# 2noise/ChatTTS

Measured on AMD Instinct MI355X. Metric: audio seconds/sec (RTF), batch=64 per GPU, higher is better.
Workload: dtype f32x3

## Files before the change

chattts_amd/_lib.py:

```python
from __future__ import annotations

import ctypes as C
import os

import numpy as np

import torch

HERE = os.path.dirname(os.path.abspath(__file__))
LIB_PATH = os.environ.get("CTTS_LIB") or os.path.join(HERE, "csrc", "libchattts_amd.so")

F32, BF16 = 0, 1
P = C.c_void_p
PP = C.POINTER(C.c_void_p)


class GptWeights(C.Structure):
    _fields_ = [
        ("n_layers", C.c_int32), ("weight_dtype", C.c_int32), ("kv_dtype", C.c_int32), ("max_pos", C.c_int32),
        ("wqkv", PP), ("wo", PP), ("wgu", PP), ("wd", PP), ("ln1", PP), ("ln2", PP),
        ("norm", P), ("emb_code", P), ("heads", P), ("rope_cos", P), ("rope_sin", P),
        ("rms_eps", C.c_float),
        ("emb_text", P), ("head_text", P), ("n_text", C.c_int32),
        ("wqkv_pk", PP), ("wo_pk", PP), ("wgu_pk", PP), ("wd_pk", PP),
        ("heads_pk", P), ("head_text_pk", P),
        ("wo_hd", PP),
        ("wqkv_x3", PP), ("wo_x3", PP), ("wgu_x3", PP), ("wd_x3", PP),
    ]


class GenState(C.Structure):
    _fields_ = [
        ("B", C.c_int32), ("T", C.c_int32), ("max_new", C.c_int32),
        ("ids_buf", P), ("len", P), ("kv_start", P), ("finish", P), ("end_idx", P), ("hiddens", P),
        ("kcache", P), ("vcache", P), ("q", P), ("nq", C.c_int32),
        ("temperature", P), ("pow_table", P),
        ("top_p_thr", C.c_float), ("use_top_p", C.c_int32), ("top_k", C.c_int32), ("use_top_k", C.c_int32),
        ("min_new", C.c_int32), ("eos", C.c_int32), ("row_offset", C.c_int32),
        ("stop_at", P), ("workspace", P), ("workspace_bytes", C.c_size_t), ("row_map", P), ("n_active", P),
        ("cap", C.c_int32), ("hid_cap", C.c_int32), ("kv_batch", C.c_int32), ("q_batch", C.c_int32), ("prompt_len", P),
        ("infer_text", C.c_int32), ("teacher_ids", P), ("sampled_ids", P), ("order", P),
        ("rng_device", C.c_int32), ("rng_per_step", C.c_int32), ("rng_seed", P), ("rng_nonce", P),
        ("margin", P), ("row_base", P), ("proj_exact", C.c_int32), ("prefill_valid_rows", C.c_int32),
        ("row_sampling", P),
    ]


RS_WINDOW = np.dtype([("in_off", "<i8"), ("n_in", "<i8"), ("origin", "<i8"), ("total", "<i8"), ("o_lo", "<i8"), ("o_hi", "<i8"),
                      ("out_off", "<i8"), ("rate", "<i4"), ("pad", "<i4")])


G711_RANGE = np.dtype([("start", "<i8"), ("n", "<i8"), ("law", "<i4"), ("pad0", "<i4"), ("pad1", "<i8")])


class Rate(C.Structure):
    _fields_ = [("taps", P), ("L", C.c_int32), ("M", C.c_int32), ("K", C.c_int32), ("reserved", C.c_int32)]


class SamplingRow(C.Structure):
    _fields_ = [
        ("temperature", C.c_float * 4), ("pow_table", C.c_float * 17), ("use_penalty", C.c_int32),
        ("top_p_thr", C.c_float), ("use_top_p", C.c_int32), ("top_k", C.c_int32), ("use_top_k", C.c_int32),
        ("min_new", C.c_int32), ("reserved0", C.c_int32), ("rng_seed", C.c_uint64), ("rng_per_step", C.c_int32),
        ("reserved1", C.c_int32),
    ]


class CodecWeights(C.Structure):
    _fields_ = [
        ("conv_in0_w", P), ("conv_in0_b", P), ("conv_in2_w", P), ("conv_in2_b", P),
        ("n_dvae_blocks", C.c_int32),
        ("d_dw_w", PP), ("d_dw_b", PP), ("d_ln_w", PP), ("d_ln_b", PP), ("d_pw1_w", PP), ("d_pw1_b", PP),
        ("d_pw2_w", PP), ("d_pw2_b", PP), ("d_gamma", PP),
        ("conv_out_w", P), ("out_conv_w", P), ("coef", P),
        ("v_embed_w", P), ("v_embed_b", P), ("v_norm_w", P), ("v_norm_b", P),
        ("n_vocos_blocks", C.c_int32),
        ("v_dw_w", PP), ("v_dw_b", PP), ("v_ln_w", PP), ("v_ln_b", PP), ("v_pw1_w", PP), ("v_pw1_b", PP),
        ("v_pw2_w", PP), ("v_pw2_b", PP), ("v_gamma", PP),
        ("v_final_w", P), ("v_final_b", P), ("head_w", P), ("head_b", P), ("window", P), ("twiddle", P),
        ("gemm_mode", C.c_int32),
        ("d_pw1_x3p", PP), ("d_pw2_x3p", PP), ("v_pw1_x3p", PP), ("v_pw2_x3p", PP),
    ]


class TrunkWeights(C.Structure):
    _fields_ = [
        ("idim", C.c_int32), ("odim", C.c_int32), ("hidden", C.c_int32), ("bn_dim", C.c_int32), ("n_blocks", C.c_int32),
        ("conv_in0_w", P), ("conv_in0_b", P), ("conv_in2_w", P), ("conv_in2_b", P),
        ("dw_w", PP), ("dw_b", PP), ("ln_w", PP), ("ln_b", PP), ("pw1_w", PP), ("pw1_b", PP), ("pw2_w", PP), ("pw2_b", PP),
        ("gamma", PP), ("conv_out_w", P),
    ]


class DvaeWeights(C.Structure):
    _fields_ = [
        ("encoder", TrunkWeights), ("decoder", TrunkWeights),
        ("ds0_w", P), ("ds0_b", P), ("ds1_w", P), ("ds1_b", P), ("out_conv_w", P), ("coef", P),
        ("q_in_w", P), ("q_in_b", P), ("q_out_w", P), ("q_out_b", P),
        ("levels", C.c_int32 * 4), ("G", C.c_int32), ("R", C.c_int32), ("D", C.c_int32), ("bound_first", C.c_int32),
        ("mel_window", P), ("mel_fb", P), ("twiddle", P),
    ]


I32, F, SZ = C.c_int32, C.c_float, C.c_size_t

SIGNATURES = {
    "ctts_last_error": (C.c_char_p, []),
    "ctts_version": (C.c_int, []),
    "ctts_gpt_create": (C.c_int, [PP, C.POINTER(GptWeights)]),
    "ctts_gpt_destroy": (None, [P]),
    "ctts_gpt_workspace_bytes": (SZ, [I32, I32]),
    "ctts_gpt_prefill": (C.c_int, [P, C.POINTER(GenState), P, P]),
    "ctts_gpt_prefill_chunk": (C.c_int, [P, C.POINTER(GenState), P, I32, I32, I32, P]),
    "ctts_gpt_decode_step": (C.c_int, [P, C.POINTER(GenState), P]),
    "ctts_gpt_graph_build": (C.c_int, [P, C.POINTER(GenState), P]),
    "ctts_gpt_graph_launch": (C.c_int, [P, I32, P]),
    "ctts_gpt_graph_build_rows": (C.c_int, [P, C.POINTER(GenState), I32, P]),
    "ctts_gpt_graph_launch_rows": (C.c_int, [P, I32, I32, P]),
    "ctts_gpt_graph_destroy": (None, [P]),
    "ctts_gpt_profile_begin": (C.c_int, [P, I32, I32, I32]),
    "ctts_gpt_profile_samples": (C.c_int, [P, C.POINTER(C.c_float), I32, C.POINTER(I32)]),
    "ctts_gpt_profile_end": (C.c_int, [P, C.POINTER(I32), C.POINTER(C.c_double)]),
    "ctts_codec_create": (C.c_int, [PP, C.POINTER(CodecWeights)]),
    "ctts_codec_destroy": (None, [P]),
    "ctts_codec_workspace_bytes": (SZ, [I32, I32]),
    "ctts_copy_bytes": (C.c_int, [P, P, SZ, P]),
    "ctts_float_to_int16": (C.c_int, [P, P, P, I32, C.c_int64, C.c_int64, I32, I32, F, P, P]),
    "ctts_dvae_decode": (C.c_int, [P, P, P, I32, I32, P, SZ, P]),
    "ctts_vocos_decode": (C.c_int, [P, P, P, I32, I32, P, SZ, P]),
    "ctts_codec_ragged_workspace_bytes": (SZ, [I32, I32]),
    "ctts_dvae_decode_ragged": (C.c_int, [P, P, P, P, I32, P, P, SZ, P]),
    "ctts_vocos_decode_ragged": (C.c_int, [P, P, P, P, I32, P, P, SZ, P]),
    "ctts_float_to_int16_ragged": (C.c_int, [P, P, P, P, P, I32, I32, F, P, P]),
    "ctts_float_to_int16_groups_scratch_bytes": (SZ, [P, I32, P, I32]),
    "ctts_float_to_int16_groups": (C.c_int, [P, P, P, P, P, I32, P, P, I32, I32, F, P, P, SZ, P]),
    "ctts_resample_supported": (I32, [I32, I32, I32]),
    "ctts_resample_ragged": (C.c_int, [P, P, P, P, P, P, I32, P, P, I32, P, I32, I32, I32, P]),
    "ctts_time_scale_ragged": (C.c_int, [P, P, P, P, P, P, P, P, P, I32, P, I32, I32, P]),
    "ctts_codec_windows_workspace_bytes": (SZ, [I32, I32]),
    "ctts_codec_decode_windows": (C.c_int, [P, P, C.c_int64, C.c_int64, I32, I32, P, P, I32, I32, P, P, I32, F, P, SZ, P]),
    "ctts_resample_windows": (C.c_int, [P, C.c_int64, P, P, I32, P, C.c_int64, P, P, I32, P, I32, I32, I32, P]),
    "ctts_codec_windows_rate_workspace_bytes": (SZ, [I32, I32, C.c_int64]),
    "ctts_codec_decode_windows_rate": (C.c_int, [P, P, C.c_int64, C.c_int64, I32, I32, P, P, P, P, P, P, I32, P, I32, I32, P, P, I32, F, P,
                                                 SZ, P]),
    "ctts_g711_encode_ranges": (C.c_int, [P, P, P, P, I32, P]),
    "ctts_dvae_create": (C.c_int, [PP, C.POINTER(DvaeWeights)]),
    "ctts_dvae_destroy": (None, [P]),
    "ctts_dvae_code_frames": (I32, [I32]),
    "ctts_dvae_encode_workspace_bytes": (SZ, [I32]),
    "ctts_dvae_decode_workspace_bytes": (SZ, [I32, I32]),
    "ctts_dvae_encode": (C.c_int, [P, P, I32, P, P, SZ, P]),
    "ctts_dvae_decode_codes": (C.c_int, [P, P, P, I32, I32, P, SZ, P]),
    "ctts_k_gemm": (C.c_int, [I32, P, P, P, I32, I32, I32, I32, I32, I32, I32, P, F, P, I32, P, P, I32, I32, I32, I32, I32, P]),
    "ctts_k_gemm_x3p": (C.c_int, [P, P, I32, I32, I32, I32, P, P, P, P, P, P]),
    "ctts_k_gemm_h1p": (C.c_int, [P, P, I32, I32, I32, I32, P, P, P, P, P, P]),
    "ctts_stream_create_cu_mask": (C.c_int, [I32, I32, I32, I32, P]),
    "ctts_stream_destroy": (C.c_int, [P]),
    "ctts_k_mlp_fused": (C.c_int, [P, P, P, I32, I32, P, P, P, P, I32, P]),
    "ctts_k_gemm_fast": (C.c_int, [P, I32, P, I32, I32, I32, P, F, I32, P, I32, P, I32, P, P]),
    "ctts_k_qkv_rope": (C.c_int, [P, P, I32, P, F, P, P, P, I32, P, P, I32, P, P, I32, P]),
    "ctts_k_gemm_dec": (C.c_int, [P, P, I32, I32, I32, P, P, F, I32, P, I32, P, I32, P, I32, P]),
    "ctts_k_gemm_dec32x": (C.c_int, [P, C.c_int64, P, C.c_int64, I32, I32, I32, P, P, I32, F, I32, P, I32, P, I32, P, C.c_int64, I32, P, I32, P, P, P]),
    "ctts_k_gemm_pre_x3": (C.c_int, [P, I32, P, P, I32, I32, I32, I32, I32, P, P, P, I32, P]),
    "ctts_k_dec32_last_variant": (C.c_char_p, []),
    "ctts_k_gemm_dec32": (C.c_int, [P, P, I32, I32, I32, P, P, I32, P, F, I32, P, I32, P, I32, P, I32, I32, I32, P]),
    "ctts_k_rows_prep": (C.c_int, [P, P, P, I32, P]),
    "ctts_k_rope_append": (C.c_int, [P, P, P, I32, I32, P, P, I32, P, P, I32, P]),
    "ctts_k_attention": (C.c_int, [P, P, P, I32, I32, P, I32, P, P, I32, P]),
    "ctts_k_attention_prefill": (C.c_int, [P, P, P, I32, P, I32, I32, P, I32, P]),
    "ctts_k_attention_dec": (C.c_int, [P, P, P, I32, P, P, P, I32, P, P, I32, P]),
    "ctts_k_attention_dec2": (C.c_int, [P, P, P, I32, I32, P, P, P, I32, I32, P]),
    "ctts_k_attention_cfg": (C.c_int, [I32, I32, I32]),
    "ctts_k_attention_heads_per_wg": (C.c_int, [I32]),
    "ctts_rccl_unique_id": (C.c_int, [P]),
    "ctts_rccl_comm_create": (C.c_int, [P, I32, P, I32]),
    "ctts_rccl_comm_destroy": (None, [P]),
    "ctts_broadcast_weights": (C.c_int, [P, P, I32, P, I32, P]),
    "ctts_k_attention_oproj": (C.c_int, [P, P, P, I32, P, P, P, I32, P, P, P, P, P, P]),
    "ctts_k_device_guard_probe": (C.c_int, [P, P, P, P, P]),
    "ctts_k_embed_codes": (C.c_int, [P, P, I32, P, P, I32, P]),
    "ctts_k_final_norm": (C.c_int, [P, I32, P, F, P, P, I32, P, I32, I32, P]),
    "ctts_k_sample": (C.c_int, [C.POINTER(GenState), P, P]),
    "ctts_k_sample_text": (C.c_int, [C.POINTER(GenState), P, I32, P]),
    "ctts_k_exp_draws": (C.c_int, [C.c_uint64, I32, I32, I32, I32, P, P]),
    "ctts_k_dwconv_ln": (C.c_int, [P, P, P, P, P, F, I32, P, I32, I32, P]),
    "ctts_k_layernorm": (C.c_int, [P, P, P, F, P, I32, P]),
    "ctts_k_istft": (C.c_int, [P, P, P, P, P, I32, I32, P]),
}

_lib = None


class EngineError(RuntimeError):
    pass


def lib() -> C.CDLL:
    global _lib
    if _lib is None:
        if not os.path.exists(LIB_PATH):
            raise EngineError(
                f"{LIB_PATH} not found: build it with `python -m chattts_amd.build` "
                "(hipcc --offload-arch=gfx950).  chattts_amd has no CPU/eager fallback.")
        l = C.CDLL(LIB_PATH)
        for name, (res, args) in SIGNATURES.items():
            fn = getattr(l, name)
            fn.restype = res
            fn.argtypes = args
        _lib = l
    return _lib


def check(rc: int, what: str = "") -> None:
    if rc != 0:
        msg = lib().ctts_last_error()
        raise EngineError(f"{what}: {msg.decode() if msg else 'unknown error'}")


def ptr(t) -> int:
    return None if t is None else t.data_ptr()


def ptr_array(tensors):
    arr = (C.c_void_p * len(tensors))(*[t.data_ptr() for t in tensors])
    return arr
```

chattts_amd/csrc/capi.hip:

```cpp
#include <hip/hip_runtime.h>
#include <dlfcn.h>
#include <stdarg.h>
#include <stdio.h>
#include <stdlib.h>
#include <string.h>
#include <algorithm>
#include <map>
#include <vector>

#include "../../include/chattts_amd.h"
#include "kernels.hpp"

static thread_local char g_err[512] = "";
int ctts_fail(const char* fmt, ...) {
  va_list ap;
  va_start(ap, fmt);
  vsnprintf(g_err, sizeof(g_err), fmt, ap);
  va_end(ap);
  return -1;
}
#define fail ctts_fail
#define CK(expr)                                                                                   \
  do {                                                                                             \
    hipError_t _e = (expr);                                                                        \
    if (_e != hipSuccess) return fail("%s failed: %s (%s:%d)", #expr, hipGetErrorString(_e), __FILE__, __LINE__); \
  } while (0)

extern "C" const char* ctts_last_error(void) { return g_err; }
extern "C" int ctts_version(void) { return 1; }

static const int HID = 768, INTER = 3072, NHEAD = 12, HDIM = 64, NVQ = 4, NAUDIO = 626, NTEXT_MAX = 21248;

struct ctts_gpt {
  ctts_gpt_weights w;
  std::vector<const void*> wqkv, wo, wgu, wd;
  std::vector<const void*> wqkv_pk, wo_pk, wgu_pk, wd_pk;
  std::vector<const void*> wo_hd;
  std::vector<const void*> wqkv_x3, wo_x3, wgu_x3, wd_x3;
  bool dec_x3 = false;
  bool qkv_att = false;
  bool att_oproj = false;
  bool dec_packed = false;
  bool dec_packed32 = false;
  bool heads_packed = false;
  int pf_mask = 0;
  int temporal_layers = 0;
  bool pre32_packed = true;
  bool embed_fold = false;
  bool pre_compact = true;
  bool pre_x3 = true;
  bool fnorm_fuse = true;
  std::vector<const float*> ln1, ln2;
  hipGraph_t graph = nullptr;
  hipGraphExec_t exec = nullptr;
  hipGraph_t graph_multi = nullptr;
  hipGraphExec_t exec_multi = nullptr;
  struct RowsGraph { hipGraph_t graph = nullptr, gm = nullptr; hipGraphExec_t exec = nullptr, exec_multi = nullptr; };
  std::map<int, RowsGraph> rows_graphs;
  int multi_steps = 1;
  int prof_tag = -1;
  int prof_max = 0;
  bool skip_finished = true;
  int n_cu = 0;
  int prof_stride = 1;
  int prof_seen = 0;
  std::vector<hipEvent_t> ev0, ev1;
  int prof_n = 0;
};

static size_t align_up(size_t v) { return (v + 255) & ~(size_t)255; }
#define ATT_CUS_MAX 512
#define QA_LAYERS_MAX 32
#define QA_STRIDE HO_STRIDE
struct GptWs {
  float *x, *qkv, *ao, *act, *hfin, *logits, *ssq;
  uint16_t* xb;
  uint16_t *xp, *aop, *actp;
  float *xp32, *aop32, *actp32;
  float* hfinp;
  float* rstd;
  RowDesc* desc;
  float* att_part;
  int32_t* att_cnt;
  int32_t* row_map;
  float* rope_cs;
  int32_t* qa_flag;
  float* op_part;
  int32_t* op_cnt;
  size_t op_part_bytes;
  size_t bytes;
};
static size_t cnt_bytes(int B) { return ((size_t)ATT_CUS_MAX + ((size_t)B + 15) / 16 * 16) * sizeof(int32_t); }
static GptWs carve(void* base, int B, int T) {
  const size_t M = (size_t)B * (T > 1 ? T : 1);
  GptWs w;
  size_t off = 0;
  char* p = (char*)base;
  w.x = (float*)(p + off); off += align_up(M * HID * 4);
  w.qkv = (float*)(p + off); off += align_up(M * 3 * HID * 4);
  w.ao = (float*)(p + off); off += align_up(M * HID * 4);
  w.act = (float*)(p + off); off += align_up(M * INTER * 4);
  w.hfin = (float*)(p + off); off += align_up((size_t)B * HID * 4);
  w.logits = (float*)(p + off); off += align_up((size_t)B * NTEXT_MAX * 4);
  w.ssq = (float*)(p + off); off += align_up(M * SSQ_PARTS * 4);
  w.xb = (uint16_t*)(p + off); off += align_up(M * HID * 2);
  const size_t Bp = ((size_t)B + 15) / 16 * 16;
  w.xp = (uint16_t*)(p + off); off += align_up(Bp * HID * 2);
  w.aop = (uint16_t*)(p + off); off += align_up(Bp * HID * 2);
  w.actp = (uint16_t*)(p + off); off += align_up(Bp * INTER * 2);
  const size_t Mp = (M + 15) / 16 * 16;
  w.xp32 = (float*)(p + off); off += align_up(Mp * HID * 4);
  w.aop32 = (float*)(p + off); off += align_up(Mp * HID * 4);
  w.actp32 = (float*)(p + off); off += align_up(Mp * INTER * 4);
  w.hfinp = (float*)(p + off); off += align_up(Bp * HID * 4);
  w.desc = (RowDesc*)(p + off); off += align_up(Mp * sizeof(RowDesc));
  w.rstd = (float*)(p + off); off += align_up(Mp * sizeof(float));
  w.row_map = (int32_t*)(p + off); off += align_up(Bp * sizeof(int32_t));
  w.att_part = (float*)(p + off); off += align_up((size_t)ATT_CUS_MAX * ATT_SPLIT_MAX * 66 * sizeof(float));
  w.att_cnt = (int32_t*)(p + off); off += align_up(cnt_bytes(B));
  w.op_cnt = w.att_cnt + ATT_CUS_MAX;
  w.op_part_bytes = Bp * NHEAD * HID * sizeof(float);
  w.op_part = (float*)(p + off); off += align_up(w.op_part_bytes);
  w.rope_cs = (float*)(p + off); off += align_up(Bp * 64 * sizeof(float));
  w.qa_flag = (int32_t*)(p + off); off += align_up((size_t)QA_LAYERS_MAX * NHEAD * QA_STRIDE * sizeof(int32_t));
  w.bytes = off;
  return w;
}

extern "C" size_t ctts_gpt_workspace_bytes(int32_t B, int32_t T) { return carve(nullptr, B, T).bytes; }

extern "C" int ctts_gpt_create(ctts_gpt** out, const ctts_gpt_weights* w) {
  if (!out || !w || w->n_layers <= 0) return fail("ctts_gpt_create: bad arguments");
  ctts_gpt* g = new ctts_gpt();
  g->w = *w;
  const int L = w->n_layers;
  g->wqkv.assign(w->wqkv, w->wqkv + L);
  g->wo.assign(w->wo, w->wo + L);
  g->wgu.assign(w->wgu, w->wgu + L);
  g->wd.assign(w->wd, w->wd + L);
  g->ln1.assign(w->ln1, w->ln1 + L);
  g->ln2.assign(w->ln2, w->ln2 + L);
  if (w->wqkv_pk && w->wo_pk && w->wgu_pk && w->wd_pk) {
    g->wqkv_pk.assign(w->wqkv_pk, w->wqkv_pk + L);
    g->wo_pk.assign(w->wo_pk, w->wo_pk + L);
    g->wgu_pk.assign(w->wgu_pk, w->wgu_pk + L);
    g->wd_pk.assign(w->wd_pk, w->wd_pk + L);
    const char* e = getenv("CTTS_DEC_PACKED");
    const bool on = !(e && atoi(e) == 0);
    g->dec_packed = on && w->weight_dtype == CTTS_BF16;
    g->dec_packed32 = on && w->weight_dtype != CTTS_BF16 && w->kv_dtype != CTTS_BF16;
  }
  { const char* e = getenv("CTTS_DEC_PACKED"); g->heads_packed = w->heads_pk != nullptr && !(e && atoi(e) == 0); }
  if (w->wqkv_x3 && w->wo_x3 && w->wgu_x3 && w->wd_x3 && w->weight_dtype != CTTS_BF16 && w->kv_dtype != CTTS_BF16) {
    g->wqkv_x3.assign(w->wqkv_x3, w->wqkv_x3 + L);
    g->wo_x3.assign(w->wo_x3, w->wo_x3 + L);
    g->wgu_x3.assign(w->wgu_x3, w->wgu_x3 + L);
    g->wd_x3.assign(w->wd_x3, w->wd_x3 + L);
    g->dec_x3 = true;
  }
  if (w->wo_hd && g->dec_packed) {
    g->wo_hd.assign(w->wo_hd, w->wo_hd + L);
    const char* e = getenv("CTTS_ATT_OPROJ");
    g->att_oproj = e && atoi(e) == 1;
  }
  { const char* e = getenv("CTTS_SKIP_FINISHED"); if (e && atoi(e) == 0) g->skip_finished = false; }
  { const char* e = getenv("CTTS_FNORM_FUSE"); if (e && atoi(e) == 0) g->fnorm_fuse = false; }
  { const char* e = getenv("CTTS_W_TEMPORAL_LAYERS"); if (e) g->temporal_layers = atoi(e); }
  { const char* e = getenv("CTTS_PF"); if (e) g->pf_mask = atoi(e); }
  { const char* e = getenv("CTTS_QKV_ATT"); g->qkv_att = e && atoi(e) == 1; }
  { const char* e = getenv("CTTS_PRE32_PACKED"); if (e && atoi(e) == 0) g->pre32_packed = false; }
  { const char* e = getenv("CTTS_PRE_X3"); if (e && atoi(e) == 0) g->pre_x3 = false; }
  { const char* e = getenv("CTTS_PRE_COMPACT"); if (e && atoi(e) == 0) g->pre_compact = false; }
  { const char* e = getenv("CTTS_EMBED_FOLD"); if (e) g->embed_fold = atoi(e) != 0; }
  {
    int dev = 0, cus = 0;
    const char* e = getenv("CTTS_ATT_SPLIT");
    if (e && atoi(e) == 1 && hipGetDevice(&dev) == hipSuccess &&
        hipDeviceGetAttribute(&cus, hipDeviceAttributeMultiprocessorCount, dev) == hipSuccess && cus > 0 && cus <= ATT_CUS_MAX)
      g->n_cu = cus;
  }
  *out = g;
  return 0;
}

extern "C" void ctts_gpt_graph_destroy(ctts_gpt* g) {
  if (!g) return;
  if (g->exec) { (void)hipGraphExecDestroy(g->exec); g->exec = nullptr; }
  if (g->graph) { (void)hipGraphDestroy(g->graph); g->graph = nullptr; }
  if (g->exec_multi) { (void)hipGraphExecDestroy(g->exec_multi); g->exec_multi = nullptr; }
  if (g->graph_multi) { (void)hipGraphDestroy(g->graph_multi); g->graph_multi = nullptr; }
  for (auto& kv : g->rows_graphs) {
    if (kv.second.exec) (void)hipGraphExecDestroy(kv.second.exec);
    if (kv.second.graph) (void)hipGraphDestroy(kv.second.graph);
    if (kv.second.exec_multi) (void)hipGraphExecDestroy(kv.second.exec_multi);
    if (kv.second.gm) (void)hipGraphDestroy(kv.second.gm);
  }
  g->rows_graphs.clear();
}

extern "C" void ctts_gpt_destroy(ctts_gpt* g) {
  if (!g) return;
  ctts_gpt_graph_destroy(g);
  for (auto e : g->ev0) (void)hipEventDestroy(e);
  for (auto e : g->ev1) (void)hipEventDestroy(e);
  delete g;
}

thread_local hipEvent_t ctts_prof_start = nullptr, ctts_prof_stop = nullptr;

struct Prof {
  ctts_gpt* g; bool on;
  Prof(ctts_gpt* g_, int tag, hipStream_t, bool allow) : g(g_), on(false) {
    if (allow && g->prof_tag == tag && g->prof_n < g->prof_max && (g->prof_seen++ % g->prof_stride) == 0) {
      on = true;
      ctts_prof_start = g->ev0[g->prof_n];
      ctts_prof_stop = g->ev1[g->prof_n];
    }
  }
  ~Prof() {
    if (on) { g->prof_n++; ctts_prof_start = nullptr; ctts_prof_stop = nullptr; }
  }
};

static_assert(sizeof(SamplingRow) == sizeof(ctts_sampling_row) && sizeof(ctts_sampling_row) == 128, "ctts_sampling_row layout");
static_assert(offsetof(SamplingRow, pow_table) == offsetof(ctts_sampling_row, pow_table) &&
              offsetof(SamplingRow, min_new) == offsetof(ctts_sampling_row, min_new) &&
              offsetof(SamplingRow, rng_seed) == offsetof(ctts_sampling_row, rng_seed) &&
              offsetof(SamplingRow, rng_per_step) == offsetof(ctts_sampling_row, rng_per_step), "ctts_sampling_row layout");

static SampleArgs make_sample_args(const ctts_gen_state* s, const float* logits) {
  SampleArgs a;
  a.logits = logits; a.ids_buf = s->ids_buf; a.tcap = s->cap ? s->cap : s->T + s->max_new; a.T = s->T; a.len = s->len; a.finish = s->finish;
  a.end_idx = s->end_idx; a.q = s->q; a.nq = s->nq; a.temperature = s->temperature; a.pow_table = s->pow_table;
  a.top_p_thr = s->top_p_thr; a.use_top_p = s->use_top_p; a.top_k = s->top_k; a.use_top_k = s->use_top_k;
  a.min_new = s->min_new; a.eos = s->eos; a.row_offset = s->row_offset; a.max_input_ids = NAUDIO - 1; a.stop_at = s->stop_at;
  a.B = s->B; a.row_map = nullptr; a.n_active = nullptr; a.prompt_len = s->prompt_len; a.q_rows = s->q_batch ? s->q_batch : s->B;
  a.teacher = s->teacher_ids; a.teacher_stride = s->hid_cap ? s->hid_cap : s->max_new; a.sampled = s->sampled_ids;
  a.dbg = nullptr;
  { const char* e = getenv("CTTS_SAMPLE_DBG_PTR"); if (e) a.dbg = (long long*)strtoull(e, nullptr, 0); }
  a.desc = nullptr; a.rng_device = s->rng_device; a.rng_per_step = s->rng_per_step; a.rng_seed = reinterpret_cast<const unsigned long long*>(s->rng_seed);
  a.rng_nonce = s->rng_nonce;
  a.margin = s->margin; a.row_base = s->row_base;
  a.rows = reinterpret_cast<const SamplingRow*>(s->row_sampling);
  memset(&a.next, 0, sizeof(a.next));
  return a;
}

static int check_state(const ctts_gpt* g, const ctts_gen_state* s, int ws_T = 0) {
  if (!g || !s) return fail("null engine/state");
  if (s->B <= 0 || s->T <= 0 || s->max_new <= 0) return fail("bad B/T/max_new");
  const int cap_ = s->cap ? s->cap : s->T + s->max_new;
  if (cap_ > g->w.max_pos) return fail("slot capacity T + max_new (%d) exceeds the RoPE table (%d)", cap_, g->w.max_pos);
  if (s->cap && s->T + 1 > s->cap) return fail("prompt does not fit the slot capacity");
  if (s->workspace_bytes < ctts_gpt_workspace_bytes(s->B, ws_T > 0 ? ws_T : s->T)) return fail("workspace too small");
  if (!s->rng_device && (s->nq <= 0 || !s->q)) return fail("q draws missing");
  if (s->rng_device && !s->rng_seed && !s->row_sampling) return fail("rng_device needs the rng_seed device scalar (or row_sampling)");
  if (g->w.weight_dtype == CTTS_BF16 && g->w.kv_dtype != CTTS_BF16) return fail("perf mode needs a bf16 KV cache");
  if (s->infer_text) {
    if (!g->w.emb_text || !g->w.head_text || g->w.n_text <= 0 || g->w.n_text > NTEXT_MAX) return fail("text head/embedding not loaded");
    if (s->pow_table) return fail("refine-text mode does not support a repetition penalty (the reference's own processor mis-broadcasts there)");
    if (s->eos < 0 || s->eos >= g->w.n_text) return fail("bad eos for text mode");
  }
  return 0;
}

static bool dev_compact(const ctts_gpt* g, const ctts_gen_state* s) {
  return s->row_map == nullptr && s->n_active != nullptr && g->skip_finished;
}

static bool prefill_compacts(const ctts_gpt* g, const ctts_gen_state* s) {
  return g->w.weight_dtype != CTTS_BF16 && g->dec_x3 && !s->proj_exact && g->pre_x3 && g->pre_compact && s->row_map == nullptr &&
         s->prefill_valid_rows > 0 && s->prefill_valid_rows < s->B * s->T;
}

static int run_step(ctts_gpt* g, const ctts_gen_state* s, int q_per_b, hipStream_t st, bool prof_ok, int slot0 = 0, bool heads = true,
                    int ws_T = 0, int rows = 0, int pre_rows = 0, const EmbedNext* next = nullptr) {
  const GptWs ws = carve(s->workspace, s->B, ws_T ? ws_T : s->T);
  const int B = s->B, Bh = (q_per_b == 1 && rows > 0 && rows < s->B) ? rows : s->B, M = q_per_b == 1 ? Bh : (pre_rows > 0 ? pre_rows : B * q_per_b);
  const int cmax = s->cap ? s->cap : s->T + s->max_new;
  const int wt = g->w.weight_dtype, kt = g->w.kv_dtype;
  const size_t kv_layer = (size_t)(s->kv_batch ? s->kv_batch : B) * NHEAD * cmax * HDIM * (kt == CTTS_BF16 ? 2 : 4);
  const bool dec = q_per_b == 1;
  const int32_t* rmap = (dec && dev_compact(g, s)) ? ws.row_map : s->row_map;
  const bool no_compact = dec && !g->skip_finished && s->row_map == nullptr;
  const int32_t* nact = (dec && !no_compact) ? s->n_active : nullptr;
  GptRowMap rm{q_per_b, s->len, s->kv_start, rmap, nact, (dec && g->skip_finished) ? s->finish : nullptr, nullptr, nullptr, nullptr, 0, slot0, 0};
  const bool fast = wt == CTTS_BF16;
  const bool packed = fast && dec && g->dec_packed;
  if (dec || pre_rows > 0) rm.desc = ws.desc;
  if (dec && dev_compact(g, s)) rm.desc_covers_all = 1;
  if (packed && g->n_cu > 0) { rm.sp_part = ws.att_part; rm.sp_cnt = ws.att_cnt; rm.sp_cus = g->n_cu; }
  if (packed) { const char* e = getenv("CTTS_ATT_DBG_PTR"); if (e) rm.dbg = (long long*)strtoull(e, nullptr, 0); }
  const bool packed32_ = !fast && dec && ((g->dec_x3 && !s->proj_exact) || g->dec_packed32);
  const bool fuse_fnorm = dec && heads && g->fnorm_fuse && g->heads_packed && (packed || packed32_) &&
                          (s->infer_text ? g->w.head_text_pk : g->w.heads_pk) != nullptr;
  for (int l = 0; packed && l < g->w.n_layers; ++l) {
    void* kc = (char*)s->kcache + kv_layer * l;
    void* vc = (char*)s->vcache + kv_layer * l;
    DecGemmArgs d;
    memset(&d, 0, sizeof(d));
    d.M = M; d.eps = g->w.rms_eps; d.n_active = nact;
    d.force_nt = l < g->temporal_layers ? 1 : 0;
#ifdef CTTS_PF_BUILD
    const PfDesc pf_none{nullptr, 0, 0};
    const PfDesc pf_o{(const char*)g->wo_pk[l], 16u * HID * 2u, HID / 16u};
    const PfDesc pf_gu{(const char*)g->wgu_pk[l], 16u * HID * 2u, 2u * INTER / 16u};
    const PfDesc pf_d{(const char*)g->wd_pk[l], 16u * INTER * 2u, HID / 16u};
    const PfDesc pf_next = l + 1 < g->w.n_layers ? PfDesc{(const char*)g->wqkv_pk[l + 1], 16u * HID * 2u, 3u * HID / 16u}
                           : (fuse_fnorm && !s->infer_text) ? PfDesc{(const char*)g->w.heads_pk, 16u * HID * 4u, (NVQ * NAUDIO + 15u) / 16u} : pf_none;
    d.pf[0] = (g->pf_mask & 1) ? pf_o : pf_none; d.pf[1] = (g->pf_mask & 16) ? pf_gu : pf_none;
    rm.pf = (g->pf_mask & 2) ? pf_gu : pf_none;
#endif
    d.Ap = ws.xp; d.Wp = (const uint16_t*)g->wqkv_pk[l]; d.N = 3 * HID; d.K = HID; d.ssq_in = ws.ssq; d.epi = FEPI_QKV_ROPE;
    d.C32 = ws.qkv; d.ldc = 3 * HID; d.desc = ws.desc; d.cos_t = g->w.rope_cos; d.sin_t = g->w.rope_sin;
    d.kc = (uint16_t*)kc; d.vc = (uint16_t*)vc; d.cmax = cmax;
    const bool fuse_qa = g->qkv_att && M <= 64 && kv_layer < ((size_t)1 << 31) && g->w.n_layers <= QA_LAYERS_MAX && g->n_cu == 0 && g->pf_mask == 0 && !(g->att_oproj) && rm.dbg == nullptr;
    bool need_o = true;
    if (fuse_qa) {
      d.ho_flag = ws.qa_flag + (size_t)l * NHEAD * QA_STRIDE; rm.qf_flag = d.ho_flag; d.rope_cs = ws.rope_cs; rm.qf_kv_bytes = (int)kv_layer;
      Prof p(g, 3, st, prof_ok);
      CK(launch_qkv_attention(d, kc, vc, cmax, ws.aop, rm, M, st));
    } else {
      { Prof p(g, 1, st, prof_ok); CK(launch_gemm_dec(d, st)); }
      if (g->att_oproj && g->n_cu == 0) {
        rm.wo_h = (const uint16_t*)g->wo_hd[l]; rm.op_part = ws.op_part; rm.op_part_bytes = (int)ws.op_part_bytes; rm.op_cnt = ws.op_cnt;
        rm.x32 = ws.x; rm.xp = ws.xp; rm.ssq = ws.ssq;
        Prof p(g, 3, st, prof_ok);
        CK(launch_attention_oproj(ws.qkv, kc, vc, cmax, rm, M, st));
        need_o = false;
      } else {
        Prof p(g, 3, st, prof_ok);
        CK(launch_attention(ws.qkv, kc, vc, kt, cmax, ws.aop, 2, rm, M, st));
      }
    }
    if (need_o) {
      d.Ap = ws.aop; d.Wp = (const uint16_t*)g->wo_pk[l]; d.N = HID; d.ssq_in = nullptr; d.epi = FEPI_RES; d.C32 = ws.x; d.ldc = HID;
      d.Cp = ws.xp; d.kch_out = HID / 32; d.ssq_out = ws.ssq; d.ho_flag = nullptr;
      Prof p(g, 4, st, prof_ok);
      CK(launch_gemm_dec(d, st));
    }
    d.Ap = ws.xp; d.Wp = (const uint16_t*)g->wgu_pk[l]; d.N = INTER; d.ssq_in = ws.ssq; d.epi = FEPI_SILU; d.C32 = nullptr;
    d.Cp = ws.actp; d.kch_out = INTER / 32; d.ssq_out = nullptr;
#ifdef CTTS_PF_BUILD
    d.pf[0] = pf_none; d.pf[1] = pf_none; (void)pf_d; (void)pf_next;
#endif
    { Prof p(g, 5, st, prof_ok); CK(launch_gemm_dec(d, st)); }
    d.Ap = ws.actp; d.Wp = (const uint16_t*)g->wd_pk[l]; d.N = HID; d.K = INTER; d.ssq_in = nullptr; d.epi = FEPI_RES; d.C32 = ws.x;
    d.ldc = HID; d.Cp = ws.xp; d.kch_out = HID / 32; d.ssq_out = ws.ssq;
    d.Cp32 = (fuse_fnorm && l == g->w.n_layers - 1) ? ws.xp32 : nullptr;
    { Prof p(g, 6, st, prof_ok); CK(launch_gemm_dec(d, st)); }
  }
  for (int l = 0; fast && !packed && l < g->w.n_layers; ++l) {
    void* kc = (char*)s->kcache + kv_layer * l;
    void* vc = (char*)s->vcache + kv_layer * l;
    uint16_t* aob = (uint16_t*)ws.ao;
    uint16_t* actb = (uint16_t*)ws.act;
    FastGemmArgs f;
    memset(&f, 0, sizeof(f));
    f.M = M; f.eps = g->w.rms_eps; f.n_active = nact; f.row_map = rmap; f.slot0 = slot0;
    f.A = ws.xb; f.lda = HID; f.W = (const uint16_t*)g->wqkv[l]; f.N = 3 * HID; f.K = HID; f.ssq_in = ws.ssq; f.epi = FEPI_QKV_ROPE;
    f.C32 = ws.qkv; f.ldc = 3 * HID;
    f.q_per_b = q_per_b; f.len = s->len; f.kv_start = s->kv_start; f.cos_t = g->w.rope_cos; f.sin_t = g->w.rope_sin;
    f.kc = (uint16_t*)kc; f.vc = (uint16_t*)vc; f.cmax = cmax;
    { Prof p(g, 1, st, prof_ok); CK(launch_gemm_fast(f, st)); }
    { Prof p(g, 3, st, prof_ok); CK(launch_attention(ws.qkv, kc, vc, kt, cmax, aob, 1, rm, M, st)); }
    f.A = aob; f.W = (const uint16_t*)g->wo[l]; f.N = HID; f.K = HID; f.ssq_in = nullptr; f.epi = FEPI_RES; f.C32 = ws.x; f.ldc = HID;
    f.Cb = ws.xb; f.ldcb = HID; f.ssq_out = ws.ssq;
    { Prof p(g, 4, st, prof_ok); CK(launch_gemm_fast(f, st)); }
    f.A = ws.xb; f.W = (const uint16_t*)g->wgu[l]; f.N = INTER; f.K = HID; f.ssq_in = ws.ssq; f.epi = FEPI_SILU; f.C32 = nullptr;
    f.Cb = actb; f.ldcb = INTER; f.ssq_out = nullptr;
    { Prof p(g, 5, st, prof_ok); CK(launch_gemm_fast(f, st)); }
    f.A = actb; f.lda = INTER; f.W = (const uint16_t*)g->wd[l]; f.N = HID; f.K = INTER; f.ssq_in = nullptr; f.epi = FEPI_RES;
    f.C32 = ws.x; f.ldc = HID; f.Cb = ws.xb; f.ldcb = HID; f.ssq_out = ws.ssq;
    { Prof p(g, 6, st, prof_ok); CK(launch_gemm_fast(f, st)); }
  }
  const bool x3 = !fast && dec && g->dec_x3 && !s->proj_exact;
  const size_t Bp16 = ((size_t)M + 15) / 16 * 16;
  for (int l = 0; x3 && l < g->w.n_layers; ++l) {
    void* kc = (char*)s->kcache + kv_layer * l;
    void* vc = (char*)s->vcache + kv_layer * l;
    uint16_t* xpx = reinterpret_cast<uint16_t*>(ws.xp32);
    uint16_t* aopx = reinterpret_cast<uint16_t*>(ws.aop32);
    uint16_t* actx = reinterpret_cast<uint16_t*>(ws.actp32);
    Dec32xArgs d;
    memset(&d, 0, sizeof(d));
    d.M = M; d.eps = g->w.rms_eps; d.n_active = nact;
    d.Ap = xpx; d.a_plane = Bp16 * HID; d.Wp = (const uint16_t*)g->wqkv_x3[l]; d.w_plane = (size_t)3 * HID * HID; d.N = 3 * HID; d.K = HID;
    d.rms = 1; d.X = ws.x; d.ldx = HID; d.ssq_in = ws.ssq; d.rope_cs = ws.rope_cs; d.epi = D32_EPI_QKV_ROPE; d.C = ws.qkv; d.ldc = 3 * HID; d.desc = ws.desc;
    d.cos_t = g->w.rope_cos; d.sin_t = g->w.rope_sin; d.kc = (float*)kc; d.vc = (float*)vc; d.cmax = cmax;
    { Prof p(g, 1, st, prof_ok); CK(launch_gemm_dec32x(d, st)); }
    rm.x3_plane = Bp16 * HID;
    { Prof p(g, 3, st, prof_ok); CK(launch_attention(ws.qkv, kc, vc, kt, cmax, aopx, 4, rm, M, st)); }
    d.Ap = aopx; d.a_plane = Bp16 * HID; d.Wp = (const uint16_t*)g->wo_x3[l]; d.w_plane = (size_t)HID * HID; d.N = HID; d.rms = 0; d.X = nullptr;
    d.ssq_in = nullptr; d.ssq_out = ws.ssq;
    d.epi = EPI_RES; d.C = ws.x; d.ldc = HID; d.res = ws.x; d.ldr = HID; d.Cp = xpx; d.c_plane = Bp16 * HID; d.kch_out = HID / 32;
    { Prof p(g, 4, st, prof_ok); CK(launch_gemm_dec32x(d, st)); }
    d.Ap = xpx; d.a_plane = Bp16 * HID; d.Wp = (const uint16_t*)g->wgu_x3[l]; d.w_plane = (size_t)2 * INTER * HID; d.N = INTER; d.rms = 1; d.X = ws.x;
    d.ssq_in = ws.ssq; d.ssq_out = nullptr;
    d.epi = EPI_SILU_MUL; d.C = nullptr; d.res = nullptr; d.Cp = actx; d.c_plane = Bp16 * INTER; d.kch_out = INTER / 32;
    { Prof p(g, 5, st, prof_ok); CK(launch_gemm_dec32x(d, st)); }
    d.Ap = actx; d.a_plane = Bp16 * INTER; d.Wp = (const uint16_t*)g->wd_x3[l]; d.w_plane = (size_t)HID * INTER; d.N = HID; d.K = INTER; d.rms = 0;
    d.ssq_in = nullptr; d.ssq_out = ws.ssq;
    d.X = nullptr; d.epi = EPI_RES; d.C = ws.x; d.ldc = HID; d.res = ws.x; d.ldr = HID; d.Cp = xpx; d.c_plane = Bp16 * HID; d.kch_out = HID / 32;
    d.Cp32 = (fuse_fnorm && l == g->w.n_layers - 1) ? ws.hfinp : nullptr; d.kch32_out = HID / 16;
    { Prof p(g, 6, st, prof_ok); CK(launch_gemm_dec32x(d, st)); }
  }
  const bool packed32 = !fast && dec && g->dec_packed32 && !x3;
  for (int l = 0; packed32 && l < g->w.n_layers; ++l) {
    void* kc = (char*)s->kcache + kv_layer * l;
    void* vc = (char*)s->vcache + kv_layer * l;
    Dec32Args d;
    memset(&d, 0, sizeof(d));
    d.M = M; d.eps = g->w.rms_eps; d.n_active = nact;
    d.Ap = ws.xp32; d.Wp = (const float*)g->wqkv_pk[l]; d.N = 3 * HID; d.K = HID; d.X = ws.x; d.ldx = HID; d.norm_w = g->ln1[l];
    d.epi = D32_EPI_QKV_ROPE; d.C = ws.qkv; d.ldc = 3 * HID; d.desc = ws.desc; d.cos_t = g->w.rope_cos; d.sin_t = g->w.rope_sin;
    d.kc = (float*)kc; d.vc = (float*)vc; d.cmax = cmax;
    { Prof p(g, 1, st, prof_ok); CK(launch_gemm_dec32(d, st)); }
    { Prof p(g, 3, st, prof_ok); CK(launch_attention(ws.qkv, kc, vc, kt, cmax, ws.aop32, 3, rm, M, st)); }
    d.Ap = ws.aop32; d.Wp = (const float*)g->wo_pk[l]; d.N = HID; d.X = nullptr; d.norm_w = nullptr; d.epi = EPI_RES; d.C = ws.x; d.ldc = HID;
    d.res = ws.x; d.ldr = HID; d.Cp = ws.xp32; d.kch_out = HID / 16;
    { Prof p(g, 4, st, prof_ok); CK(launch_gemm_dec32(d, st)); }
    d.Ap = ws.xp32; d.Wp = (const float*)g->wgu_pk[l]; d.N = INTER; d.X = ws.x; d.norm_w = g->ln2[l]; d.epi = EPI_SILU_MUL; d.C = nullptr;
    d.res = nullptr; d.Cp = ws.actp32; d.kch_out = INTER / 16;
    { Prof p(g, 5, st, prof_ok); CK(launch_gemm_dec32(d, st)); }
    d.Ap = ws.actp32; d.Wp = (const float*)g->wd_pk[l]; d.N = HID; d.K = INTER; d.X = nullptr; d.norm_w = nullptr; d.epi = EPI_RES;
    d.C = ws.x; d.ldc = HID; d.res = ws.x; d.ldr = HID; d.Cp = ws.xp32; d.kch_out = HID / 16;
    { Prof p(g, 6, st, prof_ok); CK(launch_gemm_dec32(d, st)); }
  }
  const bool pre_x3 = !fast && !dec && g->dec_x3 && !s->proj_exact && g->pre_x3;
  const bool pre32 = !fast && !dec && g->dec_packed32 && g->pre32_packed && !pre_x3;
  if (pre32) {
    CK(launch_prefill_prep32(ws.x, ws.xp32, ws.desc, q_per_b, slot0, s->kv_start, s->row_map, M, st));
  }
  for (int l = 0; pre32 && l < g->w.n_layers; ++l) {
    void* kc = (char*)s->kcache + kv_layer * l;
    void* vc = (char*)s->vcache + kv_layer * l;
    Dec32Args d;
    memset(&d, 0, sizeof(d));
    d.M = M; d.eps = g->w.rms_eps; d.n_active = nullptr;
    CK(launch_rows_rstd32(ws.x, HID, M, g->w.rms_eps, ws.rstd, st));
    d.Ap = ws.xp32; d.Wp = (const float*)g->wqkv_pk[l]; d.N = 3 * HID; d.K = HID; d.norm_w = g->ln1[l];
    d.epi = D32_EPI_QKV_ROPE; d.C = ws.qkv; d.ldc = 3 * HID; d.desc = ws.desc; d.cos_t = g->w.rope_cos; d.sin_t = g->w.rope_sin;
    d.kc = (float*)kc; d.vc = (float*)vc; d.cmax = cmax;
    CK(launch_gemm_pre32(d, ws.rstd, st));
    CK(launch_attention(ws.qkv, kc, vc, kt, cmax, ws.aop32, 3, rm, M, st));
    d.Ap = ws.aop32; d.Wp = (const float*)g->wo_pk[l]; d.N = HID; d.norm_w = nullptr; d.epi = EPI_RES; d.C = ws.x; d.ldc = HID;
    d.res = ws.x; d.ldr = HID; d.Cp = ws.xp32; d.kch_out = HID / 16;
    CK(launch_gemm_pre32(d, nullptr, st));
    CK(launch_rows_rstd32(ws.x, HID, M, g->w.rms_eps, ws.rstd, st));
    d.Ap = ws.xp32; d.Wp = (const float*)g->wgu_pk[l]; d.N = INTER; d.norm_w = g->ln2[l]; d.epi = EPI_SILU_MUL; d.C = nullptr;
    d.res = nullptr; d.Cp = ws.actp32; d.kch_out = INTER / 16;
    CK(launch_gemm_pre32(d, ws.rstd, st));
    d.Ap = ws.actp32; d.Wp = (const float*)g->wd_pk[l]; d.N = HID; d.K = INTER; d.norm_w = nullptr; d.epi = EPI_RES;
    d.C = ws.x; d.ldc = HID; d.res = ws.x; d.ldr = HID; d.Cp = ws.xp32; d.kch_out = HID / 16;
    CK(launch_gemm_pre32(d, nullptr, st));
  }
  for (int l = 0; !fast && !packed32 && !pre32 && !x3 && l < g->w.n_layers; ++l) {
    void* kc = (char*)s->kcache + kv_layer * l;
    void* vc = (char*)s->vcache + kv_layer * l;
    GemmArgs a;
    memset(&a, 0, sizeof(a));
    a.taps = 1;
    a.n_active = nact;
    a.A = ws.x; a.lda = HID; a.W = g->wqkv[l]; a.C = ws.qkv; a.ldc = 3 * HID; a.M = M; a.N = 3 * HID; a.K = HID; a.wt = wt;
    a.epi = EPI_STORE; a.norm_w = g->ln1[l]; a.eps = g->w.rms_eps;
    if (pre_x3) { CK(launch_rows_rstd32(ws.x, HID, M, g->w.rms_eps, ws.rstd, st)); CK(launch_gemm_pre_x3(a, ws.rstd, st)); }
    else { Prof p(g, 1, st, prof_ok); CK(launch_gemm_skinny(a, st)); }
    { Prof p(g, 2, st, prof_ok); CK(launch_rope_append(ws.qkv, kc, vc, kt, cmax, g->w.rope_cos, g->w.rope_sin, rm, M, st)); }
    { Prof p(g, 3, st, prof_ok); CK(launch_attention(ws.qkv, kc, vc, kt, cmax, ws.ao, 0, rm, M, st)); }
    a.A = ws.ao; a.lda = HID; a.W = g->wo[l]; a.C = ws.x; a.ldc = HID; a.N = HID; a.K = HID; a.epi = EPI_RES; a.norm_w = nullptr;
    a.res = ws.x; a.ldr = HID;
    if (pre_x3) CK(launch_gemm_pre_x3(a, nullptr, st));
    else { Prof p(g, 4, st, prof_ok); CK(launch_gemm_skinny(a, st)); }
    a.A = ws.x; a.W = g->wgu[l]; a.C = ws.act; a.ldc = INTER; a.N = INTER; a.K = HID; a.epi = EPI_SILU_MUL; a.norm_w = g->ln2[l];
    a.res = nullptr;
    if (pre_x3) { CK(launch_rows_rstd32(ws.x, HID, M, g->w.rms_eps, ws.rstd, st)); CK(launch_gemm_pre_x3(a, ws.rstd, st)); }
    else { Prof p(g, 5, st, prof_ok); CK(launch_gemm_skinny(a, st)); }
    a.A = ws.act; a.lda = INTER; a.W = g->wd[l]; a.C = ws.x; a.ldc = HID; a.N = HID; a.K = INTER; a.epi = EPI_RES; a.norm_w = nullptr;
    a.res = ws.x; a.ldr = HID;
    if (pre_x3) CK(launch_gemm_pre_x3(a, nullptr, st));
    else { Prof p(g, 6, st, prof_ok); CK(launch_gemm_skinny(a, st)); }
  }
  if (!heads) return 0;
  if (fuse_fnorm) {
    const int nlog = s->infer_text ? g->w.n_text : NVQ * NAUDIO;
    Dec32Args d;
    memset(&d, 0, sizeof(d));
    d.Ap = x3 ? ws.hfinp : ws.xp32; d.Wp = s->infer_text ? g->w.head_text_pk : g->w.heads_pk; d.M = Bh; d.N = (nlog + 15) / 16 * 16; d.K = HID; d.n_active = nact;
    d.epi = EPI_STORE; d.C = ws.logits; d.ldc = nlog; d.n_cols = nlog;
    d.fnorm = 1; d.norm_w = g->w.norm; d.eps = g->w.rms_eps; d.desc = ws.desc; d.hid = s->hiddens; d.hid_cap = s->hid_cap ? s->hid_cap : s->max_new;
    d.T = s->T; d.prompt_len = s->prompt_len;
    Prof p(g, 8, st, prof_ok);
    CK(launch_gemm_dec32(d, st));
  } else {
  { Prof p(g, 7, st, prof_ok);
    CK(launch_final_norm(ws.x, q_per_b, g->w.norm, g->w.rms_eps, ws.hfin, s->hiddens, s->hid_cap ? s->hid_cap : s->max_new, s->len, s->T, Bh, rmap,
                         nact, s->prompt_len, st, ws.hfinp, pre_rows > 0 ? ws.row_map : nullptr)); }
  {
    const int nlog = s->infer_text ? g->w.n_text : NVQ * NAUDIO;
    const float* hpk = s->infer_text ? g->w.head_text_pk : g->w.heads_pk;
    if (g->heads_packed && hpk != nullptr) {
      Dec32Args d;
      memset(&d, 0, sizeof(d));
      d.Ap = ws.hfinp; d.Wp = hpk; d.M = Bh; d.N = (nlog + 15) / 16 * 16; d.K = HID; d.n_active = nact; d.epi = EPI_STORE;
      d.C = ws.logits; d.ldc = nlog; d.n_cols = nlog;
      Prof p(g, 8, st, prof_ok);
      CK(launch_gemm_dec32(d, st));
    } else {
    GemmArgs a;
    memset(&a, 0, sizeof(a));
    a.taps = 1;
    a.A = ws.hfin; a.lda = HID; a.W = s->infer_text ? g->w.head_text : g->w.heads; a.C = ws.logits; a.ldc = nlog; a.M = Bh; a.N = nlog;
    a.K = HID; a.wt = WT_F32; a.epi = EPI_STORE; a.n_active = nact;
    Prof p(g, 8, st, prof_ok);
    CK(launch_gemm_skinny(a, st));
    }
  }
  }
  {
    Prof p(g, 9, st, prof_ok);
    SampleArgs sa = make_sample_args(s, ws.logits);
    sa.B = Bh;
    sa.row_map = rmap; sa.n_active = nact;
    if (dec && dev_compact(g, s)) sa.desc = ws.desc;
    if (next != nullptr && sa.desc != nullptr && !s->infer_text) sa.next = *next;
    if (s->infer_text) CK(launch_sample_text(sa, g->w.n_text, st));
    else CK(launch_sample(sa, st));
  }
  return 0;
}

extern "C" int ctts_gpt_prefill(ctts_gpt* g, const ctts_gen_state* s, const float* emb, void* stream) {
  if (check_state(g, s)) return -1;
  CttsDeviceGuard dg(stream);
  hipStream_t st = (hipStream_t)stream;
  const GptWs ws = carve(s->workspace, s->B, s->T);
  CK(hipMemsetAsync(ws.att_cnt, 0, cnt_bytes(s->B), st));
  if (prefill_compacts(g, s)) {
    CK(launch_prefill_compact(emb, ws.x, ws.desc, ws.row_map, s->B, s->T, s->kv_start, st));
    if (run_step(g, s, s->T, st, false, 0, true, 0, 0, s->prefill_valid_rows)) return -1;
    CK(hipMemsetAsync(carve(s->workspace, s->B, 1).att_cnt, 0, cnt_bytes(s->B), st));
    return 0;
  }
  CK(hipMemcpyAsync(ws.x, emb, (size_t)s->B * s->T * HID * 4, hipMemcpyDeviceToDevice, st));
  if (g->w.weight_dtype == CTTS_BF16) CK(launch_rows_prep(ws.x, ws.xb, ws.ssq, s->B * s->T, st));
  if (run_step(g, s, s->T, st, false)) return -1;
  CK(hipMemsetAsync(carve(s->workspace, s->B, 1).att_cnt, 0, cnt_bytes(s->B), st));
  return 0;
}

extern "C" int ctts_gpt_prefill_chunk(ctts_gpt* g, const ctts_gen_state* s, const float* emb_chunk, int32_t t0, int32_t tc, int32_t last,
                                      void* stream) {
  if (check_state(g, s, tc > 0 ? tc : 1)) return -1;
  if (t0 < 0 || tc <= 0 || t0 + tc > s->T || (last && t0 + tc != s->T)) return fail("ctts_gpt_prefill_chunk: bad chunk [%d, %d) of a %d-slot prompt", t0, t0 + tc, s->T);
  if (s->workspace_bytes < ctts_gpt_workspace_bytes(s->B, tc)) return fail("workspace too small for the chunk");
  CttsDeviceGuard dg(stream);
  hipStream_t st = (hipStream_t)stream;
  const GptWs ws = carve(s->workspace, s->B, tc);
  CK(hipMemcpyAsync(ws.x, emb_chunk, (size_t)s->B * tc * HID * 4, hipMemcpyDeviceToDevice, st));
  if (g->w.weight_dtype == CTTS_BF16) CK(launch_rows_prep(ws.x, ws.xb, ws.ssq, s->B * tc, st));
  if (run_step(g, s, tc, st, false, t0, last != 0, tc)) return -1;
  if (last) CK(hipMemsetAsync(carve(s->workspace, s->B, 1).att_cnt, 0, cnt_bytes(s->B), st));
  return 0;
}

static int decode_body(ctts_gpt* g, const ctts_gen_state* s, hipStream_t st, bool prof_ok, int rows = 0, bool skip_embed = false,
                       bool fold_next = false) {
  const GptWs ws = carve(s->workspace, s->B, 1);
  EmbedNext nx;
  memset(&nx, 0, sizeof(nx));
  { Prof p(g, 0, st, prof_ok); const bool fast = g->w.weight_dtype == CTTS_BF16;
    const bool packed = fast && g->dec_packed;
    const bool dc = dev_compact(g, s);
    const bool x3 = !fast && g->dec_x3 && !s->proj_exact;
    StepPrep sp{ws.desc, s->kv_start, g->skip_finished ? s->finish : nullptr, (packed || x3) ? 1 : 0, (!fast && g->dec_packed32 && !x3) ? ws.xp32 : nullptr,
                dc ? ws.row_map : nullptr,
                dc ? const_cast<int32_t*>(s->n_active) : nullptr, dc ? s->order : nullptr,
                ((packed && g->qkv_att && g->w.n_layers <= QA_LAYERS_MAX) || x3) ? ws.rope_cs : nullptr, g->w.rope_cos, g->w.rope_sin,
                (packed && g->qkv_att && g->w.n_layers <= QA_LAYERS_MAX) ? ws.qa_flag : nullptr, g->w.n_layers * NHEAD, QA_STRIDE};
    const int32_t* nact0 = (!g->skip_finished && s->row_map == nullptr) ? nullptr : s->n_active;
    uint16_t* xb = fast ? (packed ? ws.xp : ws.xb) : x3 ? reinterpret_cast<uint16_t*>(ws.xp32) : nullptr;
    if (x3) sp.xb_lo_plane = ((size_t)((rows > 0 && rows < s->B) ? rows : s->B) + 15) / 16 * 16 * HID;
    const bool foldable = dc && !s->infer_text && sp.zero_p == nullptr;
    if (fold_next && foldable) { nx.emb_code = g->w.emb_code; nx.x = ws.x; nx.xb = xb; nx.ssq = (fast || x3) ? ws.ssq : nullptr; nx.sp = sp; }
    if (skip_embed && foldable) {  }
    else if (s->infer_text)
      CK(launch_embed_text(g->w.emb_text, g->w.n_text, s->ids_buf, s->cap ? s->cap : s->T + s->max_new, s->len, ws.x, xb,
                           (fast || x3) ? ws.ssq : nullptr, s->B, s->row_map, nact0, st, &sp));
    else
      CK(launch_embed_codes(g->w.emb_code, s->ids_buf, s->cap ? s->cap : s->T + s->max_new, s->len, ws.x, xb, (fast || x3) ? ws.ssq : nullptr, s->B,
                            s->row_map, nact0, st, &sp)); }
  return run_step(g, s, 1, st, prof_ok, 0, true, 1, rows, 0, nx.x != nullptr ? &nx : nullptr);
}

extern "C" int ctts_gpt_decode_step(ctts_gpt* g, const ctts_gen_state* s, void* stream) {
  if (check_state(g, s, 1)) return -1;
  CttsDeviceGuard dg(stream);
  return decode_body(g, s, (hipStream_t)stream, true);
}

static int capture_graphs(ctts_gpt* g, const ctts_gen_state* s, hipStream_t st, int rows, hipGraph_t* graph, hipGraphExec_t* exec, hipGraph_t* gm,
                          hipGraphExec_t* exec_multi) {
  CK(hipStreamBeginCapture(st, hipStreamCaptureModeThreadLocal));
  const int rc = decode_body(g, s, st, false, rows);
  hipGraph_t gr = nullptr;
  hipError_t e = hipStreamEndCapture(st, &gr);
  if (rc != 0) { if (gr) (void)hipGraphDestroy(gr); return -1; }
  if (e != hipSuccess) return fail("hipStreamEndCapture: %s", hipGetErrorString(e));
  *graph = gr;
  CK(hipGraphInstantiate(exec, gr, nullptr, nullptr, 0));
  if (g->multi_steps > 1) {
    CK(hipStreamBeginCapture(st, hipStreamCaptureModeThreadLocal));
    int rc2 = 0;
    for (int i = 0; i < g->multi_steps && rc2 == 0; ++i)
      rc2 = decode_body(g, s, st, false, rows, g->embed_fold && i > 0, g->embed_fold && i + 1 < g->multi_steps);
    hipGraph_t g2 = nullptr;
    hipError_t e3 = hipStreamEndCapture(st, &g2);
    if (rc2 != 0) { if (g2) (void)hipGraphDestroy(g2); return -1; }
    if (e3 != hipSuccess) return fail("hipStreamEndCapture (multi-step graph): %s", hipGetErrorString(e3));
    *gm = g2;
    CK(hipGraphInstantiate(exec_multi, g2, nullptr, nullptr, 0));
  }
  return 0;
}

extern "C" int ctts_gpt_graph_build(ctts_gpt* g, const ctts_gen_state* s, void* stream) {
  if (check_state(g, s, 1)) return -1;
  CttsDeviceGuard dg(stream);
  ctts_gpt_graph_destroy(g);
  hipStream_t st = (hipStream_t)stream;
  if (st == nullptr) return fail("graph capture needs a non-default stream");
  {
    const GptWs ws = carve(s->workspace, s->B, 1);
    CK(hipMemsetAsync(ws.att_cnt, 0, cnt_bytes(s->B), st));
  }
  { const char* e2 = getenv("CTTS_GRAPH_STEPS"); g->multi_steps = e2 ? atoi(e2) : 8; }
  if (g->multi_steps < 1 || g->multi_steps > 64) g->multi_steps = 1;
  return capture_graphs(g, s, st, 0, &g->graph, &g->exec, &g->graph_multi, &g->exec_multi);
}

extern "C" int ctts_gpt_graph_build_rows(ctts_gpt* g, const ctts_gen_state* s, int32_t rows, void* stream) {
  if (check_state(g, s, 1)) return -1;
  if (!g->exec) return fail("ctts_gpt_graph_build_rows: build the plain graph first");
  if (rows <= 0) return fail("ctts_gpt_graph_build_rows: bad bound");
  if (rows >= s->B || g->rows_graphs.count(rows)) return 0;
  CttsDeviceGuard dg(stream);
  hipStream_t st = (hipStream_t)stream;
  if (st == nullptr) return fail("graph capture needs a non-default stream");
  ctts_gpt::RowsGraph rg;
  if (capture_graphs(g, s, st, rows, &rg.graph, &rg.exec, &rg.gm, &rg.exec_multi)) return -1;
  g->rows_graphs[rows] = rg;
  return 0;
}

extern "C" int ctts_gpt_graph_launch(ctts_gpt* g, int32_t n_steps, void* stream) {
  if (!g || !g->exec) return fail("no captured graph");
  CttsDeviceGuard dg(stream);
  int left = n_steps;
  while (g->exec_multi && left >= g->multi_steps) { CK(hipGraphLaunch(g->exec_multi, (hipStream_t)stream)); left -= g->multi_steps; }
  for (int i = 0; i < left; ++i) CK(hipGraphLaunch(g->exec, (hipStream_t)stream));
  return 0;
}

extern "C" int ctts_gpt_graph_launch_rows(ctts_gpt* g, int32_t n_steps, int32_t rows, void* stream) {
  if (!g || !g->exec) return fail("no captured graph");
  auto it = g->rows_graphs.find(rows);
  if (rows <= 0 || it == g->rows_graphs.end()) return ctts_gpt_graph_launch(g, n_steps, stream);
  CttsDeviceGuard dg(stream);
  int left = n_steps;
  while (it->second.exec_multi && left >= g->multi_steps) { CK(hipGraphLaunch(it->second.exec_multi, (hipStream_t)stream)); left -= g->multi_steps; }
  for (int i = 0; i < left; ++i) CK(hipGraphLaunch(it->second.exec, (hipStream_t)stream));
  return 0;
}

extern "C" int ctts_gpt_profile_begin(ctts_gpt* g, int32_t tag, int32_t max_samples, int32_t stride) {
  if (!g || max_samples <= 0 || stride <= 0) return fail("bad profile args");
  while ((int)g->ev0.size() < max_samples) {
    hipEvent_t a, b;
    static int sysfence = -1;
    if (sysfence < 0) { const char* e = getenv("CTTS_PROF_SYSFENCE"); sysfence = (e && atoi(e) == 1) ? 1 : 0; }
    const unsigned fl = sysfence ? hipEventDefault : hipEventDisableSystemFence;
    CK(hipEventCreateWithFlags(&a, fl));
    CK(hipEventCreateWithFlags(&b, fl));
    g->ev0.push_back(a);
    g->ev1.push_back(b);
  }
  g->prof_tag = tag; g->prof_max = max_samples; g->prof_n = 0; g->prof_stride = stride; g->prof_seen = 0;
  return 0;
}

extern "C" int ctts_gpt_profile_samples(ctts_gpt* g, float* ms_out, int32_t cap, int32_t* n_samples) {
  if (!g || !ms_out || cap < 0) return fail("bad profile_samples args");
  const int n = g->prof_n < cap ? g->prof_n : cap;
  for (int i = 0; i < n; ++i) {
    CK(hipEventSynchronize(g->ev1[i]));
    CK(hipEventElapsedTime(&ms_out[i], g->ev0[i], g->ev1[i]));
  }
  if (n_samples) *n_samples = n;
  return 0;
}

extern "C" int ctts_gpt_profile_end(ctts_gpt* g, int32_t* n_samples, double* total_ms) {
  if (!g) return fail("null engine");
  double tot = 0.0;
  for (int i = 0; i < g->prof_n; ++i) {
    CK(hipEventSynchronize(g->ev1[i]));
    float ms = 0.f;
    CK(hipEventElapsedTime(&ms, g->ev0[i], g->ev1[i]));
// ... 463 lines not shown
}
extern "C" int ctts_stream_destroy(void* stream) {
  if (stream) CK(hipStreamDestroy((hipStream_t)stream));
  return 0;
}

extern "C" int ctts_k_mlp_fused(const uint16_t* Ap, const uint16_t* W1p, const uint16_t* W2p, int32_t M, int32_t inter, const float* b1,
                                const float* b2, const float* gamma, float* C, int32_t planes, void* stream) {
  if (planes != 1) return fail("ctts_k_mlp_fused: planes must be 1 (fp16 plane)");
  MlpArgs m;
  memset(&m, 0, sizeof(m));
  m.Ap = Ap; m.W1p = W1p; m.W2p = W2p; m.M = M; m.inter = inter; m.b1 = b1; m.b2 = b2; m.gamma = gamma; m.C = C;
  { const char* e = getenv("CTTS_X3_DBG_PTR"); if (e) m.dbg = (long long*)strtoull(e, nullptr, 0); }
  CK(launch_mlp_fused_h1p(m, (hipStream_t)stream));
  return 0;
}
extern "C" int ctts_k_gemm_fast(const uint16_t* A, int32_t lda, const uint16_t* W, int32_t M, int32_t N, int32_t K, const float* ssq_in,
                                float eps, int32_t epi, float* C32, int32_t ldc, uint16_t* Cb, int32_t ldcb, float* ssq_out, void* stream) {
  FastGemmArgs f;
  memset(&f, 0, sizeof(f));
  f.A = A; f.lda = lda; f.W = W; f.M = M; f.N = N; f.K = K; f.ssq_in = ssq_in; f.eps = eps; f.epi = epi; f.C32 = C32; f.ldc = ldc;
  f.Cb = Cb; f.ldcb = ldcb; f.ssq_out = ssq_out;
  { const char* e = getenv("CTTS_GEMM_DBG_PTR"); if (e) f.dbg = (long long*)strtoull(e, nullptr, 0); }
  CK(launch_gemm_fast(f, (hipStream_t)stream));
  return 0;
}
extern "C" int ctts_k_qkv_rope(const uint16_t* A, const uint16_t* W, int32_t M, const float* ssq_in, float eps, float* qkv, uint16_t* kcache,
                               uint16_t* vcache, int32_t cmax, const float* cos_tab, const float* sin_tab, int32_t q_per_b,
                               const int32_t* len, const int32_t* kv_start, int32_t force_mb, void* stream) {
  FastGemmArgs f;
  memset(&f, 0, sizeof(f));
  f.A = A; f.lda = HID; f.W = W; f.M = M; f.N = 3 * HID; f.K = HID; f.ssq_in = ssq_in; f.eps = eps; f.epi = FEPI_QKV_ROPE; f.C32 = qkv;
  f.ldc = 3 * HID; f.q_per_b = q_per_b; f.len = len; f.kv_start = kv_start; f.cos_t = cos_tab; f.sin_t = sin_tab; f.kc = kcache;
  f.vc = vcache; f.cmax = cmax; f.force_mb = force_mb;
  CK(launch_gemm_fast(f, (hipStream_t)stream));
  return 0;
}
extern "C" int ctts_k_gemm_dec(const uint16_t* Ap, const uint16_t* Wp, int32_t M, int32_t N, int32_t K, const int32_t* n_active,
                               const float* ssq_in, float eps, int32_t epi, float* C32, int32_t ldc, uint16_t* Cp, int32_t kch_out,
                               float* ssq_out, int32_t force_mb, void* stream) {
  if (epi == FEPI_QKV_ROPE) return fail("ctts_k_gemm_dec: the fused QKV epilogue is reached through the decode step only");
  DecGemmArgs d;
  memset(&d, 0, sizeof(d));
  d.Ap = Ap; d.Wp = Wp; d.M = M; d.N = N; d.K = K; d.n_active = n_active; d.ssq_in = ssq_in; d.eps = eps; d.epi = epi; d.C32 = C32;
  d.ldc = ldc; d.Cp = Cp; d.kch_out = kch_out; d.ssq_out = ssq_out; d.force_mb = force_mb;
  { const char* e = getenv("CTTS_GEMM_DBG_PTR"); if (e) d.dbg = (long long*)strtoull(e, nullptr, 0); }
  CK(launch_gemm_dec(d, (hipStream_t)stream));
  return 0;
}
extern "C" int ctts_k_gemm_dec32(const float* Ap, const float* Wp, int32_t M, int32_t N, int32_t K, const int32_t* n_active, const float* X,
                                 int32_t ldx, const float* norm_w, float eps, int32_t epi, float* C, int32_t ldc, const float* res, int32_t ldr,
                                 float* Cp, int32_t kch_out, int32_t force_mb, int32_t n_cols, void* stream) {
  Dec32Args d;
  memset(&d, 0, sizeof(d));
  d.n_cols = n_cols;
  d.Ap = Ap; d.Wp = Wp; d.M = M; d.N = N; d.K = K; d.n_active = n_active; d.X = X; d.ldx = ldx; d.norm_w = norm_w; d.eps = eps; d.epi = epi;
  d.C = C; d.ldc = ldc; d.res = res; d.ldr = ldr; d.Cp = Cp; d.kch_out = kch_out; d.force_mb = force_mb;
  CK(launch_gemm_dec32(d, (hipStream_t)stream));
  return 0;
}
extern "C" int ctts_k_gemm_dec32x(const uint16_t* Ap, int64_t a_plane, const uint16_t* Wp, int64_t w_plane, int32_t M, int32_t N, int32_t K,
                                  const int32_t* n_active, const float* X, int32_t ldx, float eps, int32_t epi, float* C, int32_t ldc,
                                  const float* res, int32_t ldr, uint16_t* Cp, int64_t c_plane, int32_t kch_out, float* Cp32, int32_t force_mb,
                                  const float* ssq_in, float* ssq_out, void* stream) {
  Dec32xArgs d;
  memset(&d, 0, sizeof(d));
  d.ssq_in = ssq_in; d.ssq_out = ssq_out;
  d.Ap = Ap; d.a_plane = (size_t)a_plane; d.Wp = Wp; d.w_plane = (size_t)w_plane; d.M = M; d.N = N; d.K = K; d.n_active = n_active;
  d.rms = X != nullptr || ssq_in != nullptr; d.X = X; d.ldx = ldx; d.eps = eps; d.epi = epi; d.C = C; d.ldc = ldc; d.res = res; d.ldr = ldr;
  d.Cp = Cp; d.c_plane = (size_t)c_plane; d.kch_out = kch_out; d.Cp32 = Cp32; d.kch32_out = N / 16; d.force_mb = force_mb;
  CK(launch_gemm_dec32x(d, (hipStream_t)stream));
  return 0;
}
extern "C" const char* ctts_k_dec32_last_variant(void) { return dec32_last_variant(); }
extern "C" int ctts_k_rows_prep(const float* x32, uint16_t* xb, float* ssq, int32_t M, void* stream) {
  CK(launch_rows_prep(x32, xb, ssq, M, (hipStream_t)stream));
  return 0;
}
extern "C" int ctts_k_rope_append(float* qkv, void* kcache, void* vcache, int32_t kv_dtype, int32_t cmax, const float* cos_tab,
                                  const float* sin_tab, int32_t q_per_b, const int32_t* len, const int32_t* kv_start, int32_t M,
                                  void* stream) {
  GptRowMap rm{q_per_b, len, kv_start, nullptr, nullptr, nullptr, nullptr, nullptr, nullptr, 0, 0, 0};
  CK(launch_rope_append(qkv, kcache, vcache, kv_dtype, cmax, cos_tab, sin_tab, rm, M, (hipStream_t)stream));
  return 0;
}
extern "C" int ctts_k_attention(const float* qkv, const void* kcache, const void* vcache, int32_t kv_dtype, int32_t cmax, float* out,
                                int32_t q_per_b, const int32_t* len, const int32_t* kv_start, int32_t M, void* stream) {
  GptRowMap rm{q_per_b, len, kv_start, nullptr, nullptr, nullptr, nullptr, nullptr, nullptr, 0, 0, 0};
  CK(launch_attention(qkv, kcache, vcache, kv_dtype, cmax, out, 0, rm, M, (hipStream_t)stream));
  return 0;
}
extern "C" int ctts_k_attention_prefill(const float* qkv, const uint16_t* kcache, const uint16_t* vcache, int32_t cmax, float* out, int32_t q_per_b,
                                        int32_t slot0, const int32_t* kv_start, int32_t M, void* stream) {
  GptRowMap rm{q_per_b, nullptr, kv_start, nullptr, nullptr, nullptr, nullptr, nullptr, nullptr, 0, slot0, 0};
  CK(launch_attention(qkv, kcache, vcache, WT_BF16, cmax, out, 0, rm, M, (hipStream_t)stream));
  return 0;
}
extern "C" int ctts_k_attention_dec(const float* qkv, const uint16_t* kcache, const uint16_t* vcache, int32_t cmax, uint16_t* out_packed,
                                    const int32_t* desc, const int32_t* n_active, int32_t M, float* part, int32_t* cnt, int32_t n_cu,
                                    void* stream) {
  if (n_cu < 0 || n_cu > ATT_CUS_MAX) return fail("ctts_k_attention_dec: bad n_cu");
  GptRowMap rm{1, nullptr, nullptr, nullptr, n_active, nullptr, reinterpret_cast<const RowDesc*>(desc), part, cnt, n_cu, 0, 0};
  CK(launch_attention(qkv, kcache, vcache, WT_BF16, cmax, out_packed, 2, rm, M, (hipStream_t)stream));
  return 0;
}
extern "C" int ctts_k_attention_dec2(const float* qkv, const void* kcache, const void* vcache, int32_t kv_dtype, int32_t cmax, void* out_packed,
                                     const int32_t* desc, const int32_t* n_active, int32_t covers_all, int32_t M, void* stream) {
  if (!desc || M <= 0 || kv_dtype < 0 || kv_dtype > 2) return fail("ctts_k_attention_dec2: bad arguments");
  GptRowMap rm{1, nullptr, nullptr, nullptr, n_active, nullptr, reinterpret_cast<const RowDesc*>(desc), nullptr, nullptr, 0, 0, covers_all};
  if (kv_dtype == 2) rm.x3_plane = ((size_t)M + 15) / 16 * 16 * HID;
  CK(launch_attention(qkv, kcache, vcache, kv_dtype == CTTS_BF16 ? WT_BF16 : WT_F32, cmax, out_packed, kv_dtype == CTTS_BF16 ? 2 : kv_dtype == 2 ? 4 : 3, rm, M,
                      (hipStream_t)stream));
  return 0;
}
extern "C" int ctts_k_attention_cfg(int32_t persist, int32_t workgroups, int32_t ring) {
  if (ring > 0 && ring != 2 && ring != 3 && ring != 4) return fail("ctts_k_attention_cfg: ring depth must be 2, 3 or 4");
  attention_persist_override(persist, workgroups, ring);
  return 0;
}
extern "C" int ctts_k_attention_heads_per_wg(int32_t hpw) {
  if (hpw != 1 && hpw != 2 && hpw != 3 && hpw != 4) return fail("ctts_k_attention_heads_per_wg: 1, 2, 3 or 4");
  attention_hpw_override(hpw);
  return 0;
}
extern "C" int ctts_k_attention_oproj(const float* qkv, const uint16_t* kcache, const uint16_t* vcache, int32_t cmax, const uint16_t* wo_hd,
                                      const int32_t* desc, const int32_t* n_active, int32_t M, float* part, int32_t* cnt, float* x32,
                                      uint16_t* xp, float* ssq, void* stream) {
  if (!wo_hd || !desc || !part || !cnt || !x32 || !xp || !ssq || M <= 0) return fail("ctts_k_attention_oproj: bad arguments");
  GptRowMap rm{1, nullptr, nullptr, nullptr, n_active, nullptr, reinterpret_cast<const RowDesc*>(desc), nullptr, nullptr, 0, 0, 0};
  rm.wo_h = wo_hd; rm.op_part = part; rm.op_part_bytes = (int)((size_t)((M + 15) / 16 * 16) * NHEAD * HID * sizeof(float)); rm.op_cnt = cnt;
  rm.x32 = x32; rm.xp = xp; rm.ssq = ssq;
  CK(launch_attention_oproj(qkv, kcache, vcache, cmax, rm, M, (hipStream_t)stream));
  return 0;
}
extern "C" int ctts_k_embed_codes(const float* emb_code, const int64_t* ids_buf, int32_t tcap, const int32_t* len, float* x, int32_t B,
                                  void* stream) {
  CK(launch_embed_codes(emb_code, ids_buf, tcap, len, x, nullptr, nullptr, B, nullptr, nullptr, (hipStream_t)stream));
  return 0;
}
extern "C" int ctts_k_final_norm(const float* x, int32_t q_per_b, const float* w, float eps, float* hfin, float* hiddens,
                                 int32_t max_new, const int32_t* len, int32_t T, int32_t B, void* stream) {
  CK(launch_final_norm(x, q_per_b, w, eps, hfin, hiddens, max_new, len, T, B, nullptr, nullptr, nullptr, (hipStream_t)stream));
  return 0;
}
extern "C" int ctts_k_gemm_pre_x3(const float* A, int32_t lda, const float* W, float* C, int32_t ldc, int32_t M, int32_t N, int32_t K, int32_t epi,
                                  const float* norm_w, const float* rstd, const float* res, int32_t ldr, void* stream) {
  GemmArgs a;
  memset(&a, 0, sizeof(a));
  a.taps = 1; a.A = A; a.lda = lda; a.W = W; a.C = C; a.ldc = ldc; a.M = M; a.N = N; a.K = K; a.wt = WT_F32; a.epi = epi;
  a.norm_w = norm_w; a.res = res; a.ldr = ldr;
  CK(launch_gemm_pre_x3(a, rstd, (hipStream_t)stream));
  return 0;
}
extern "C" int ctts_k_sample(const ctts_gen_state* s, const float* logits, void* stream) {
  if (!s || !logits) return fail("ctts_k_sample: bad arguments");
  CK(launch_sample(make_sample_args(s, logits), (hipStream_t)stream));
  return 0;
}
extern "C" int ctts_k_sample_text(const ctts_gen_state* s, const float* logits, int32_t n_text, void* stream) {
  if (!s || !logits || n_text <= 0 || n_text > NTEXT_MAX) return fail("ctts_k_sample_text: bad arguments");
  CK(launch_sample_text(make_sample_args(s, logits), n_text, (hipStream_t)stream));
  return 0;
}
extern "C" int ctts_k_device_guard_probe(void* stream, int32_t* before, int32_t* stream_dev, int32_t* inside, int32_t* switched) {
  if (!before || !stream_dev || !inside || !switched) return fail("ctts_k_device_guard_probe: null argument");
  int b = -1, in = -1;
  CK(hipGetDevice(&b));
  *stream_dev = -1;
  if (stream != nullptr) { hipDevice_t d; CK(hipStreamGetDevice((hipStream_t)stream, &d)); *stream_dev = (int32_t)d; }
  {
    CttsDeviceGuard dg(stream);
    CK(hipGetDevice(&in));
    *switched = dg.switched ? 1 : 0;
  }
  int after = -1;
  CK(hipGetDevice(&after));
  if (after != b) return fail("CttsDeviceGuard did not restore the current device (%d -> %d)", b, after);
  *before = b; *inside = in;
  return 0;
}
extern "C" int ctts_float_to_int16(const float* wav, int16_t* pcm, uint8_t* keep_bits, int32_t rows, int64_t n, int64_t ld, int32_t per_row,
                                   int32_t product, float keep_thr, uint32_t* peak, void* stream) {
  if (!wav || !pcm || !peak || rows < 0 || n < 0 || ld < n || (product != 0 && product != 1)) return fail("ctts_float_to_int16: bad arguments");
  CttsDeviceGuard dg(stream);
  CK(launch_float_to_int16(wav, n, ld, rows, per_row != 0, product, keep_thr, peak, pcm, keep_bits, (hipStream_t)stream));
  return 0;
}
extern "C" int ctts_float_to_int16_ragged(const float* wav, int16_t* pcm, uint8_t* keep_bits, const int64_t* off_dev, const int64_t* off_host,
                                          int32_t n_seg, int32_t product, float keep_thr, uint32_t* peak, void* stream) {
  if (!wav || !pcm || !peak || !off_dev || !off_host || n_seg < 1 || (product != 0 && product != 1))
    return fail("ctts_float_to_int16_ragged: bad arguments");
  if (off_host[0] != 0) return fail("ctts_float_to_int16_ragged: the first sample offset must be 0");
  long long n_max = 0;
  for (int i = 0; i < n_seg; ++i) {
    if (off_host[i + 1] <= off_host[i]) return fail("ctts_float_to_int16_ragged: segment %d is empty or the offsets do not ascend", i);
    n_max = std::max(n_max, (long long)(off_host[i + 1] - off_host[i]));
  }
  CttsDeviceGuard dg(stream);
  CK(launch_float_to_int16_ragged(wav, (const long long*)off_dev, n_seg, n_max, product, keep_thr, peak, pcm, keep_bits, (hipStream_t)stream));
  return 0;
}
static long long groups_scratch_words(const int64_t* off_host, const int32_t* grp_host, int32_t n_grp, long long* n_max_out) {
  long long n_max = 0;
  for (int g = 0; g < n_grp; ++g) n_max = std::max(n_max, (long long)(off_host[grp_host[g + 1]] - off_host[grp_host[g]]));
  if (n_max_out) *n_max_out = n_max;
  return (long long)n_grp * ((n_max + 2047) / 2048);
}
static int groups_check(const char* who, const int64_t* off_host, int32_t n_seg, const int32_t* grp_host, int32_t n_grp) {
  if (!off_host || !grp_host) return fail("%s: bad arguments", who);
  if (n_grp < 1 || n_grp > 65535) return fail("%s: need 1 <= n_grp <= 65535 (got %d)", who, n_grp);
  if (n_seg < n_grp) return fail("%s: %d groups need at least as many segments (got %d)", who, n_grp, n_seg);
  if (off_host[0] != 0) return fail("%s: the first sample offset must be 0", who);
  for (int i = 0; i < n_seg; ++i)
    if (off_host[i + 1] <= off_host[i]) return fail("%s: segment %d is empty or the offsets do not ascend", who, i);
  if (grp_host[0] != 0 || grp_host[n_grp] != n_seg) return fail("%s: the group table must run from 0 to n_seg", who);
  for (int g = 0; g < n_grp; ++g) {
    if (grp_host[g + 1] <= grp_host[g]) return fail("%s: group %d is empty or the group table does not ascend", who, g);
    if (off_host[grp_host[g + 1]] - off_host[grp_host[g]] >= (1ll << 31)) return fail("%s: group %d holds 2^31 samples or more", who, g);
  }
  return 0;
}
extern "C" size_t ctts_float_to_int16_groups_scratch_bytes(const int64_t* off_host, int32_t n_seg, const int32_t* grp_host, int32_t n_grp) {
  if (groups_check("ctts_float_to_int16_groups_scratch_bytes", off_host, n_seg, grp_host, n_grp)) return 0;
  return (size_t)groups_scratch_words(off_host, grp_host, n_grp, nullptr) * sizeof(uint32_t);
}
extern "C" int ctts_float_to_int16_groups(const float* wav, int16_t* pcm, int64_t* n_kept, const int64_t* off_dev, const int64_t* off_host,
                                          int32_t n_seg, const int32_t* grp_dev, const int32_t* grp_host, int32_t n_grp, int32_t product,
                                          float keep_thr, uint32_t* peak, void* scratch, size_t scratch_bytes, void* stream) {
  const char* who = "ctts_float_to_int16_groups";
  if (!wav || !pcm || !off_dev || !grp_dev || (product != 0 && product != 1)) return fail("%s: bad arguments", who);
  if (!peak || !n_kept) return fail("%s: the peak and count buffers must not be null", who);
  if (groups_check(who, off_host, n_seg, grp_host, n_grp)) return -1;
  if (((uintptr_t)pcm & 15) || ((uintptr_t)n_kept & 7)) return fail("%s: pcm must be 16-byte aligned, n_kept 8-byte aligned", who);
  long long n_max = 0;
  const long long words = groups_scratch_words(off_host, grp_host, n_grp, &n_max);
  if (!scratch || scratch_bytes < (size_t)words * sizeof(uint32_t)) return fail("%s: scratch too small (%zu bytes, need %lld)", who, scratch_bytes, words * 4);
  CttsDeviceGuard dg(stream);
  CK(launch_float_to_int16_groups(wav, (const long long*)off_dev, grp_dev, n_grp, n_max, product, keep_thr, peak, (unsigned*)scratch, pcm,
                                  (long long*)n_kept, (hipStream_t)stream));
  return 0;
}
extern "C" int32_t ctts_resample_supported(int32_t L, int32_t M, int32_t K) { return resample_mode(L, M, K); }
extern "C" int ctts_resample_ragged(const float* x, const int64_t* off_in_dev, const int64_t* off_in_host, float* y, const int64_t* off_out_dev,
                                    const int64_t* off_out_host, int32_t n_seg, const int32_t* sel_dev, const int32_t* sel_host, int32_t n_sel,
                                    const float* taps, int32_t L, int32_t M, int32_t K, void* stream) {
  const char* who = "ctts_resample_ragged";
  if (!x || !y || !off_in_dev || !off_in_host || !off_out_dev || !off_out_host || !taps || n_seg < 1) return fail("%s: bad arguments", who);
  if ((sel_dev == nullptr) != (sel_host == nullptr)) return fail("%s: the segment selection must be given on the device and the host, or on neither", who);
  if (L < 1 || M < 1 || L == M) return fail("%s: need L != M, both positive (got %d/%d)", who, L, M);
  if (resample_mode(L, M, K) == 0)
    return fail("%s: conversion %d/%d with %d taps is not supported (K = 2 width + M; a tile's input span within %d floats, the table within %d)",
                who, L, M, K, RS_LDS_FLOATS, RS_TAB_MAX);
  if (off_in_host[0] != 0 || off_out_host[0] != 0) return fail("%s: the first offsets must be 0", who);
  for (int i = 0; i < n_seg; ++i) {
    if (off_in_host[i + 1] <= off_in_host[i]) return fail("%s: segment %d is empty or the input offsets do not ascend", who, i);
    if (off_out_host[i + 1] <= off_out_host[i]) return fail("%s: segment %d's output is empty or the output offsets do not ascend", who, i);
  }
  if (off_out_host[n_seg] >= (1ll << 31)) return fail("%s: the output holds 2^31 samples or more", who);
  const int n_launch = sel_host ? n_sel : n_seg;
  if (n_launch < 1 || n_launch > 65535) return fail("%s: need 1 <= converted segments <= 65535 (got %d)", who, n_launch);
  long long n_out_max = 0;
  for (int q = 0; q < n_launch; ++q) {
    const int i = sel_host ? sel_host[q] : q;
    if (i < 0 || i >= n_seg) return fail("%s: selected segment %d is outside the pack", who, i);
    const long long n = off_in_host[i + 1] - off_in_host[i], no = off_out_host[i + 1] - off_out_host[i];
    if (n >= (1ll << 31) || no != (n * L + M - 1) / M) return fail("%s: segment %d: %lld samples in need ceil(n L / M) out, got %lld", who, i, n, no);
    n_out_max = std::max(n_out_max, no);
  }
  CttsDeviceGuard dg(stream);
  CK(launch_resample_ragged(x, (const long long*)off_in_dev, y, (const long long*)off_out_dev, sel_dev, n_launch, n_out_max, taps, L, M, K,
                            (hipStream_t)stream));
  return 0;
}
extern "C" int ctts_time_scale_ragged(const float* x, const int64_t* off_in_dev, const int64_t* off_in_host, float* y, const int64_t* off_out_dev,
                                      const int64_t* off_out_host, int32_t* path, const int64_t* path_off_dev, const int64_t* path_off_host,
                                      int32_t n_seg, const float* window, int32_t num, int32_t den, void* stream) {
  const char* who = "ctts_time_scale_ragged";
  if (!x || !y || !path || !window || !off_in_dev || !off_in_host || !off_out_dev || !off_out_host || !path_off_dev || !path_off_host)
    return fail("%s: a null pointer (x, y, path, the window and the three offset tables on the device and the host are needed)", who);
  if (n_seg < 1 || n_seg > 65535) return fail("%s: need 1 <= n_seg <= 65535 (got %d)", who, n_seg);
  if (den != 100 || num < 50 || num > 200) return fail("%s: the speed is num / 100 with 50 <= num <= 200 (got %d/%d)", who, num, den);
  if (num == den) return fail("%s: speed 1 (%d/%d): there is nothing to scale", who, num, den);
  if (off_in_host[0] != 0 || off_out_host[0] != 0 || path_off_host[0] != 0) return fail("%s: the first offsets must be 0", who);
  long long n_out_max = 0;
  for (int i = 0; i < n_seg; ++i) {
    const long long n = off_in_host[i + 1] - off_in_host[i], no = off_out_host[i + 1] - off_out_host[i];
    if (n <= 0) return fail("%s: segment %d is empty or the input offsets do not ascend", who, i);
    if (no <= 0) return fail("%s: segment %d's output is empty or the output offsets do not ascend", who, i);
    if (off_in_host[i + 1] >= (1ll << 31) - 4096) return fail("%s: the input holds 2^31 samples or more (less the 4096 a frame may reach past it)", who);
    if (no != (n * den + num - 1) / num) return fail("%s: segment %d: %lld samples in need ceil(n den / num) out, got %lld", who, i, n, no);
    if (path_off_host[i + 1] - path_off_host[i] != (no + TS_HS - 1) / TS_HS + 1)
      return fail("%s: segment %d: %lld samples out are ceil(n_out / %d) + 1 frames of path, got %lld", who, i, no, TS_HS,
                  (long long)(path_off_host[i + 1] - path_off_host[i]));
    n_out_max = std::max(n_out_max, no);
  }
  if (off_out_host[n_seg] >= (1ll << 31)) return fail("%s: the output holds 2^31 samples or more", who);
  CttsDeviceGuard dg(stream);
  CK(launch_time_scale_ragged(x, (const long long*)off_in_dev, y, (const long long*)off_out_dev, path, (const long long*)path_off_dev, n_seg,
                              n_out_max, window, num, den, (hipStream_t)stream));
  return 0;
}
extern "C" int ctts_copy_bytes(void* dst,const void* src, size_t bytes, void* stream) {
  if (!dst || !src || (bytes & 15) || (((uintptr_t)dst | (uintptr_t)src) & 15)) return fail("ctts_copy_bytes: pointers and size must be 16-byte aligned");
  CttsDeviceGuard dg(stream);
  CK(launch_copy16(src, dst, bytes, (hipStream_t)stream));
  return 0;
// ... 114 lines not shown
```

chattts_amd/csrc/common.hpp:

```cpp
#pragma once
#include <hip/hip_runtime.h>
#include <stdint.h>

typedef uint16_t bf16_t;

typedef float f32x4 __attribute__((ext_vector_type(4)));
typedef float f32x16 __attribute__((ext_vector_type(16)));
typedef __bf16 bf16x8 __attribute__((ext_vector_type(8)));

#define WAVE 64

__device__ __forceinline__ float bf16_to_f32(bf16_t v) { return __uint_as_float(((uint32_t)v) << 16); }

__device__ __forceinline__ bf16_t f32_to_bf16(float f) {
  uint32_t u = __float_as_uint(f);
  if ((u & 0x7fffffffu) > 0x7f800000u) return (bf16_t)0x7fc0;
  u += 0x7fffu + ((u >> 16) & 1u);
  return (bf16_t)(u >> 16);
}

typedef _Float16 f16x8 __attribute__((ext_vector_type(8)));
__device__ __forceinline__ uint32_t pack_f16x2(float a, float b) {
  a = fminf(fmaxf(a, -65504.f), 65504.f);
  b = fminf(fmaxf(b, -65504.f), 65504.f);
  const _Float16 ha = (_Float16)a, hb = (_Float16)b;
  return (uint32_t)__builtin_bit_cast(uint16_t, ha) | ((uint32_t)__builtin_bit_cast(uint16_t, hb) << 16);
}
#define X3_LO_SCALE 2048.0f
#define X3_LO_INV (1.0f / 2048.0f)
__device__ __forceinline__ void x3_split(float v, uint16_t& hi, uint16_t& lo) {
  v = v > 65504.0f ? 65504.0f : (v < -65504.0f ? -65504.0f : v);
  const _Float16 h = (_Float16)v;
  const _Float16 l = (_Float16)((v - (float)h) * X3_LO_SCALE);
  hi = __builtin_bit_cast(uint16_t, h);
  lo = __builtin_bit_cast(uint16_t, l);
}

typedef float f32x2_t __attribute__((ext_vector_type(2)));
typedef __bf16 bf16x2_t __attribute__((ext_vector_type(2)));
__device__ __forceinline__ uint32_t pack_bf16x2(float a, float b) {
  const bf16x2_t r = __builtin_convertvector((f32x2_t){a, b}, bf16x2_t);
  return __builtin_bit_cast(uint32_t, r);
}

__device__ __forceinline__ float wave_sum(float v) {
#pragma unroll
  for (int o = 32; o > 0; o >>= 1) v += __shfl_xor(v, o, 64);
  return v;
}
__device__ __forceinline__ double wave_sum_d(double v) {
#pragma unroll
  for (int o = 32; o > 0; o >>= 1) v += __shfl_xor(v, o, 64);
  return v;
}
__device__ __forceinline__ float wave_max(float v) {
#pragma unroll
  for (int o = 32; o > 0; o >>= 1) v = fmaxf(v, __shfl_xor(v, o, 64));
  return v;
}

template <int CTRL, int ROW_MASK>
__device__ __forceinline__ int dpp_i(int v) {
  return __builtin_amdgcn_update_dpp(v, v, CTRL, ROW_MASK, 0xf, false);
}
__device__ __forceinline__ float wave_max_dpp(float v) {
#define CTTS_FMAX_DPP(C, M) v = fmaxf(v, __int_as_float(dpp_i<C, M>(__float_as_int(v))))
  CTTS_FMAX_DPP(0xB1, 0xf);
  CTTS_FMAX_DPP(0x4E, 0xf);
  CTTS_FMAX_DPP(0x141, 0xf);
  CTTS_FMAX_DPP(0x140, 0xf);
  CTTS_FMAX_DPP(0x142, 0xa);
  CTTS_FMAX_DPP(0x143, 0xc);
#undef CTTS_FMAX_DPP
  return __int_as_float(__builtin_amdgcn_readlane(__float_as_int(v), 63));
}
__device__ __forceinline__ int wave_min_dpp(int v) {
#define CTTS_IMIN_DPP(C, M) v = min(v, dpp_i<C, M>(v))
  CTTS_IMIN_DPP(0xB1, 0xf);
  CTTS_IMIN_DPP(0x4E, 0xf);
  CTTS_IMIN_DPP(0x141, 0xf);
  CTTS_IMIN_DPP(0x140, 0xf);
  CTTS_IMIN_DPP(0x142, 0xa);
  CTTS_IMIN_DPP(0x143, 0xc);
#undef CTTS_IMIN_DPP
  return __builtin_amdgcn_readlane(v, 63);
}

__device__ __forceinline__ float gelu_erf(float x) { return 0.5f * x * (1.0f + erff(x * 0.70710678118654752440f)); }
__device__ __forceinline__ float gelu_fast(float x) {
  const float z = fabsf(x) * 0.70710678118654752440f;
  const float t = __builtin_amdgcn_rcpf(fmaf(0.3275911f, z, 1.0f));
  float p = fmaf(1.061405429f, t, -1.453152027f);
  p = fmaf(p, t, 1.421413741f);
  p = fmaf(p, t, -0.284496736f);
  p = fmaf(p, t, 0.254829592f);
  const float half_erfc = 0.5f * (p * t) * __builtin_amdgcn_exp2f(-1.4426950408889634f * z * z);
  const float phi = x < 0.f ? half_erfc : 1.0f - half_erfc;
  return x * phi;
}
__device__ __forceinline__ float silu_f(float x) { return x / (1.0f + expf(-x)); }

struct alignas(16) u128 {
  uint32_t x, y, z, w;
};

typedef unsigned u32x4_t __attribute__((ext_vector_type(4)));
__device__ __forceinline__ u128 load16_nt(const void* p) {
  const u32x4_t v = __builtin_nontemporal_load(reinterpret_cast<const u32x4_t*>(p));
  u128 r;
  r.x = v.x; r.y = v.y; r.z = v.z; r.w = v.w;
  return r;
}
__device__ __forceinline__ u128 load16(const void* p) { return *reinterpret_cast<const u128*>(p); }
__device__ __forceinline__ u128 load16_sc1(const void* p) {
  const unsigned long long* q = reinterpret_cast<const unsigned long long*>(p);
  const unsigned long long a = __hip_atomic_load(q, __ATOMIC_RELAXED, __HIP_MEMORY_SCOPE_AGENT);
  const unsigned long long b = __hip_atomic_load(q + 1, __ATOMIC_RELAXED, __HIP_MEMORY_SCOPE_AGENT);
  u128 r;
  r.x = (uint32_t)a; r.y = (uint32_t)(a >> 32); r.z = (uint32_t)b; r.w = (uint32_t)(b >> 32);
  return r;
}
__device__ __forceinline__ unsigned xcc_id() {
#if defined(__HIP_DEVICE_COMPILE__)
  unsigned x;
  asm volatile("s_getreg_b32 %0, hwreg(HW_REG_XCC_ID)" : "=s"(x));
  return x;
#else
  return 0;
#endif
}

__device__ __forceinline__ size_t pk_off(int m, int c, int kch) {
  return ((size_t)((m >> 4) * kch + (c >> 5)) * 64 + (((c & 31) >> 3) << 4) + (m & 15)) * 8 + (c & 7);
}
__device__ __forceinline__ size_t pk32_off(int m, int c, int kch) {
  return ((size_t)((m >> 4) * kch + (c >> 4)) * 64 + (((c & 15) >> 2) << 4) + (m & 15)) * 4 + (c & 3);
}
__device__ __forceinline__ float rope_lo(float x1, float x2, float c, float s) {
#pragma clang fp contract(off)
  const float p = x2 * s;
  return __builtin_fmaf(x1, c, -p);
}
__device__ __forceinline__ float rope_hi(float x1, float x2, float c, float s) {
#pragma clang fp contract(off)
  const float p = x1 * s;
  return __builtin_fmaf(x2, c, p);
}
__device__ __forceinline__ float rms_acc4(float ss, const float4 v) {
#pragma clang fp contract(off)
  const float xx = v.x * v.x, yy = v.y * v.y, zz = v.z * v.z, ww = v.w * v.w;
  const float t = ((xx + yy) + zz) + ww;
  return ss + t;
}
__device__ __forceinline__ float rms_rstd_of(float ss, int K, float eps) { return 1.0f / sqrtf(ss / (float)K + eps); }
__device__ __forceinline__ float rms_finish(float ss, int K, float eps) { return rms_rstd_of(wave_sum(ss), K, eps); }
__device__ __forceinline__ float wave_row_rstd(const float* __restrict__ row, int K, float eps, int lane) {
  float ss = 0.f;
  for (int k = lane * 4; k < K; k += 256) ss = rms_acc4(ss, *reinterpret_cast<const float4*>(row + k));
  return rms_finish(ss, K, eps);
}
template <int NR>
__device__ __forceinline__ void wave_rows_rstd_768(const float* const (&rows)[NR], float eps, int lane, float (&rstd)[NR]) {
  float4 v[NR][3];
#pragma unroll
  for (int q = 0; q < NR; ++q)
#pragma unroll
    for (int t = 0; t < 3; ++t) v[q][t] = *reinterpret_cast<const float4*>(rows[q] + lane * 4 + 256 * t);
#pragma unroll
  for (int q = 0; q < NR; ++q) {
    float ss = 0.f;
#pragma unroll
    for (int t = 0; t < 3; ++t) ss = rms_acc4(ss, v[q][t]);
    rstd[q] = rms_finish(ss, 768, eps);
  }
}

#ifdef CTTS_PF_BUILD
struct PfDesc {
  const char* base;
  unsigned tile_bytes;
  unsigned n_tiles;
};
__device__ __forceinline__ void prefetch_weight_tiles(const PfDesc& pf, int lane, unsigned wg, unsigned n_wg) {
  if (pf.base == nullptr) return;
  const unsigned x = wg & 7u, q = wg >> 3;
  if (x >= pf.n_tiles || x >= n_wg) return;
  const unsigned nq = (n_wg - x + 7u) >> 3;
  const unsigned nt = (pf.n_tiles - x + 7u) >> 3;
// ... 13 lines not shown
```

chattts_amd/csrc/kernels.hpp:

```cpp
#pragma once
#include <hip/hip_runtime.h>
#include <hip/hip_ext.h>
#include <stdint.h>

#include "common.hpp"

extern thread_local hipEvent_t ctts_prof_start, ctts_prof_stop;
#define CTTS_LAUNCH(kern, grid, block, st, ...)                                                                   \
  do {                                                                                                            \
    if (ctts_prof_start) {                                                                                        \
      hipExtLaunchKernelGGL(kern, grid, block, 0, st, ctts_prof_start, ctts_prof_stop, 0, __VA_ARGS__);           \
      ctts_prof_start = nullptr; ctts_prof_stop = nullptr;                                                        \
    } else {                                                                                                      \
      hipLaunchKernelGGL(kern, grid, block, 0, st, __VA_ARGS__);                                                  \
    }                                                                                                             \
  } while (0)

#define CTTS_LAUNCH_SMEM(kern, grid, block, smem, st, ...)                                                        \
  do {                                                                                                            \
    if (ctts_prof_start) {                                                                                        \
      hipExtLaunchKernelGGL(kern, grid, block, smem, st, ctts_prof_start, ctts_prof_stop, 0, __VA_ARGS__);        \
      ctts_prof_start = nullptr; ctts_prof_stop = nullptr;                                                        \
    } else {                                                                                                      \
      hipLaunchKernelGGL(kern, grid, block, smem, st, __VA_ARGS__);                                               \
    }                                                                                                             \
  } while (0)

#ifdef CTTS_PROBE_EXIT
#define CTTS_PROBE_RETURN() do { return; } while (0)
#else
#define CTTS_PROBE_RETURN() do { } while (0)
#endif

enum { WT_F32 = 0, WT_BF16 = 1 };

constexpr int HO_STRIDE = 1088;

enum GemmEpi {
  EPI_STORE = 0,
  EPI_RES = 1,
  EPI_SILU_MUL = 2,
  EPI_BIAS = 3,
  EPI_BIAS_GELU = 4,
  EPI_BIAS_SCALE_RES = 5,
  EPI_SCALE = 6,
  EPI_LOG_DIV = 7,
};

struct GemmArgs {
  const float* A;
  const void* W;
  float* C;
  int M, N, K;
  int lda, ldc;
  int wt;
  int epi;
  const float* norm_w;
  float eps;
  const float* res; int ldr;
  const float* bias;
  const float* gamma;
  const int32_t* n_active;
  int taps, cin, frames, pad, dil;
  long long* dbg;
  const int2* seg;
};

hipError_t launch_gemm_skinny(const GemmArgs& a, hipStream_t st);
hipError_t launch_gemm_pre_x3(const GemmArgs& a, const float* rstd, hipStream_t st);

enum FastEpi { FEPI_STORE32 = 0, FEPI_RES = 1, FEPI_SILU = 2, FEPI_QKV_ROPE = 3 };
#define SSQ_PARTS 48
struct FastGemmArgs {
  const uint16_t* A; int lda;
  const uint16_t* W;
  int M, N, K;
  const float* ssq_in;
  float eps;
  int epi;
  float* C32; int ldc;
  uint16_t* Cb; int ldcb;
  float* ssq_out;
  int q_per_b; const int32_t* len; const int32_t* kv_start;
  const int32_t* row_map;
  const int32_t* n_active;
  const float* cos_t; const float* sin_t;
  uint16_t* kc; uint16_t* vc; int cmax;
  int slot0;
  int force_mb;
  int w_nt;
  long long* dbg;
};
hipError_t launch_gemm_fast(const FastGemmArgs& a, hipStream_t st);
bool gemm_prefill_supported(const FastGemmArgs& a);
hipError_t launch_gemm_prefill(const FastGemmArgs& a, hipStream_t st);
hipError_t launch_rows_prep(const float* x32, uint16_t* xb, float* ssq, int M, hipStream_t st);
hipError_t launch_gemm_tiled(const GemmArgs& a, hipStream_t st);
hipError_t launch_gemm_tiled_bf16x3(const GemmArgs& a, hipStream_t st);

struct alignas(16) RowDesc {
  int32_t b;
  int32_t slot;
  int32_t pos;
  int32_t jlo;
};
struct DecGemmArgs {
  const uint16_t* Ap;
  const uint16_t* Wp;
  int M, N, K;
  const int32_t* n_active;
  const float* ssq_in;
  float eps;
  int epi;
  float* C32; int ldc;
  uint16_t* Cp; int kch_out;
  float* Cp32;
  float* ssq_out;
  const RowDesc* desc;
  const float* cos_t; const float* sin_t;
  uint16_t* kc; uint16_t* vc; int cmax;
  int force_mb;
  int w_nt;
  int a_early;
  int force_nt;
#ifdef CTTS_PF_BUILD
  PfDesc pf[2];
#endif
  long long* dbg;
  const float* rope_cs;
  int32_t* ho_flag;
};
hipError_t launch_gemm_dec(const DecGemmArgs& a, hipStream_t st);

struct Dec32Args {
  const float* Ap;
  const float* Wp;
  int M, N, K;
  const int32_t* n_active;
  const float* X; int ldx;
  const float* norm_w; float eps;
  int epi;
  float* C; int ldc;
  const float* res; int ldr;
  float* Cp; int kch_out;
  int n_cols;
  const RowDesc* desc;
  const float* cos_t; const float* sin_t;
  float* kc; float* vc; int cmax;
  int force_mb;
  int w_nt;
  int a_early;
  int fnorm;
  float* hid; int hid_cap;
  int T; const int32_t* prompt_len;
};
enum { D32_EPI_QKV_ROPE = 100 };
hipError_t launch_gemm_dec32(const Dec32Args& a, hipStream_t st);
hipError_t launch_rows_rstd32(const float* X, int ldx, int M, float eps, float* rstd, hipStream_t st);
hipError_t launch_gemm_pre32(const Dec32Args& a, const float* rstd, hipStream_t st);
struct Dec32xArgs {
  const uint16_t* Ap; size_t a_plane;
  const uint16_t* Wp; size_t w_plane;
  int M, N, K;
  const int32_t* n_active;
  int rms; const float* X; int ldx; float eps;
  const float* ssq_in;
  float* ssq_out;
  const float* rope_cs;
  int epi;
  float* C; int ldc;
  const float* res; int ldr;
  uint16_t* Cp; size_t c_plane; int kch_out;
  float* Cp32; int kch32_out;
  const RowDesc* desc; const float* cos_t; const float* sin_t; float* kc; float* vc; int cmax;
  int force_mb;
  int w_nt;
};
hipError_t launch_gemm_dec32x(const Dec32xArgs& a, hipStream_t st);
const char* dec32_last_variant();

struct GptRowMap {
  int q_per_b;
  const int32_t* len;
  const int32_t* kv_start;
  const int32_t* row_map;
  const int32_t* n_active;
  const uint8_t* finish;
  const RowDesc* desc;
  float* sp_part;
  int32_t* sp_cnt;
  int sp_cus;
  int slot0;
  int desc_covers_all;
#ifdef CTTS_PF_BUILD
  PfDesc pf;
#endif
  long long* dbg;
  const uint16_t* wo_h;
  float* op_part;
  int op_part_bytes;
  int32_t* op_cnt;
  float* x32;
  uint16_t* xp;
  float* ssq;
  const int32_t* qf_flag;
  int qf_rows;
  int qf_kv_bytes;
  size_t x3_plane;
};
#define ATT_SPLIT_MAX 8

struct StepPrep {
  RowDesc* desc;
  const int32_t* kv_start;
  const uint8_t* finish;
  int xb_packed;
  float* xp32;
  int32_t* row_map_out;
  int32_t* n_active_out;
  const int32_t* order;
  float* rope_cs; const float* cos_t; const float* sin_t;
  int32_t* zero_p; int zero_n; int zero_stride;
// ... 200 lines not shown
```

chattts_amd/csrc/prefill32x.hip:

```cpp
#include <stdlib.h>

#include "common.hpp"
#include "kernels.hpp"

namespace {

constexpr int XBK = 32, XLD = XBK + 8;
constexpr int XNT = 256;

typedef float xf2 __attribute__((ext_vector_type(2)));
typedef _Float16 xb2 __attribute__((ext_vector_type(2)));

__device__ __forceinline__ void split2(const float a, const float b, uint32_t& hi, uint32_t& lo) {
  const xf2 v = {a > 65504.0f ? 65504.0f : (a < -65504.0f ? -65504.0f : a), b > 65504.0f ? 65504.0f : (b < -65504.0f ? -65504.0f : b)};
  const xb2 h = __builtin_convertvector(v, xb2);
  hi = __builtin_bit_cast(uint32_t, h);
  const xf2 hf = __builtin_convertvector(h, xf2);
  const xb2 l = __builtin_convertvector((v - hf) * X3_LO_SCALE, xb2);
  lo = __builtin_bit_cast(uint32_t, l);
}
__device__ __forceinline__ void split4(const float4 v, ushort4& hi, ushort4& lo) {
  uint32_t h0, l0, h1, l1;
  split2(v.x, v.y, h0, l0);
  split2(v.z, v.w, h1, l1);
  hi = __builtin_bit_cast(ushort4, make_uint2(h0, h1));
  lo = __builtin_bit_cast(ushort4, make_uint2(l0, l1));
}

template <int EPI, int MBLK>
__global__ __launch_bounds__(XNT) void gemm_pre_x3_k(GemmArgs a, const float* __restrict__ rstd) {
  constexpr bool SILU = EPI == EPI_SILU_MUL;
  constexpr int BM = 64 * MBLK;
  constexpr int BN = 128;
  constexpr int BNO = SILU ? 64 : 128;
  __shared__ __attribute__((aligned(16))) uint16_t As[2][2][BM][XLD], Ws[2][2][BN][XLD];
  __shared__ float rstd_s[BM];

  const int tid = threadIdx.x, wave = tid >> 6, lane = tid & 63;
  const int wm = wave & 1, wn = wave >> 1;
  const int M = a.M, N = a.N, K = a.K;
  const int m0 = blockIdx.y * BM, n0 = blockIdx.x * BNO;
  const float* Wf = reinterpret_cast<const float*>(a.W);

  if (rstd != nullptr && tid < BM) rstd_s[tid] = rstd[min(m0 + tid, M - 1)];

  const int lr = tid >> 3, lk = (tid & 7) * 4;
  constexpr int PA = BM / 32;
  const float* ap[PA];
  const float* wp[4];
#pragma unroll
  for (int p = 0; p < PA; ++p) ap[p] = a.A + (size_t)min(m0 + lr + 32 * p, M - 1) * a.lda + lk;
#pragma unroll
  for (int p = 0; p < 4; ++p) {
    const int r = lr + 32 * p;
    const int gr = SILU ? (r < 64 ? n0 + r : N + n0 + (r - 64)) : min(n0 + r, N - 1);
    wp[p] = Wf + (size_t)gr * K + lk;
  }
  float4 ra[PA], rw[4], rg;
#define X_FETCH(K0)                                                                                               \
  do {                                                                                                            \
    _Pragma("unroll") for (int p = 0; p < PA; ++p) ra[p] = *reinterpret_cast<const float4*>(ap[p] + (K0));         \
    _Pragma("unroll") for (int p = 0; p < 4; ++p) rw[p] = *reinterpret_cast<const float4*>(wp[p] + (K0));          \
    rg = a.norm_w != nullptr ? *reinterpret_cast<const float4*>(a.norm_w + (K0) + lk) : make_float4(1.f, 1.f, 1.f, 1.f); \
  } while (0)
#define X_STAGE(SB)                                                                                               \
  do {                                                                                                            \
    _Pragma("unroll") for (int p = 0; p < PA; ++p) {                                                              \
      ushort4 h, l;                                                                                               \
      split4(make_float4(ra[p].x * rg.x, ra[p].y * rg.y, ra[p].z * rg.z, ra[p].w * rg.w), h, l);                  \
      *reinterpret_cast<ushort4*>(&As[SB][0][lr + 32 * p][lk]) = h;                                               \
      *reinterpret_cast<ushort4*>(&As[SB][1][lr + 32 * p][lk]) = l;                                               \
    }                                                                                                             \
    _Pragma("unroll") for (int p = 0; p < 4; ++p) {                                                               \
      ushort4 h, l;                                                                                               \
      split4(rw[p], h, l);                                                                                        \
      *reinterpret_cast<ushort4*>(&Ws[SB][0][lr + 32 * p][lk]) = h;                                               \
      *reinterpret_cast<ushort4*>(&Ws[SB][1][lr + 32 * p][lk]) = l;                                               \
    }                                                                                                             \
  } while (0)

  f32x16 acc[MBLK][2], accx[MBLK][2];
#pragma unroll
  for (int i = 0; i < MBLK; ++i)
#pragma unroll
    for (int j = 0; j < 2; ++j)
#pragma unroll
      for (int r = 0; r < 16; ++r) { acc[i][j][r] = 0.f; accx[i][j][r] = 0.f; }

  X_FETCH(0);
  X_STAGE(0);
  if (XBK < K) X_FETCH(XBK);
  __syncthreads();
  const int ri = lane & 31, kg = (lane >> 5) * 8;
  const int wrow0 = SILU ? wn * 32 : wn * 64, wrow1 = SILU ? 64 + wn * 32 : wn * 64 + 32;
  int sb = 0;
  for (int k0 = 0; k0 < K; k0 += XBK) {
    if (k0 + XBK < K) X_STAGE(sb ^ 1);
    if (k0 + 2 * XBK < K) X_FETCH(k0 + 2 * XBK);
#pragma unroll
    for (int kk = 0; kk < XBK; kk += 16) {
      const f16x8 wh0 = *reinterpret_cast<const f16x8*>(&Ws[sb][0][wrow0 + ri][kk + kg]);
      const f16x8 wl0 = *reinterpret_cast<const f16x8*>(&Ws[sb][1][wrow0 + ri][kk + kg]);
      const f16x8 wh1 = *reinterpret_cast<const f16x8*>(&Ws[sb][0][wrow1 + ri][kk + kg]);
      const f16x8 wl1 = *reinterpret_cast<const f16x8*>(&Ws[sb][1][wrow1 + ri][kk + kg]);
#pragma unroll
      for (int i = 0; i < MBLK; ++i) {
        const f16x8 ah = *reinterpret_cast<const f16x8*>(&As[sb][0][(wm * MBLK + i) * 32 + ri][kk + kg]);
        const f16x8 al = *reinterpret_cast<const f16x8*>(&As[sb][1][(wm * MBLK + i) * 32 + ri][kk + kg]);
        f32x16 x0 = accx[i][0], x1 = accx[i][1];
        x0 = __builtin_amdgcn_mfma_f32_32x32x16_f16(al, wh0, x0, 0, 0, 0);
        x1 = __builtin_amdgcn_mfma_f32_32x32x16_f16(al, wh1, x1, 0, 0, 0);
        x0 = __builtin_amdgcn_mfma_f32_32x32x16_f16(ah, wl0, x0, 0, 0, 0);
        x1 = __builtin_amdgcn_mfma_f32_32x32x16_f16(ah, wl1, x1, 0, 0, 0);
        accx[i][0] = x0; accx[i][1] = x1;
        acc[i][0] = __builtin_amdgcn_mfma_f32_32x32x16_f16(ah, wh0, acc[i][0], 0, 0, 0);
        acc[i][1] = __builtin_amdgcn_mfma_f32_32x32x16_f16(ah, wh1, acc[i][1], 0, 0, 0);
      }
    }
    __syncthreads();
    sb ^= 1;
  }
#undef X_FETCH
#undef X_STAGE

#pragma unroll
  for (int i = 0; i < MBLK; ++i)
#pragma unroll
    for (int j = 0; j < 2; ++j)
#pragma unroll
      for (int r = 0; r < 16; ++r) acc[i][j][r] += accx[i][j][r] * X3_LO_INV;
  const int cl = lane & 31;
#pragma unroll
  for (int i = 0; i < MBLK; ++i) {
#pragma unroll
    for (int r = 0; r < 16; ++r) {
      const int lrow = (wm * MBLK + i) * 32 + (r & 3) + 8 * (r >> 2) + 4 * (lane >> 5);
      const int row = m0 + lrow;
      if (row >= M) continue;
      const float rs = rstd != nullptr ? rstd_s[lrow] : 1.0f;
      if (EPI == EPI_SILU_MUL) {
        const int col = n0 + wn * 32 + cl;
        a.C[(size_t)row * a.ldc + col] = silu_f(acc[i][0][r] * rs) * (acc[i][1][r] * rs);
      } else {
#pragma unroll
        for (int j = 0; j < 2; ++j) {
          const int col = n0 + wn * 64 + j * 32 + cl;
          if (col >= N) continue;
          const float v = acc[i][j][r] * rs;
          a.C[(size_t)row * a.ldc + col] = (EPI == EPI_RES) ? a.res[(size_t)row * a.ldr + col] + v : v;
        }
      }
    }
  }
}

}

hipError_t launch_gemm_pre_x3(const GemmArgs& a, const float* rstd, hipStream_t st) {
  if (a.M <= 0 || a.N <= 0 || a.K <= 0 || (a.K % XBK) || (a.lda & 3) || !a.A || !a.W || !a.C || a.wt != WT_F32 || a.taps != 1) return hipErrorInvalidValue;
  if ((a.norm_w != nullptr) != (rstd != nullptr)) return hipErrorInvalidValue;
  if (a.epi == EPI_SILU_MUL ? (a.N % 64) != 0 : (a.N % 128) != 0) return hipErrorInvalidValue;
  if (a.epi == EPI_RES && !a.res) return hipErrorInvalidValue;
  const dim3 block(XNT);
  const int nx = a.epi == EPI_SILU_MUL ? a.N / 64 : a.N / 128;
  static int force_small = -1;
  if (force_small < 0) { const char* e = getenv("CTTS_PREX3_SMALL"); force_small = e ? atoi(e) : 0; }
  const bool small = force_small == 1 || (force_small != 2 && (long)nx * ((a.M + 127) / 128) < 1024);
  const dim3 grid(nx, small ? (a.M + 63) / 64 : (a.M + 127) / 128);
  switch (a.epi) {
    case EPI_SILU_MUL:
      if (small) CTTS_LAUNCH((gemm_pre_x3_k<EPI_SILU_MUL, 1>), grid, block, st, a, rstd); else CTTS_LAUNCH((gemm_pre_x3_k<EPI_SILU_MUL, 2>), grid, block, st, a, rstd);
      break;
    case EPI_RES:
      if (small) CTTS_LAUNCH((gemm_pre_x3_k<EPI_RES, 1>), grid, block, st, a, rstd); else CTTS_LAUNCH((gemm_pre_x3_k<EPI_RES, 2>), grid, block, st, a, rstd);
      break;
    case EPI_STORE:
      if (small) CTTS_LAUNCH((gemm_pre_x3_k<EPI_STORE, 1>), grid, block, st, a, rstd); else CTTS_LAUNCH((gemm_pre_x3_k<EPI_STORE, 2>), grid, block, st, a, rstd);
      break;
    default: return hipErrorInvalidValue;
  }
  return hipGetLastError();
}
```

chattts_amd/engine.py:

```python
from __future__ import annotations

import ctypes as C
import os
import logging
import math
from dataclasses import dataclass, field
from typing import Iterator, List, Optional, Sequence

import numpy as np
import torch

from . import _lib
from . import g711 as G711
from . import resample as RS
from . import timescale as TS
from ._sync import wait_event, wait_stream
from .config import DVAE, GPT, VOCOS
from .rng import ExpDraws, penalty_table
from .weights import fold_weight_norm, gpt_layer_count

log = logging.getLogger("chattts_amd")


@dataclass
# ... 101 lines not shown
    with torch.cuda.device(dev):
        _lib.check(lib.ctts_stream_create_cu_mask(first, n, stride, 1 if complement else 0, C.byref(h)), "ctts_stream_create_cu_mask")
    return torch.cuda.ExternalStream(h.value, device=dev)


def codec_cu_spec():
    spec = os.environ.get("CTTS_CODEC_CUS", "")
    if not spec:
        return None
    parts = [int(v) for v in spec.split(":")]
    return (parts[2] if len(parts) > 2 else 0), parts[0], (parts[1] if len(parts) > 1 else 1)


def left_pad_starts(attention_mask: torch.Tensor) -> torch.Tensor:
    m = attention_mask.to(torch.bool).cpu()
    T = m.shape[1]
    n = m.sum(1)
    start = T - n
    ar = torch.arange(T)[None, :]
    if not torch.equal(m, ar >= start[:, None]):
        raise NotImplementedError("only left-padded attention masks (what Tokenizer.encode produces) are supported")
    if int(n.min()) <= 0:
        raise ValueError("empty prompt row")
    return start.to(torch.int32)


def rope_row_perm() -> torch.Tensor:
    idx = []
    for h in range(GPT.n_heads):
        for t in range(4):
            idx += [h * 64 + 8 * t + i for i in range(8)] + [h * 64 + 32 + 8 * t + i for i in range(8)]
    return torch.tensor(idx, dtype=torch.long)


def pack_frag(w: torch.Tensor) -> torch.Tensor:
    R, Cc = w.shape
    assert R % 16 == 0 and Cc % 32 == 0
    return w.reshape(R // 16, 16, Cc // 32, 4, 8).permute(0, 2, 3, 1, 4).contiguous()


X3_LO_SCALE = 2048.0


def split_f16(w: torch.Tensor):
    w = w.to(torch.float32).clamp(-65504.0, 65504.0)
    hi = w.to(torch.float16)
    lo = ((w - hi.to(torch.float32)) * X3_LO_SCALE).to(torch.float16)
    return hi, lo


def pack_frag_x3(w: torch.Tensor) -> torch.Tensor:
    hi, lo = split_f16(w)
    return torch.stack([pack_frag(hi), pack_frag(lo)], 0).contiguous()


def unpack_frag_x3(p: torch.Tensor, R: int, Cc: int) -> torch.Tensor:
    return unpack_frag(p[0].float(), R, Cc) + unpack_frag(p[1].float(), R, Cc) / X3_LO_SCALE


def pack_wo_heads(wo: torch.Tensor) -> torch.Tensor:
    assert tuple(wo.shape) == (GPT.hidden, GPT.hidden)
    return wo.view(GPT.hidden, GPT.n_heads, 8, 8).permute(1, 2, 0, 3).contiguous()


def pack_frag32(w: torch.Tensor) -> torch.Tensor:
    R, Cc = w.shape
    assert R % 16 == 0 and Cc % 16 == 0
    return w.reshape(R // 16, 16, Cc // 16, 4, 4).permute(0, 2, 3, 1, 4).contiguous()


def unpack_frag32(p: torch.Tensor, R: int, Cc: int) -> torch.Tensor:
    return p.reshape(R // 16, Cc // 16, 4, 16, 4).permute(0, 3, 1, 2, 4).reshape(R, Cc).contiguous()


def unpack_frag(p: torch.Tensor, R: int, Cc: int) -> torch.Tensor:
    return p.reshape(R // 16, Cc // 32, 4, 16, 8).permute(0, 3, 1, 2, 4).reshape(R, Cc).contiguous()


def rope_tables(max_pos: int, head_dim: int = GPT.head_dim, theta: float = GPT.rope_theta):
    inv_freq = 1.0 / (theta ** (torch.arange(0, head_dim, 2, dtype=torch.int64).to(torch.float32) / head_dim))
    pos = torch.arange(max_pos, dtype=torch.float32)
    freqs = pos[:, None] * inv_freq[None, :]
    return freqs.cos().contiguous(), freqs.sin().contiguous()


class GptEngine:

    NQ_RING = 64
    POLL = 16
    REL_ERR_X3 = 5.3e-6

    def __init__(self, gpt_sd: dict, embed_sd: dict, device: torch.device, dtype: str = "bf16",
                 max_pos: int = GPT.max_pos, logger: logging.Logger = log, rms_eps: float = GPT.rms_eps,
                 rope_theta: float = GPT.rope_theta, certify: Optional[bool] = None, exact_fallback: bool = False):
        if dtype not in ("bf16", "f32", "f32x3"):
            raise ValueError("dtype must be 'bf16' (perf), 'f32' (parity, exact float32) or 'f32x3' (parity, split-fp16 projections)")
        self.lib = _lib.lib()
        self.device = torch.device(device)
        if self.device.type != "cuda":
            raise _lib.EngineError("GptEngine needs a ROCm GPU device (there is no CPU path)")
        self.logger = logger
        self.dtype = dtype
        self.wdt = torch.bfloat16 if dtype == "bf16" else torch.float32
        self.code = _lib.BF16 if dtype == "bf16" else _lib.F32
        self.n_layers = gpt_layer_count(gpt_sd)
        self.max_pos = max_pos
        dev = self.device
        f = lambda t: t.to(torch.float32).contiguous().to(dev)
        wcast = lambda t: t.to(torch.float32).to(self.wdt).contiguous().to(dev)
        self.wqkv, self.wo, self.wgu, self.wd, self.ln1, self.ln2 = [], [], [], [], [], []
        fold = (lambda w, g: w.float() * g.float()[None, :]) if dtype == "bf16" else (lambda w, g: w)
        perm = rope_row_perm() if dtype == "bf16" else torch.arange(GPT.hidden)
        for i in range(self.n_layers):
            p = f"layers.{i}."
            ln1, ln2 = gpt_sd[p + "input_layernorm.weight"], gpt_sd[p + "post_attention_layernorm.weight"]
            self.wqkv.append(wcast(fold(torch.cat([gpt_sd[p + "self_attn.q_proj.weight"][perm], gpt_sd[p + "self_attn.k_proj.weight"][perm],
                                                   gpt_sd[p + "self_attn.v_proj.weight"]], 0), ln1)))
            self.wo.append(wcast(gpt_sd[p + "self_attn.o_proj.weight"]))
            self.wgu.append(wcast(fold(torch.cat([gpt_sd[p + "mlp.gate_proj.weight"], gpt_sd[p + "mlp.up_proj.weight"]], 0), ln2)))
            self.wd.append(wcast(gpt_sd[p + "mlp.down_proj.weight"]))
            self.ln1.append(f(gpt_sd[p + "input_layernorm.weight"]))
            self.ln2.append(f(gpt_sd[p + "post_attention_layernorm.weight"]))
        self.norm = f(gpt_sd["norm.weight"])
        self.emb_code = f(torch.stack([embed_sd[f"emb_code.{k}.weight"] for k in range(GPT.n_vq)], 0))
        self.emb_text = f(embed_sd["emb_text.weight"])
        self.heads = f(torch.cat([fold_weight_norm(embed_sd[f"head_code.{k}.parametrizations.weight.original0"].float(),
                                                   embed_sd[f"head_code.{k}.parametrizations.weight.original1"].float())
                                  for k in range(GPT.n_vq)], 0))
        self.head_text = f(fold_weight_norm(embed_sd["head_text.parametrizations.weight.original0"].float(),
                                            embed_sd["head_text.parametrizations.weight.original1"].float()))
        ng = float(self.norm.pow(2).mean().sqrt())
        self.logit_scale = {False: float(self.heads.pow(2).sum(1).mean().sqrt()) * ng, True: float(self.head_text.pow(2).sum(1).mean().sqrt()) * ng}
        cos, sin = rope_tables(max_pos, theta=rope_theta)
        self.rope_cos, self.rope_sin = cos.to(dev), sin.to(dev)
        self._arrs = [_lib.ptr_array(x) for x in (self.wqkv, self.wo, self.wgu, self.wd, self.ln1, self.ln2)]
        use_packed = os.environ.get("CTTS_DEC_PACKED", "1") != "0"
        self.certify = (dtype == "f32x3") if certify is None else bool(certify)
        self.exact_fallback = bool(exact_fallback) and dtype == "f32x3"
        pk = pack_frag if dtype == "bf16" else pack_frag32
        self.packed, self._pk_arrs = None, None
        rp = rope_row_perm().to(dev)
        qk_perm = torch.cat([rp, GPT.hidden + rp, 2 * GPT.hidden + torch.arange(GPT.hidden, device=dev)])
        if use_packed and (dtype != "f32x3" or self.exact_fallback):
            self.packed = [[pk(t) for t in ws] for ws in (self.wqkv, self.wo, self.wgu, self.wd)]
            if dtype != "bf16":
                self.packed[0] = [pack_frag32(t[qk_perm]) for t in self.wqkv]
            self._pk_arrs = [_lib.ptr_array(x) for x in self.packed]
        self.x3, self._x3_arrs = None, None
        if use_packed and dtype == "f32x3":
            gain = lambda w_, g_: w_.float() * g_.float()[None, :]
            self.x3 = [[pack_frag_x3(gain(t[qk_perm], g_)) for t, g_ in zip(self.wqkv, self.ln1)], [pack_frag_x3(t) for t in self.wo],
                       [pack_frag_x3(gain(t, g_)) for t, g_ in zip(self.wgu, self.ln2)], [pack_frag_x3(t) for t in self.wd]]
            self._x3_arrs = [_lib.ptr_array(x) for x in self.x3]
        self.wo_hd = [pack_wo_heads(t) for t in self.wo] if (use_packed and dtype == "bf16" and os.environ.get("CTTS_ATT_OPROJ") == "1") else None
        self._wo_hd_arr = None if self.wo_hd is None else _lib.ptr_array(self.wo_hd)

        def pad16(t):
            r = (-t.shape[0]) % 16
            return t if r == 0 else torch.cat([t, torch.zeros((r, t.shape[1]), dtype=t.dtype, device=t.device)], 0)
        self.heads_pk = pack_frag32(pad16(self.heads)) if use_packed else None
        self.head_text_pk = pack_frag32(pad16(self.head_text)) if use_packed else None
        w = _lib.GptWeights()
        w.n_layers, w.weight_dtype, w.kv_dtype, w.max_pos = self.n_layers, self.code, self.code, max_pos
        w.wqkv, w.wo, w.wgu, w.wd, w.ln1, w.ln2 = [C.cast(a, _lib.PP) for a in self._arrs]
        w.norm, w.emb_code, w.heads = self.norm.data_ptr(), self.emb_code.data_ptr(), self.heads.data_ptr()
        w.rope_cos, w.rope_sin = self.rope_cos.data_ptr(), self.rope_sin.data_ptr()
        w.rms_eps = float(rms_eps)
        w.emb_text, w.head_text, w.n_text = self.emb_text.data_ptr(), self.head_text.data_ptr(), GPT.n_text
        if self._pk_arrs is not None:
            w.wqkv_pk, w.wo_pk, w.wgu_pk, w.wd_pk = [C.cast(a, _lib.PP) for a in self._pk_arrs]
        w.heads_pk, w.head_text_pk = _lib.ptr(self.heads_pk), _lib.ptr(self.head_text_pk)
        if self._wo_hd_arr is not None:
            w.wo_hd = C.cast(self._wo_hd_arr, _lib.PP)
        if self._x3_arrs is not None:
            w.wqkv_x3, w.wo_x3, w.wgu_x3, w.wd_x3 = [C.cast(a, _lib.PP) for a in self._x3_arrs]
        self._w = w
        h = C.c_void_p()
        _lib.check(self.lib.ctts_gpt_create(C.byref(h), C.byref(w)), "ctts_gpt_create")
        self.handle = h
        spec = codec_cu_spec() if os.environ.get("CTTS_GPT_COMPLEMENT") == "1" else None
        self.stream = cu_masked_stream(self.lib, dev, *spec, True) if spec else torch.cuda.Stream(device=dev)
        self._lane_res = [(self.handle, self.stream)]
        self._lane_res_alt = []
        self._lane_res_text = []
        self.default_lanes = 1
        self.rng = "host"
        self.last_stats = {}
        self._session = None
        self._session_alt = None
        self._session_text = None
        self._draws_cache = None

    def __del__(self):
        try:
            for h, _ in [*getattr(self, "_lane_res", []), *getattr(self, "_lane_res_alt", []), *getattr(self, "_lane_res_text", [])]:
                self.lib.ctts_gpt_destroy(h)
            self._lane_res, self._lane_res_alt, self._lane_res_text = [], [], []
            self.handle = None
        except Exception:
            pass

    def weight_bytes_per_step(self) -> int:
        es = 2 if self.dtype == "bf16" else 4
        per_layer = (3 * 768 * 768 + 768 * 768 + 2 * 3072 * 768 + 768 * 3072) * es
        return per_layer * self.n_layers + self.heads.numel() * 4

    def embed_prompt(self, input_ids: torch.Tensor, text_mask: torch.Tensor) -> torch.Tensor:
        ids = input_ids.to(self.device)
        tm = text_mask.to(self.device).bool()
        et = self.emb_text[ids[..., 0].clamp(0, GPT.n_text - 1)]
        cid = ids.clamp(0, GPT.n_audio - 1)
        ec = self.emb_code[0][cid[..., 0]]
        for k in range(1, GPT.n_vq):
            ec = ec + self.emb_code[k][cid[..., k]]
        return torch.where(tm[..., None], et, ec).contiguous()

    def _lane_resources(self, n: int, pool: str = ""):
        pool = getattr(self, "_lane_res" + pool)
        while len(pool) < n:
            h = C.c_void_p()
            _lib.check(self.lib.ctts_gpt_create(C.byref(h), C.byref(self._w)), "ctts_gpt_create")
            pool.append((h, torch.cuda.Stream(device=self.device)))
        return pool[:n]

    def generate(self, emb: torch.Tensor, inputs_ids: torch.Tensor, temperature: torch.Tensor, eos_token: int = GPT.n_audio - 1,
                 attention_mask: Optional[torch.Tensor] = None, max_new_token: int = 2048, min_new_token: int = 0,
                 logits_processors: Sequence = (), infer_text: bool = False, return_attn: bool = False,
                 return_hidden: bool = False, stream: bool = False, show_tqdm: bool = False, ensure_non_empty: bool = True,
                 stream_batch: int = 24, manual_seed: Optional[int] = None, context: Optional[Context] = None,
                 *, use_graph: bool = True, stop_at: Optional[torch.Tensor] = None, row_offset: int = 0,
                 total_rows: Optional[int] = None, profile_tag: Optional[int] = None,
                 profile_stride: int = 1, lanes: Optional[int] = None,
                 teacher_ids: Optional[torch.Tensor] = None, prefill_chunk: Optional[int] = None,
                 return_sampled: bool = False, rng: Optional[str] = None, rng_seed: Optional[int] = None,
                 rng_nonce=None, row_ids: Optional[torch.Tensor] = None, exact: bool = False,
                 text_rng: Optional[str] = None) -> Iterator[GenerationOutputs]:
        if return_attn:
            raise NotImplementedError("return_attn is not supported by the fused attention kernel")
        context = context or Context()
        plan = plan_from_processors(logits_processors, infer_text)
        lib, dev = self.lib, self.device
        B, T, nvq = inputs_ids.shape
        assert nvq == GPT.n_vq and emb.shape == (B, T, GPT.hidden)
        nrow = 1 if infer_text else nvq
        V = GPT.n_text if infer_text else GPT.n_audio
        max_new = int(max_new_token)
        if T + max_new > self.max_pos:
            raise ValueError(f"T + max_new_token = {T + max_new} exceeds max_position_embeddings {self.max_pos}")
        if attention_mask is None:
            attention_mask = torch.ones((B, T), dtype=torch.bool)
        kv_start_all = left_pad_starts(attention_mask)
        n_lanes = self.default_lanes if lanes is None else int(lanes)
        n_lanes = max(1, min(n_lanes, B))
        exact = bool(exact) and self.x3 is not None
        certify = self.certify and teacher_ids is None
        rng_state0 = torch.get_rng_state() if (manual_seed is None and self.exact_fallback and not exact) else None
        rid = None
        if row_ids is not None:
            rid = torch.as_tensor(row_ids, dtype=torch.int64).reshape(-1).cpu()
            assert rid.numel() == B and total_rows is not None, "row_ids needs one global index per utterance and total_rows"
        if profile_tag is not None or not use_graph:
            n_lanes = 1
        from .dist import shard_bounds
        bounds = [shard_bounds(B, n_lanes, i) for i in range(n_lanes)]
        slot_sfx = "_alt" if exact else ("_text" if infer_text else "")
        res = self._lane_resources(n_lanes, slot_sfx)
        caller = torch.cuda.current_stream(dev)
        rng_mode = rng or self.rng
        if rng_mode not in ("host", "device"):
            raise ValueError("rng must be 'host' or 'device'")
        if text_rng not in (None, "host", "device"):
            raise ValueError("text_rng must be 'host' or 'device'")
        device_rng = (text_rng == "device") if infer_text else rng_mode == "device"
        dkey = (total_rows if total_rows is not None else B * nrow, V, manual_seed, row_offset, B * nrow, None if rid is None else tuple(rid.tolist()))
        if device_rng:
            draws = None
            seed_val = int(rng_seed) if rng_seed is not None else (int(manual_seed) if manual_seed is not None
                                                                    else int(torch.randint(0, 2 ** 62, (1,)).item()))
        elif manual_seed is not None and self._draws_cache is not None and self._draws_cache[0] == dkey:
            draws = self._draws_cache[1]
        else:
            srows = None if rid is None else (rid[:, None] * nrow + torch.arange(nrow)[None, :]).reshape(-1)
            draws = ExpDraws(dkey[0], V, manual_seed, row_begin=row_offset, row_end=row_offset + B * nrow, rows=srows)
            self._draws_cache = (dkey, draws) if draws.constant else None
        const_q = device_rng or draws.constant
        ptab = penalty_table(plan.penalty)
        nq = 1 if const_q else self.NQ_RING
        emb_all = emb.to(torch.float32).contiguous().to(dev)
        ids_all = inputs_ids.to(dev)
        temp_d = temperature.to(torch.float32).reshape(-1).to(dev)
        assert temp_d.numel() == nrow, "temperature must have one entry per sampling row of an utterance"
        ptab_d = None if ptab is None else ptab.to(dev)
        wait_stream(caller)

        class Lane:
            pass

        top_p_thr = float(np.float32(1.0 - plan.top_p)) if plan.top_p is not None else 0.0
        key = (tuple(bounds), T, max_new, nrow, V, nq, self.dtype, top_p_thr, plan.top_p is not None, int(plan.top_k or 0),
               plan.top_k is not None, int(min_new_token), int(eos_token), int(row_offset), bool(infer_text), stop_at is not None,
               ptab is not None, teacher_ids is not None, bool(return_sampled),
               None if prefill_chunk is None else int(prefill_chunk), device_rng, manual_seed is None, device_rng and rng_nonce is not None,
               exact, certify, rid is not None)
        slot = "_session" + slot_sfx
        sess = getattr(self, slot)
        sess = sess if (sess is not None and sess["key"] == key) else None
        if sess is None:
            setattr(self, slot, None)
            sess = dict(key=key, lanes=[], graph=False, temp=torch.empty((nrow,), dtype=torch.float32, device=dev),
                        ptab=None if ptab is None else torch.empty_like(ptab, device=dev), q_sig=None,
                        seed=torch.zeros((1,), dtype=torch.int64, device=dev))
            for (lo, hi), (handle, st) in zip(bounds, res):
                ln = Lane()
                ln.lo, ln.hi, ln.handle, ln.st = lo, hi, handle, st
                Bl = hi - lo
                with torch.cuda.stream(st):
                    ln.ids_buf = torch.empty((Bl, T + max_new, nvq), dtype=torch.int64, device=dev)
                    ln.len_d = torch.empty((Bl,), dtype=torch.int32, device=dev)
                    Bp = (Bl + 15) // 16 * 16
                    ln.state_blk = torch.zeros((5 * Bp,), dtype=torch.uint8, device=dev)
                    ln.finish = ln.state_blk[:Bl]
                    ln.order = torch.empty((Bl,), dtype=torch.int32, device=dev)
                    ln.n_active = torch.empty((1,), dtype=torch.int32, device=dev)
                    ln.end_idx = ln.state_blk[Bp:].view(torch.int32)[:Bl]
                    ln.hiddens = torch.empty((Bl, max_new, GPT.hidden), dtype=torch.float32, device=dev)
                    kv_shape = (self.n_layers, Bl, GPT.n_heads, T + max_new, GPT.head_dim)
                    ln.kcache = torch.empty(kv_shape, dtype=self.wdt, device=dev)
                    ln.vcache = torch.empty(kv_shape, dtype=self.wdt, device=dev)
# ... 305 lines not shown
                    inflight.clear()
                if stream:
                    emit = False
                    if not all_done and steps_done % stream_batch == 0:
                        emit = True
                    elif all_done:
                        i_star = max(max(ln.end_snap) for ln in L)
                        emit = i_star > 0 and i_star % stream_batch == 0
                    if emit:
                        yield outputs()
                if context.get():
                    interrupted = True
                    while inflight:
                        n2, snaps2 = inflight.pop(0)
                        for ln, k in zip(L, snaps2):
                            if k is not None and not ln.done:
                                collect(ln, k)
                        steps_done += n2
                    all_done = all(ln.done for ln in L)
                    break
            if profile_tag is not None:
                n_s, tot = C.c_int32(0), C.c_double(0.0)
                buf = (C.c_float * 4096)()
                _lib.check(lib.ctts_gpt_profile_samples(L[0].handle, buf, 4096, C.byref(n_s)), "profile_samples")
                self.last_stats["profile_samples_ms"] = np.ctypeslib.as_array(buf)[: int(n_s.value)].copy()
                _lib.check(lib.ctts_gpt_profile_end(L[0].handle, C.byref(n_s), C.byref(tot)), "profile_end")
                self.last_stats["profile"] = (int(n_s.value), float(tot.value))
        finally:
            if feeder is not None:
                feeder["pool"].shutdown(wait=True)
            for ln in L:
                wait_stream(ln.st)
            self.last_stats["decode_ms"] = 1e3 * (_time.perf_counter() - t_dec0)
        if not all_done:
            if interrupted:
                self.logger.warning("generation is interrupted")
            else:
                self.logger.warning(f"incomplete result. hit max_new_token: {max_new_token}")
        self.last_stats.update(steps=steps_done, B=B, T=T, lanes=n_lanes)
        for ln in L:
            if not ln.done or ln.end_snap is None:
                poll(ln)
        steps_ref = (max(max(ln.end_snap) for ln in L) + 1) if all_done else min(steps_done, max_new)
        finish_rng(min(steps_ref, max_new))
        if return_sampled:
            self.last_sampled = [ln.sampled[b, : ln.end_snap[b]].clone() for ln in L for b in range(ln.hi - ln.lo)]
        final = outputs()
        if certify:
            marg = torch.cat([ln.margin for ln in L]).cpu().numpy()
            x3_run = self.x3 is not None and not exact
            bound = 2.0 * self.REL_ERR_X3 * self.logit_scale[bool(infer_text)] / max(float(temperature.min()), 1e-6) if x3_run else 0.0
            unsafe = np.nonzero(marg < bound)[0].tolist()
            self.last_margins = marg
            self.last_stats.update(min_margin=float(marg.min()) if marg.size else float("inf"), margin_bound=bound,
                                   certified=not unsafe, uncertified_rows=unsafe, exact_rerun_rows=[])
            if unsafe:
                (self.logger.warning if self.exact_fallback else self.logger.info)(
                                    "parity certificate: %d of %d utterances had a draw decided by less than %.2e tempered-logit units "
                                    "(smallest margin %.2e)%s", len(unsafe), B, bound, float(marg.min()),
                                    "; generating them again on the exact f32 kernels" if (self.exact_fallback and not stream and not interrupted)
                                    else "; the split-fp16 result stands as it is")
                if self.exact_fallback and not stream and not interrupted:
                    final = self._rerun_exact(final, unsafe, emb, inputs_ids, temperature, eos_token, attention_mask, max_new_token, min_new_token,
                                              logits_processors, infer_text, return_hidden, stream_batch, manual_seed, context, use_graph, stop_at,
                                              row_offset // nrow, (total_rows if total_rows is not None else B * nrow), prefill_chunk, rng,
                                              seed_val if device_rng else None, rng_nonce, rid, rng_state0, text_rng)
        yield final

    def _rerun_exact(self, final, rows, emb, inputs_ids, temperature, eos_token, attention_mask, max_new_token, min_new_token,
                     logits_processors, infer_text, return_hidden, stream_batch, manual_seed, context, use_graph, stop_at, first_row,
                     total_rows, prefill_chunk, rng, rng_seed, rng_nonce, rid, rng_state0, text_rng=None):
        stats = dict(self.last_stats)
        sel = torch.tensor(rows, dtype=torch.long)
        gid = rid[sel] if rid is not None else sel + int(first_row)
        nz = None
        if rng_nonce is not None:
            nz = torch.as_tensor(rng_nonce, dtype=torch.int64).reshape(-1)
            nz = nz if nz.numel() == 1 else nz[sel]
        state_after = None
        if rng_state0 is not None:
            state_after = torch.get_rng_state()
            torch.set_rng_state(rng_state0)
        sub = None
        try:
            for sub in self.generate(emb[sel.to(emb.device)], inputs_ids[sel.to(inputs_ids.device)], temperature, eos_token,
                                     None if attention_mask is None else attention_mask[sel.to(attention_mask.device)], max_new_token, min_new_token,
                                     logits_processors, infer_text, False, return_hidden, False, False, False, stream_batch, manual_seed, context,
                                     use_graph=use_graph, stop_at=None if stop_at is None else stop_at[sel.to(stop_at.device)], total_rows=total_rows,
                                     lanes=1, prefill_chunk=prefill_chunk, rng=rng, rng_seed=rng_seed, rng_nonce=nz, row_ids=gid, exact=True, text_rng=text_rng):
                pass
        finally:
            if state_after is not None:
                keep_rerun = sub is not None and (len(rows) == len(final.ids) or self.last_stats.get("steps", 0) > stats.get("steps", 0))
                if not keep_rerun:
                    torch.set_rng_state(state_after)
        rerun_stats = self.last_stats
        self.last_stats = stats
        if sub is None:
            self.logger.warning("parity certificate: the exact re-run ended at step 0; the split-fp16 rows stand")
            return final
        same_len = all(int(sub.ids[j].shape[0]) == int(final.ids[b].shape[0]) for j, b in enumerate(rows))
        padded = getattr(final.hiddens, "padded", None)
        if return_hidden and not (same_len and padded is not None):
            final.hiddens = RowList(list(final.hiddens))
            padded = None
        for j, b in enumerate(rows):
            final.ids[b] = sub.ids[j]
            if return_hidden:
                if padded is not None:
                    padded[b, : sub.hiddens[j].shape[0]].copy_(sub.hiddens[j])
                else:
                    final.hiddens[b] = sub.hiddens[j]
        self.last_stats.update(exact_rerun_rows=list(rows), exact_rerun_steps=rerun_stats.get("steps"),
                               exact_rerun_min_margin=rerun_stats.get("min_margin"), certified=True)
        return final


def split_bf16(w: torch.Tensor) -> torch.Tensor:
    N, K = w.shape
    Kp = (K + 31) // 32 * 32
    wp = torch.zeros((N, Kp), dtype=torch.float32)
    wp[:, :K] = w
    hi = wp.to(torch.bfloat16)
    lo = (wp - hi.to(torch.float32)).to(torch.bfloat16)
    return torch.stack([hi.view(N, Kp // 32, 32), lo.view(N, Kp // 32, 32)], 2).contiguous()


def pack_x3p(w: torch.Tensor) -> torch.Tensor:
    R, K = w.shape
    assert R % 32 == 0 and K % 16 == 0
    w = w.to(torch.float32)
    hi = w.to(torch.bfloat16)
    lo = (w - hi.to(torch.float32)).to(torch.bfloat16)
    x = torch.stack([hi, lo], 0).reshape(2, R // 32, 32, K // 16, 2, 8)
    return x.permute(1, 3, 0, 4, 2, 5).contiguous()


def unpack_x3p(p: torch.Tensor, R: int, K: int) -> torch.Tensor:
    x = p.reshape(R // 32, K // 16, 2, 2, 32, 8).permute(2, 0, 4, 1, 3, 5).reshape(2, R, K).to(torch.float32)
    return x[0] + x[1]


def pack_h1p(w: torch.Tensor) -> torch.Tensor:
    R, K = w.shape
    assert R % 32 == 0 and K % 16 == 0
    h = w.to(torch.float32).clamp(-65504.0, 65504.0).to(torch.float16)
    return h.reshape(R // 32, 32, K // 16, 2, 8).permute(0, 2, 3, 1, 4).contiguous()


def unpack_h1p(p: torch.Tensor, R: int, K: int) -> torch.Tensor:
    return p.reshape(R // 32, K // 16, 2, 32, 8).permute(0, 3, 1, 2, 4).reshape(R, K).to(torch.float32)


class PendingWavs:

    def __init__(self, codec, view, done, keep):
        self._codec, self._view, self._done, self._keep, self._out = codec, view, done, keep, None

    def done(self) -> bool:
        return self._out is not None or self._done.query()

    def result(self) -> np.ndarray:
        if self._out is None:
            wait_event(self._done)
            self._out = self._codec._copy_out(self._view) if self._view.numel() else np.zeros(tuple(self._view.shape), np.float32)
            self._keep = None
        return self._out


def ragged_offsets(lens):
    lens = np.asarray(lens, dtype=np.int64)
    tok = np.zeros(len(lens) + 1, np.int64)
    np.cumsum(lens, out=tok[1:])
    off = VOCOS.hop * (2 * tok - np.arange(len(lens) + 1))
    return tok.astype(np.int32), off, keep_offsets(off)


def keep_offsets(off) -> np.ndarray:
    off = np.asarray(off, dtype=np.int64)
    k = np.zeros(len(off), np.int64)
    np.cumsum((np.diff(off) + 7) // 8, out=k[1:])
    return k


def group_starts(off, grp) -> np.ndarray:
    off, grp = np.asarray(off, dtype=np.int64), np.asarray(grp, dtype=np.int64)
    s = np.zeros(len(grp), np.int64)
    np.cumsum((np.diff(off[grp]) + 7) // 8 * 8, out=s[1:])
    return s


def ragged_views(flat, off) -> list:
    return [flat[int(off[i]): int(off[i + 1])] for i in range(len(off) - 1)]


HALO_FRAMES = 27 + 75


def window_for_samples(Tn: int, s_lo: int, s_hi: int):
    Tn = int(Tn)
    hop, nfft = VOCOS.hop, VOCOS.n_fft
    total = hop * (2 * Tn - 1)
    s_lo, s_hi = max(0, int(s_lo)), min(total, int(s_hi))
    if s_hi <= s_lo:
        return None
    f_a = (s_lo + nfft // 2) // hop - (nfft // hop - 1)
    f_b = min((s_hi - 1 + nfft // 2) // hop, 2 * Tn - 1)
    t_lo = max(0, (f_a - HALO_FRAMES) // 2)
    t_hi = min(Tn, (f_b + HALO_FRAMES) // 2 + 1)
    off = 2 * hop * t_lo
    return t_lo, t_hi, s_lo - off, s_hi - off


class CodecEngine:

    def __init__(self, decoder_sd: dict, vocos_sd: dict, device: torch.device, gemm: str = "bf16x3"):
        if gemm not in ("bf16x3", "f32", "f16"):
            raise ValueError("gemm must be 'bf16x3', 'f16' or 'f32'")
        self.gemm = gemm
        self.lib = _lib.lib()
        self.device = torch.device(device)
        if self.device.type != "cuda":
            raise _lib.EngineError("CodecEngine needs a ROCm GPU device (there is no CPU path)")
        dev = self.device
        f = lambda t: t.to(torch.float32).contiguous().to(dev)
        dww = lambda t: f(t[:, 0, :].t())

        def dense(t):
            t = t.to(torch.float32).reshape(t.shape[0], -1).contiguous()
            if gemm == "f32":
                return t.to(dev)
            return split_bf16(t).to(dev)

        convw = lambda t: dense(t.permute(0, 2, 1))
        self.keep = []
        k = self.keep.append
        w = _lib.CodecWeights()

        def P(t):
            k(t)
            return t.data_ptr()

        def PA(ts):
            k(ts)
            arr = _lib.ptr_array(ts)
            k(arr)
            return C.cast(arr, _lib.PP)

        d = decoder_sd
        w.conv_in0_w, w.conv_in0_b = P(convw(d["decoder.conv_in.0.weight"])), P(f(d["decoder.conv_in.0.bias"]))
        w.conv_in2_w, w.conv_in2_b = P(convw(d["decoder.conv_in.2.weight"])), P(f(d["decoder.conv_in.2.bias"]))
        nb = 0
        while f"decoder.decoder_block.{nb}.weight" in d:
            nb += 1
        w.n_dvae_blocks = nb
        blk = lambda i, n: d[f"decoder.decoder_block.{i}.{n}"]
        w.d_dw_w = PA([dww(blk(i, "dwconv.weight")) for i in range(nb)])
        w.d_dw_b = PA([f(blk(i, "dwconv.bias")) for i in range(nb)])
        w.d_ln_w = PA([f(blk(i, "norm.weight")) for i in range(nb)])
        w.d_ln_b = PA([f(blk(i, "norm.bias")) for i in range(nb)])
        w.d_pw1_w = PA([dense(blk(i, "pwconv1.weight")) for i in range(nb)])
        w.d_pw1_b = PA([f(blk(i, "pwconv1.bias")) for i in range(nb)])
        w.d_pw2_w = PA([dense(blk(i, "pwconv2.weight")) for i in range(nb)])
        w.d_pw2_b = PA([f(blk(i, "pwconv2.bias")) for i in range(nb)])
        w.d_gamma = PA([f(blk(i, "weight")) for i in range(nb)])
        w.conv_out_w = P(dense(d["decoder.conv_out.weight"][:, :, 0]))
        w.out_conv_w = P(convw(d["out_conv.weight"]))
        w.coef = P(f(d["coef"].reshape(-1)))
        v = vocos_sd
        w.v_embed_w, w.v_embed_b = P(convw(v["backbone.embed.weight"])), P(f(v["backbone.embed.bias"]))
        w.v_norm_w, w.v_norm_b = P(f(v["backbone.norm.weight"])), P(f(v["backbone.norm.bias"]))
        nv = 0
        while f"backbone.convnext.{nv}.gamma" in v:
            nv += 1
        w.n_vocos_blocks = nv
        vb = lambda i, n: v[f"backbone.convnext.{i}.{n}"]
        w.v_dw_w = PA([dww(vb(i, "dwconv.weight")) for i in range(nv)])
        w.v_dw_b = PA([f(vb(i, "dwconv.bias")) for i in range(nv)])
        w.v_ln_w = PA([f(vb(i, "norm.weight")) for i in range(nv)])
        w.v_ln_b = PA([f(vb(i, "norm.bias")) for i in range(nv)])
        w.v_pw1_w = PA([dense(vb(i, "pwconv1.weight")) for i in range(nv)])
        w.v_pw1_b = PA([f(vb(i, "pwconv1.bias")) for i in range(nv)])
        w.v_pw2_w = PA([dense(vb(i, "pwconv2.weight")) for i in range(nv)])
        w.v_pw2_b = PA([f(vb(i, "pwconv2.bias")) for i in range(nv)])
        w.v_gamma = PA([f(vb(i, "gamma")) for i in range(nv)])
        w.v_final_w, w.v_final_b = P(f(v["backbone.final_layer_norm.weight"])), P(f(v["backbone.final_layer_norm.bias"]))
        w.head_w, w.head_b = P(dense(v["head.out.weight"])), P(f(v["head.out.bias"]))
        w.window = P(f(v["head.istft.window"]))
        kk = torch.arange(VOCOS.n_fft // 2, dtype=torch.float64) * (2.0 * math.pi / VOCOS.n_fft)
        w.twiddle = P(f(torch.stack([kk.cos(), kk.sin()], 1)))
        w.gemm_mode = {"f32": 0, "bf16x3": 1, "f16": 2}[gemm]
        if gemm == "f16":
            h1p = lambda t: pack_h1p(t.to(torch.float32).reshape(t.shape[0], -1)).to(dev)
            w.d_pw1_x3p = PA([h1p(blk(i, "pwconv1.weight")) for i in range(nb)])
            w.d_pw2_x3p = PA([h1p(blk(i, "pwconv2.weight")) for i in range(nb)])
            w.v_pw1_x3p = PA([h1p(vb(i, "pwconv1.weight")) for i in range(nv)])
            w.v_pw2_x3p = PA([h1p(vb(i, "pwconv2.weight")) for i in range(nv)])
        if gemm == "bf16x3":
            x3p = lambda t: pack_x3p(t.to(torch.float32).reshape(t.shape[0], -1)).to(dev)
            w.d_pw1_x3p = PA([x3p(blk(i, "pwconv1.weight")) for i in range(nb)])
            w.d_pw2_x3p = PA([x3p(blk(i, "pwconv2.weight")) for i in range(nb)])
            w.v_pw1_x3p = PA([x3p(vb(i, "pwconv1.weight")) for i in range(nv)])
            w.v_pw2_x3p = PA([x3p(vb(i, "pwconv2.weight")) for i in range(nv)])
        self._w = w
        h = C.c_void_p()
        _lib.check(self.lib.ctts_codec_create(C.byref(h), C.byref(w)), "ctts_codec_create")
# ... 677 lines not shown
```

include/chattts_amd.h:

```cpp
#ifndef CHATTTS_AMD_H
#define CHATTTS_AMD_H

#include <stddef.h>
#include <stdint.h>

#ifdef __cplusplus
extern "C" {
#endif

#define CTTS_F32 0
#define CTTS_BF16 1

typedef struct ctts_gpt ctts_gpt;
typedef struct ctts_codec ctts_codec;

const char* ctts_last_error(void);
int ctts_version(void);

typedef struct {
  int32_t n_layers;
  int32_t weight_dtype;
  int32_t kv_dtype;
  int32_t max_pos;
  const void* const* wqkv;
  const void* const* wo;
  const void* const* wgu;
  const void* const* wd;
  const float* const* ln1;
  const float* const* ln2;
  const float* norm;
  const float* emb_code;
  const float* heads;
  const float* rope_cos;
  const float* rope_sin;
  float rms_eps;
  const float* emb_text;
  const float* head_text;
  int32_t n_text;
  const void* const* wqkv_pk;
  const void* const* wo_pk;
  const void* const* wgu_pk;
  const void* const* wd_pk;
  const float* heads_pk;
  const float* head_text_pk;
  const void* const* wo_hd;
  const void* const* wqkv_x3;
  const void* const* wo_x3;
  const void* const* wgu_x3;
  const void* const* wd_x3;
} ctts_gpt_weights;

typedef struct {
  float temperature[4];
  float pow_table[17];
  int32_t use_penalty;
  float top_p_thr;
  int32_t use_top_p;
  int32_t top_k;
  int32_t use_top_k;
  int32_t min_new;
  int32_t reserved0;
  uint64_t rng_seed;
  int32_t rng_per_step;
  int32_t reserved1;
} ctts_sampling_row;

typedef struct {
  int32_t B, T, max_new;
  int64_t* ids_buf;
  int32_t* len;
  const int32_t* kv_start;
  uint8_t* finish;
  int32_t* end_idx;
  float* hiddens;
  void* kcache;
  void* vcache;
  const float* q;
  int32_t nq;
  const float* temperature;
  const float* pow_table;
  float top_p_thr;
  int32_t use_top_p;
  int32_t top_k;
  int32_t use_top_k;
  int32_t min_new;
  int32_t eos;
  int32_t row_offset;
  const int32_t* stop_at;
  void* workspace;
  size_t workspace_bytes;
  const int32_t* row_map;
  const int32_t* n_active;
  int32_t cap;
  int32_t hid_cap;
  int32_t kv_batch;
  int32_t q_batch;
  const int32_t* prompt_len;
  int32_t infer_text;
  const int64_t* teacher_ids;
  int64_t* sampled_ids;
  const int32_t* order;
  int32_t rng_device;
  int32_t rng_per_step;
  const uint64_t* rng_seed;
  const uint32_t* rng_nonce;
  float* margin;
  const int32_t* row_base;
  int32_t proj_exact;
  int32_t prefill_valid_rows;
  const ctts_sampling_row* row_sampling;
} ctts_gen_state;

int ctts_gpt_create(ctts_gpt** out, const ctts_gpt_weights* w);
void ctts_gpt_destroy(ctts_gpt* g);
size_t ctts_gpt_workspace_bytes(int32_t B, int32_t T);

int ctts_gpt_prefill(ctts_gpt* g, const ctts_gen_state* s, const float* emb, void* stream);
int ctts_gpt_prefill_chunk(ctts_gpt* g, const ctts_gen_state* s, const float* emb_chunk, int32_t t0, int32_t tc, int32_t last, void* stream);
int ctts_gpt_decode_step(ctts_gpt* g, const ctts_gen_state* s, void* stream);
int ctts_gpt_graph_build(ctts_gpt* g, const ctts_gen_state* s, void* stream);
int ctts_gpt_graph_launch(ctts_gpt* g, int32_t n_steps, void* stream);
int ctts_gpt_graph_build_rows(ctts_gpt* g, const ctts_gen_state* s, int32_t rows, void* stream);
int ctts_gpt_graph_launch_rows(ctts_gpt* g, int32_t n_steps, int32_t rows, void* stream);
void ctts_gpt_graph_destroy(ctts_gpt* g);

int ctts_gpt_profile_begin(ctts_gpt* g, int32_t tag, int32_t max_samples, int32_t stride );
int ctts_gpt_profile_samples(ctts_gpt* g, float* ms_out, int32_t cap, int32_t* n_samples);
int ctts_gpt_profile_end(ctts_gpt* g, int32_t* n_samples, double* total_ms);

typedef struct {
  const float* conv_in0_w; const float* conv_in0_b;
  const float* conv_in2_w; const float* conv_in2_b;
  int32_t n_dvae_blocks;
  const float* const* d_dw_w; const float* const* d_dw_b;
  const float* const* d_ln_w; const float* const* d_ln_b;
  const float* const* d_pw1_w; const float* const* d_pw1_b;
  const float* const* d_pw2_w; const float* const* d_pw2_b;
  const float* const* d_gamma;
  const float* conv_out_w;
  const float* out_conv_w;
  const float* coef;
  const float* v_embed_w; const float* v_embed_b;
  const float* v_norm_w; const float* v_norm_b;
  int32_t n_vocos_blocks;
  const float* const* v_dw_w; const float* const* v_dw_b;
  const float* const* v_ln_w; const float* const* v_ln_b;
  const float* const* v_pw1_w; const float* const* v_pw1_b;
  const float* const* v_pw2_w; const float* const* v_pw2_b;
  const float* const* v_gamma;
  const float* v_final_w; const float* v_final_b;
  const float* head_w; const float* head_b;
  const float* window;
  const float* twiddle;
  int32_t gemm_mode;
  const void* const* d_pw1_x3p; const void* const* d_pw2_x3p;
  const void* const* v_pw1_x3p; const void* const* v_pw2_x3p;
} ctts_codec_weights;

int ctts_codec_create(ctts_codec** out, const ctts_codec_weights* w);
void ctts_codec_destroy(ctts_codec* c);
size_t ctts_codec_workspace_bytes(int32_t B, int32_t F);
typedef struct { char internal[128]; } ctts_rccl_id;
int ctts_rccl_unique_id(ctts_rccl_id* out);
int ctts_rccl_comm_create(void** comm , int32_t world, const ctts_rccl_id* id, int32_t rank);
void ctts_rccl_comm_destroy(void* comm);
int ctts_broadcast_weights(void* const* bufs, const size_t* bytes, int32_t n, void* comm , int32_t root, void* stream);

int ctts_float_to_int16(const float* wav, int16_t* pcm, uint8_t* keep_bits, int32_t rows, int64_t n, int64_t ld, int32_t per_row,
                        int32_t product, float keep_thr, uint32_t* peak, void* stream);
int ctts_copy_bytes(void* dst, const void* src, size_t bytes, void* stream);
int ctts_dvae_decode(ctts_codec* c, const float* hid, float* mel, int32_t B, int32_t T, void* workspace, size_t ws_bytes, void* stream);
int ctts_vocos_decode(ctts_codec* c, const float* mel, float* wav, int32_t B, int32_t F, void* workspace, size_t ws_bytes, void* stream);

size_t ctts_codec_ragged_workspace_bytes(int32_t n_seg, int32_t total_tokens);
int ctts_dvae_decode_ragged(ctts_codec* c, const float* hid, const int32_t* tok_off_dev, const int32_t* tok_off_host, int32_t n_seg,
                            float* mel, void* workspace, size_t ws_bytes, void* stream);
int ctts_vocos_decode_ragged(ctts_codec* c, const float* mel, const int32_t* tok_off_dev, const int32_t* tok_off_host, int32_t n_seg,
                             float* wav, void* workspace, size_t ws_bytes, void* stream);
int ctts_float_to_int16_ragged(const float* wav, int16_t* pcm, uint8_t* keep_bits, const int64_t* off_dev, const int64_t* off_host,
                               int32_t n_seg, int32_t product, float keep_thr, uint32_t* peak, void* stream);

size_t ctts_float_to_int16_groups_scratch_bytes(const int64_t* off_host, int32_t n_seg, const int32_t* grp_host, int32_t n_grp);
int ctts_float_to_int16_groups(const float* wav, int16_t* pcm, int64_t* n_kept, const int64_t* off_dev, const int64_t* off_host, int32_t n_seg,
                               const int32_t* grp_dev, const int32_t* grp_host, int32_t n_grp, int32_t product, float keep_thr, uint32_t* peak,
                               void* scratch, size_t scratch_bytes, void* stream);

int32_t ctts_resample_supported(int32_t L, int32_t M, int32_t K);
int ctts_resample_ragged(const float* x, const int64_t* off_in_dev, const int64_t* off_in_host, float* y, const int64_t* off_out_dev,
                         const int64_t* off_out_host, int32_t n_seg, const int32_t* sel_dev, const int32_t* sel_host, int32_t n_sel,
                         const float* taps, int32_t L, int32_t M, int32_t K, void* stream);

int ctts_time_scale_ragged(const float* x, const int64_t* off_in_dev, const int64_t* off_in_host, float* y, const int64_t* off_out_dev,
                           const int64_t* off_out_host, int32_t* path, const int64_t* path_off_dev, const int64_t* path_off_host, int32_t n_seg,
                           const float* window, int32_t num, int32_t den, void* stream);

typedef struct {
  int32_t slot;
  int32_t t_lo, t_hi;
  int32_t c_lo, c_hi;
  int32_t keep;
  int32_t reserved[2];
} ctts_window;
size_t ctts_codec_windows_workspace_bytes(int32_t n_win, int32_t total_tokens);
int ctts_codec_decode_windows(ctts_codec* c, const float* hid, int64_t slot_stride, int64_t row_stride, int32_t n_slots, int32_t hid_cap,
                              const ctts_window* win_dev, const ctts_window* win_host, int32_t n_win, int32_t out_type, void* out,
                              uint8_t* keep_bits, int32_t product, float keep_thr, void* workspace, size_t ws_bytes, void* stream);

typedef struct {
  int64_t in_off, n_in;
  int64_t origin;
  int64_t total;
  int64_t o_lo, o_hi;
  int64_t out_off;
  int32_t rate;
  int32_t pad;
} ctts_rs_window;
int ctts_resample_windows(const float* x, int64_t n_x, const ctts_rs_window* win_dev, const ctts_rs_window* win_host, int32_t n_win, float* y,
                          int64_t n_y, const int32_t* sel_dev, const int32_t* sel_host, int32_t n_sel, const float* taps, int32_t L, int32_t M,
                          int32_t K, void* stream);

typedef struct {
  const float* taps;
  int32_t L, M, K, reserved;
} ctts_rate;
size_t ctts_codec_windows_rate_workspace_bytes(int32_t n_win, int32_t total_tokens, int64_t chunk_floats);
int ctts_codec_decode_windows_rate(ctts_codec* c, const float* hid, int64_t slot_stride, int64_t row_stride, int32_t n_slots, int32_t hid_cap,
                                   const ctts_window* win_dev, const ctts_window* win_host, const ctts_rs_window* rs_dev,
                                   const ctts_rs_window* rs_host, const int32_t* sel_dev, const int32_t* sel_host, int32_t n_win,
                                   const ctts_rate* rates, int32_t n_rates, int32_t out_type, void* out, uint8_t* keep_bits, int32_t product,
                                   float keep_thr, void* workspace, size_t ws_bytes, void* stream);

typedef struct {
  int64_t start;
  int64_t n;
  int32_t law;
  int32_t reserved0;
  int64_t reserved1;
} ctts_g711_range;
int ctts_g711_encode_ranges(const int16_t* pcm, uint8_t* out, const ctts_g711_range* rng_dev, const ctts_g711_range* rng_host, int32_t n_rng,
                            void* stream);

typedef struct ctts_dvae ctts_dvae;

typedef struct {
  int32_t idim, odim, hidden , bn_dim, n_blocks;
  const float* conv_in0_w; const float* conv_in0_b;
  const float* conv_in2_w; const float* conv_in2_b;
  const float* const* dw_w; const float* const* dw_b;
  const float* const* ln_w; const float* const* ln_b;
  const float* const* pw1_w; const float* const* pw1_b;
  const float* const* pw2_w; const float* const* pw2_b;
  const float* const* gamma;
  const float* conv_out_w;
} ctts_trunk_weights;

typedef struct {
  ctts_trunk_weights encoder;
  ctts_trunk_weights decoder;
  const float* ds0_w; const float* ds0_b;
  const float* ds1_w; const float* ds1_b;
  const float* out_conv_w;
  const float* coef;
  const float* q_in_w; const float* q_in_b;
  const float* q_out_w; const float* q_out_b;
  int32_t levels[4];
  int32_t G, R, D;
  int32_t bound_first;
  const float* mel_window;
  const float* mel_fb;
  const float* twiddle;
} ctts_dvae_weights;

int ctts_dvae_create(ctts_dvae** out, const ctts_dvae_weights* w);
void ctts_dvae_destroy(ctts_dvae* c);
int32_t ctts_dvae_code_frames(int32_t n_samples);
size_t ctts_dvae_encode_workspace_bytes(int32_t n_samples);
size_t ctts_dvae_decode_workspace_bytes(int32_t B, int32_t T);
int ctts_dvae_encode(ctts_dvae* c, const float* wav, int32_t n_samples, int32_t* codes, void* workspace, size_t ws_bytes, void* stream);
int ctts_dvae_decode_codes(ctts_dvae* c, const int64_t* codes, float* mel, int32_t B, int32_t T, void* workspace, size_t ws_bytes,
                           void* stream);

int ctts_k_gemm(int32_t tiled , const float* A, const void* W, float* C, int32_t M, int32_t N, int32_t K, int32_t lda, int32_t ldc,
                int32_t wt, int32_t epi, const float* norm_w, float eps, const float* res, int32_t ldr, const float* bias,
                const float* gamma, int32_t taps, int32_t cin, int32_t frames, int32_t pad, int32_t dil, void* stream);
int ctts_k_gemm_x3p(const uint16_t* Ap, const uint16_t* Wp, int32_t M, int32_t N, int32_t K, int32_t epi, const float* bias,
                    const float* gamma, const float* res, float* C, uint16_t* Cp, void* stream);
int ctts_k_gemm_h1p(const uint16_t* Ap, const uint16_t* Wp, int32_t M, int32_t N, int32_t K, int32_t epi, const float* bias,
                    const float* gamma, const float* res, float* C, uint16_t* Cp, void* stream);
int ctts_stream_create_cu_mask(int32_t first_cu, int32_t n_cus, int32_t stride, int32_t complement , void** stream);
int ctts_stream_destroy(void* stream);
int ctts_k_mlp_fused(const uint16_t* Ap, const uint16_t* W1p, const uint16_t* W2p, int32_t M, int32_t inter, const float* b1,
                     const float* b2, const float* gamma, float* C, int32_t planes, void* stream);
int ctts_k_gemm_fast(const uint16_t* A, int32_t lda, const uint16_t* W, int32_t M, int32_t N, int32_t K, const float* ssq_in, float eps,
                     int32_t epi, float* C32, int32_t ldc, uint16_t* Cb, int32_t ldcb, float* ssq_out, void* stream);
int ctts_k_qkv_rope(const uint16_t* A, const uint16_t* W, int32_t M, const float* ssq_in, float eps, float* qkv, uint16_t* kcache,
                    uint16_t* vcache, int32_t cmax, const float* cos_tab, const float* sin_tab, int32_t q_per_b, const int32_t* len,
                    const int32_t* kv_start, int32_t force_mb, void* stream);
int ctts_k_gemm_dec(const uint16_t* Ap, const uint16_t* Wp, int32_t M, int32_t N, int32_t K, const int32_t* n_active, const float* ssq_in,
                    float eps, int32_t epi, float* C32, int32_t ldc, uint16_t* Cp, int32_t kch_out, float* ssq_out, int32_t force_mb,
                    void* stream);
int ctts_k_gemm_dec32(const float* Ap, const float* Wp, int32_t M, int32_t N, int32_t K, const int32_t* n_active, const float* X, int32_t ldx,
                      const float* norm_w, float eps, int32_t epi, float* C, int32_t ldc, const float* res, int32_t ldr, float* Cp,
                      int32_t kch_out, int32_t force_mb, int32_t n_cols ,
                      void* stream);
int ctts_k_gemm_dec32x(const uint16_t* Ap, int64_t a_plane, const uint16_t* Wp, int64_t w_plane, int32_t M, int32_t N, int32_t K,
                       const int32_t* n_active, const float* X, int32_t ldx, float eps, int32_t epi, float* C, int32_t ldc, const float* res,
                       int32_t ldr, uint16_t* Cp, int64_t c_plane, int32_t kch_out, float* Cp32, int32_t force_mb, const float* ssq_in,
                       float* ssq_out, void* stream);
int ctts_k_gemm_pre_x3(const float* A, int32_t lda, const float* W, float* C, int32_t ldc, int32_t M, int32_t N, int32_t K, int32_t epi,
                       const float* norm_w, const float* rstd, const float* res, int32_t ldr, void* stream);
const char* ctts_k_dec32_last_variant(void);
int ctts_k_rows_prep(const float* x32, uint16_t* xb, float* ssq, int32_t M, void* stream);
int ctts_k_rope_append(float* qkv, void* kcache, void* vcache, int32_t kv_dtype, int32_t cmax, const float* cos_tab, const float* sin_tab,
                       int32_t q_per_b, const int32_t* len, const int32_t* kv_start, int32_t M, void* stream);
int ctts_k_attention(const float* qkv, const void* kcache, const void* vcache, int32_t kv_dtype, int32_t cmax, float* out,
                     int32_t q_per_b, const int32_t* len, const int32_t* kv_start, int32_t M, void* stream);
int ctts_k_attention_prefill(const float* qkv, const uint16_t* kcache, const uint16_t* vcache, int32_t cmax, float* out, int32_t q_per_b,
                             int32_t slot0, const int32_t* kv_start, int32_t M, void* stream);
int ctts_k_attention_dec(const float* qkv, const uint16_t* kcache, const uint16_t* vcache, int32_t cmax, uint16_t* out_packed,
                         const int32_t* desc, const int32_t* n_active, int32_t M, float* part, int32_t* cnt, int32_t n_cu, void* stream);
int ctts_k_attention_dec2(const float* qkv, const void* kcache, const void* vcache, int32_t kv_dtype, int32_t cmax, void* out_packed,
                          const int32_t* desc, const int32_t* n_active, int32_t covers_all, int32_t M, void* stream);
int ctts_k_attention_cfg(int32_t persist, int32_t workgroups, int32_t ring);
int ctts_k_attention_heads_per_wg(int32_t hpw);
int ctts_k_attention_oproj(const float* qkv, const uint16_t* kcache, const uint16_t* vcache, int32_t cmax, const uint16_t* wo_hd,
                           const int32_t* desc, const int32_t* n_active, int32_t M, float* part, int32_t* cnt, float* x32, uint16_t* xp,
                           float* ssq, void* stream);
int ctts_k_device_guard_probe(void* stream, int32_t* before, int32_t* stream_dev, int32_t* inside, int32_t* switched);
int ctts_k_embed_codes(const float* emb_code, const int64_t* ids_buf, int32_t tcap, const int32_t* len, float* x, int32_t B, void* stream);
int ctts_k_final_norm(const float* x, int32_t q_per_b, const float* w, float eps, float* hfin, float* hiddens, int32_t max_new,
                      const int32_t* len, int32_t T, int32_t B, void* stream);
int ctts_k_sample(const ctts_gen_state* s, const float* logits, void* stream);
int ctts_k_sample_text(const ctts_gen_state* s, const float* logits, int32_t n_text, void* stream);
int ctts_k_exp_draws(uint64_t seed, int32_t step, int32_t row0, int32_t rows, int32_t V, float* out, void* stream);
int ctts_k_dwconv_ln(const float* x, const float* w, const float* b, const float* ln_w, const float* ln_b, float eps, int32_t dil,
                     float* y, int32_t B, int32_t F, void* stream);
int ctts_k_layernorm(const float* x, const float* w, const float* b, float eps, float* y, int32_t rows, void* stream);
int ctts_k_istft(const float* head, const float* window, const float* twiddle, float* frames, float* wav, int32_t B, int32_t F, void* stream);

#ifdef __cplusplus
}
#endif
#endif
```

Before: 1059.

## Pre-split prefill weights into fp16 hi/lo fragment planes for x3 GEMM

Adds a load-time kernel that splits each f32 layer weight into fp16 high and low planes in an MFMA fragment layout. It also adds a new prefill GEMM kernel that streams these pre-split planes straight into shared memory instead of splitting f32 weights on every call. The kernel double-buffers with register prefetch and picks its tile size from the problem shape. It is enabled by default when x3 weights exist, and costs extra weight memory, plus a new rule that rejects one-slot prefill chunks.

```diff
diff --git a/chattts_amd/_lib.py b/chattts_amd/_lib.py
--- a/chattts_amd/_lib.py
+++ b/chattts_amd/_lib.py
@@ -26,6 +26,7 @@
         ("heads_pk", P), ("head_text_pk", P),
         ("wo_hd", PP),
         ("wqkv_x3", PP), ("wo_x3", PP), ("wgu_x3", PP), ("wd_x3", PP),
+        ("wqkv_x3w", PP), ("wo_x3w", PP), ("wgu_x3w", PP), ("wd_x3w", PP),
     ]
 
 
@@ -162,6 +163,9 @@
     "ctts_k_gemm_dec": (C.c_int, [P, P, I32, I32, I32, P, P, F, I32, P, I32, P, I32, P, I32, P]),
     "ctts_k_gemm_dec32x": (C.c_int, [P, C.c_int64, P, C.c_int64, I32, I32, I32, P, P, I32, F, I32, P, I32, P, I32, P, C.c_int64, I32, P, I32, P, P, P]),
     "ctts_k_gemm_pre_x3": (C.c_int, [P, I32, P, P, I32, I32, I32, I32, I32, P, P, P, I32, P]),
+    "ctts_k_split_x3w": (C.c_int, [P, I32, I32, P, P]),
+    "ctts_k_gemm_pre_x3w": (C.c_int, [P, I32, P, P, I32, I32, I32, I32, I32, P, P, P, I32, P]),
+    "ctts_k_gemm_pre_x3w_tile": (C.c_int, [I32]),
     "ctts_k_dec32_last_variant": (C.c_char_p, []),
     "ctts_k_gemm_dec32": (C.c_int, [P, P, I32, I32, I32, P, P, I32, P, F, I32, P, I32, P, I32, P, I32, I32, I32, P]),
     "ctts_k_rows_prep": (C.c_int, [P, P, P, I32, P]),
diff --git a/chattts_amd/csrc/capi.hip b/chattts_amd/csrc/capi.hip
--- a/chattts_amd/csrc/capi.hip
+++ b/chattts_amd/csrc/capi.hip
@@ -37,6 +37,8 @@
   std::vector<const void*> wqkv_pk, wo_pk, wgu_pk, wd_pk;
   std::vector<const void*> wo_hd;
   std::vector<const void*> wqkv_x3, wo_x3, wgu_x3, wd_x3;
+  std::vector<const void*> wqkv_x3w, wo_x3w, wgu_x3w, wd_x3w;
+  bool pre_x3w = false;
   bool dec_x3 = false;
   bool qkv_att = false;
   bool att_oproj = false;
@@ -157,6 +159,14 @@
     g->wgu_x3.assign(w->wgu_x3, w->wgu_x3 + L);
     g->wd_x3.assign(w->wd_x3, w->wd_x3 + L);
     g->dec_x3 = true;
+  }
+  if (w->wqkv_x3w && w->wo_x3w && w->wgu_x3w && w->wd_x3w && g->dec_x3) {
+    g->wqkv_x3w.assign(w->wqkv_x3w, w->wqkv_x3w + L);
+    g->wo_x3w.assign(w->wo_x3w, w->wo_x3w + L);
+    g->wgu_x3w.assign(w->wgu_x3w, w->wgu_x3w + L);
+    g->wd_x3w.assign(w->wd_x3w, w->wd_x3w + L);
+    const char* e = getenv("CTTS_PRE_X3W");
+    g->pre_x3w = !(e && atoi(e) == 0);
   }
   if (w->wo_hd && g->dec_packed) {
     g->wo_hd.assign(w->wo_hd, w->wo_hd + L);
@@ -429,6 +439,8 @@
   }
   const bool pre_x3 = !fast && !dec && g->dec_x3 && !s->proj_exact && g->pre_x3;
   const bool pre32 = !fast && !dec && g->dec_packed32 && g->pre32_packed && !pre_x3;
+  const bool x3w = pre_x3 && g->pre_x3w;
+  hipError_t (*const pre_gemm)(const GemmArgs&, const float*, hipStream_t) = x3w ? launch_gemm_pre_x3w : launch_gemm_pre_x3;
   if (pre32) {
     CK(launch_prefill_prep32(ws.x, ws.xp32, ws.desc, q_per_b, slot0, s->kv_start, s->row_map, M, st));
   }
@@ -464,21 +476,25 @@
     a.n_active = nact;
     a.A = ws.x; a.lda = HID; a.W = g->wqkv[l]; a.C = ws.qkv; a.ldc = 3 * HID; a.M = M; a.N = 3 * HID; a.K = HID; a.wt = wt;
     a.epi = EPI_STORE; a.norm_w = g->ln1[l]; a.eps = g->w.rms_eps;
-    if (pre_x3) { CK(launch_rows_rstd32(ws.x, HID, M, g->w.rms_eps, ws.rstd, st)); CK(launch_gemm_pre_x3(a, ws.rstd, st)); }
+    if (x3w) a.W = g->wqkv_x3w[l];
+    if (pre_x3) { CK(launch_rows_rstd32(ws.x, HID, M, g->w.rms_eps, ws.rstd, st)); CK(pre_gemm(a, ws.rstd, st)); }
     else { Prof p(g, 1, st, prof_ok); CK(launch_gemm_skinny(a, st)); }
     { Prof p(g, 2, st, prof_ok); CK(launch_rope_append(ws.qkv, kc, vc, kt, cmax, g->w.rope_cos, g->w.rope_sin, rm, M, st)); }
     { Prof p(g, 3, st, prof_ok); CK(launch_attention(ws.qkv, kc, vc, kt, cmax, ws.ao, 0, rm, M, st)); }
     a.A = ws.ao; a.lda = HID; a.W = g->wo[l]; a.C = ws.x; a.ldc = HID; a.N = HID; a.K = HID; a.epi = EPI_RES; a.norm_w = nullptr;
     a.res = ws.x; a.ldr = HID;
-    if (pre_x3) CK(launch_gemm_pre_x3(a, nullptr, st));
+    if (x3w) a.W = g->wo_x3w[l];
+    if (pre_x3) CK(pre_gemm(a, nullptr, st));
     else { Prof p(g, 4, st, prof_ok); CK(launch_gemm_skinny(a, st)); }
     a.A = ws.x; a.W = g->wgu[l]; a.C = ws.act; a.ldc = INTER; a.N = INTER; a.K = HID; a.epi = EPI_SILU_MUL; a.norm_w = g->ln2[l];
     a.res = nullptr;
-    if (pre_x3) { CK(launch_rows_rstd32(ws.x, HID, M, g->w.rms_eps, ws.rstd, st)); CK(launch_gemm_pre_x3(a, ws.rstd, st)); }
+    if (x3w) a.W = g->wgu_x3w[l];
+    if (pre_x3) { CK(launch_rows_rstd32(ws.x, HID, M, g->w.rms_eps, ws.rstd, st)); CK(pre_gemm(a, ws.rstd, st)); }
     else { Prof p(g, 5, st, prof_ok); CK(launch_gemm_skinny(a, st)); }
     a.A = ws.act; a.lda = INTER; a.W = g->wd[l]; a.C = ws.x; a.ldc = HID; a.N = HID; a.K = INTER; a.epi = EPI_RES; a.norm_w = nullptr;
     a.res = ws.x; a.ldr = HID;
-    if (pre_x3) CK(launch_gemm_pre_x3(a, nullptr, st));
+    if (x3w) a.W = g->wd_x3w[l];
+    if (pre_x3) CK(pre_gemm(a, nullptr, st));
     else { Prof p(g, 6, st, prof_ok); CK(launch_gemm_skinny(a, st)); }
   }
   if (!heads) return 0;
@@ -554,6 +570,8 @@
   if (check_state(g, s, tc > 0 ? tc : 1)) return -1;
   if (t0 < 0 || tc <= 0 || t0 + tc > s->T || (last && t0 + tc != s->T)) return fail("ctts_gpt_prefill_chunk: bad chunk [%d, %d) of a %d-slot prompt", t0, t0 + tc, s->T);
   if (s->workspace_bytes < ctts_gpt_workspace_bytes(s->B, tc)) return fail("workspace too small for the chunk");
+  if (tc == 1 && g->w.weight_dtype != CTTS_BF16 && g->dec_x3 && !s->proj_exact)
+    return fail("ctts_gpt_prefill_chunk: a one-slot chunk is not supported by the split-fp16 arithmetic (choose a chunk size that leaves a tail of 2 or more slots)");
   CttsDeviceGuard dg(stream);
   hipStream_t st = (hipStream_t)stream;
   const GptWs ws = carve(s->workspace, s->B, tc);
@@ -1323,6 +1341,24 @@
   CK(launch_gemm_pre_x3(a, rstd, (hipStream_t)stream));
   return 0;
 }
+extern "C" int ctts_k_split_x3w(const float* W, int32_t R, int32_t K, uint16_t* planes, void* stream) {
+  CK(launch_split_x3w(W, planes, R, K, (hipStream_t)stream));
+  return 0;
+}
+extern "C" int ctts_k_gemm_pre_x3w(const float* A, int32_t lda, const uint16_t* Wp, float* C, int32_t ldc, int32_t M, int32_t N, int32_t K, int32_t epi,
+                                   const float* norm_w, const float* rstd, const float* res, int32_t ldr, void* stream) {
+  GemmArgs a;
+  memset(&a, 0, sizeof(a));
+  a.taps = 1; a.A = A; a.lda = lda; a.W = Wp; a.C = C; a.ldc = ldc; a.M = M; a.N = N; a.K = K; a.wt = WT_F32; a.epi = epi;
+  a.norm_w = norm_w; a.res = res; a.ldr = ldr;
+  CK(launch_gemm_pre_x3w(a, rstd, (hipStream_t)stream));
+  return 0;
+}
+extern "C" int ctts_k_gemm_pre_x3w_tile(int32_t tile) {
+  if (tile < 0 || tile > 3) return fail("ctts_k_gemm_pre_x3w_tile: 0 (by shape), 1 (64 x 64), 2 (64 x 128) or 3 (128 x 128)");
+  gemm_pre_x3w_tile_override(tile);
+  return 0;
+}
 extern "C" int ctts_k_sample(const ctts_gen_state* s, const float* logits, void* stream) {
   if (!s || !logits) return fail("ctts_k_sample: bad arguments");
   CK(launch_sample(make_sample_args(s, logits), (hipStream_t)stream));
diff --git a/chattts_amd/csrc/common.hpp b/chattts_amd/csrc/common.hpp
--- a/chattts_amd/csrc/common.hpp
+++ b/chattts_amd/csrc/common.hpp
@@ -34,6 +34,25 @@
   const _Float16 l = (_Float16)((v - (float)h) * X3_LO_SCALE);
   hi = __builtin_bit_cast(uint16_t, h);
   lo = __builtin_bit_cast(uint16_t, l);
+}
+
+typedef float xf2 __attribute__((ext_vector_type(2)));
+typedef _Float16 xb2 __attribute__((ext_vector_type(2)));
+
+__device__ __forceinline__ void split2(const float a, const float b, uint32_t& hi, uint32_t& lo) {
+  const xf2 v = {a > 65504.0f ? 65504.0f : (a < -65504.0f ? -65504.0f : a), b > 65504.0f ? 65504.0f : (b < -65504.0f ? -65504.0f : b)};
+  const xb2 h = __builtin_convertvector(v, xb2);
+  hi = __builtin_bit_cast(uint32_t, h);
+  const xf2 hf = __builtin_convertvector(h, xf2);
+  const xb2 l = __builtin_convertvector((v - hf) * X3_LO_SCALE, xb2);
+  lo = __builtin_bit_cast(uint32_t, l);
+}
+__device__ __forceinline__ void split4(const float4 v, ushort4& hi, ushort4& lo) {
+  uint32_t h0, l0, h1, l1;
+  split2(v.x, v.y, h0, l0);
+  split2(v.z, v.w, h1, l1);
+  hi = __builtin_bit_cast(ushort4, make_uint2(h0, h1));
+  lo = __builtin_bit_cast(ushort4, make_uint2(l0, l1));
 }
 
 typedef float f32x2_t __attribute__((ext_vector_type(2)));
diff --git a/chattts_amd/csrc/kernels.hpp b/chattts_amd/csrc/kernels.hpp
--- a/chattts_amd/csrc/kernels.hpp
+++ b/chattts_amd/csrc/kernels.hpp
@@ -68,6 +68,9 @@
 
 hipError_t launch_gemm_skinny(const GemmArgs& a, hipStream_t st);
 hipError_t launch_gemm_pre_x3(const GemmArgs& a, const float* rstd, hipStream_t st);
+hipError_t launch_split_x3w(const float* W, uint16_t* planes, int R, int K, hipStream_t st);
+hipError_t launch_gemm_pre_x3w(const GemmArgs& a, const float* rstd, hipStream_t st);
+void gemm_pre_x3w_tile_override(int tile);
 
 enum FastEpi { FEPI_STORE32 = 0, FEPI_RES = 1, FEPI_SILU = 2, FEPI_QKV_ROPE = 3 };
 #define SSQ_PARTS 48
diff --git a/chattts_amd/csrc/prefill32x.hip b/chattts_amd/csrc/prefill32x.hip
--- a/chattts_amd/csrc/prefill32x.hip
+++ b/chattts_amd/csrc/prefill32x.hip
@@ -8,24 +8,6 @@
 constexpr int XBK = 32, XLD = XBK + 8;
 constexpr int XNT = 256;
 
-typedef float xf2 __attribute__((ext_vector_type(2)));
-typedef _Float16 xb2 __attribute__((ext_vector_type(2)));
-
-__device__ __forceinline__ void split2(const float a, const float b, uint32_t& hi, uint32_t& lo) {
-  const xf2 v = {a > 65504.0f ? 65504.0f : (a < -65504.0f ? -65504.0f : a), b > 65504.0f ? 65504.0f : (b < -65504.0f ? -65504.0f : b)};
-  const xb2 h = __builtin_convertvector(v, xb2);
-  hi = __builtin_bit_cast(uint32_t, h);
-  const xf2 hf = __builtin_convertvector(h, xf2);
-  const xb2 l = __builtin_convertvector((v - hf) * X3_LO_SCALE, xb2);
-  lo = __builtin_bit_cast(uint32_t, l);
-}
-__device__ __forceinline__ void split4(const float4 v, ushort4& hi, ushort4& lo) {
-  uint32_t h0, l0, h1, l1;
-  split2(v.x, v.y, h0, l0);
-  split2(v.z, v.w, h1, l1);
-  hi = __builtin_bit_cast(ushort4, make_uint2(h0, h1));
-  lo = __builtin_bit_cast(ushort4, make_uint2(l0, l1));
-}
 
 template <int EPI, int MBLK>
 __global__ __launch_bounds__(XNT) void gemm_pre_x3_k(GemmArgs a, const float* __restrict__ rstd) {
@@ -145,6 +127,169 @@
 #pragma unroll
         for (int j = 0; j < 2; ++j) {
           const int col = n0 + wn * 64 + j * 32 + cl;
+          if (col >= N) continue;
+          const float v = acc[i][j][r] * rs;
+          a.C[(size_t)row * a.ldc + col] = (EPI == EPI_RES) ? a.res[(size_t)row * a.ldr + col] + v : v;
+        }
+      }
+    }
+  }
+}
+
+__global__ __launch_bounds__(256) void split_x3w_k(const float* __restrict__ W, uint16_t* __restrict__ planes, int R, int K) {
+  const size_t u = (size_t)blockIdx.x * 256 + threadIdx.x;
+  const size_t units = (size_t)R * K / 8;
+  if (u >= units) return;
+  const int lane = (int)(u & 63), kch = K / 16;
+  const size_t chunk = u >> 6;
+  const int rb = (int)(chunk / kch), kc = (int)(chunk % kch);
+  const float* src = W + (size_t)(rb * 32 + (lane & 31)) * K + kc * 16 + (lane >> 5) * 8;
+  ushort4 h0, l0, h1, l1;
+  split4(*reinterpret_cast<const float4*>(src), h0, l0);
+  split4(*reinterpret_cast<const float4*>(src + 4), h1, l1);
+  uint4 h, l;
+  h.x = __builtin_bit_cast(uint2, h0).x; h.y = __builtin_bit_cast(uint2, h0).y; h.z = __builtin_bit_cast(uint2, h1).x; h.w = __builtin_bit_cast(uint2, h1).y;
+  l.x = __builtin_bit_cast(uint2, l0).x; l.y = __builtin_bit_cast(uint2, l0).y; l.z = __builtin_bit_cast(uint2, l1).x; l.w = __builtin_bit_cast(uint2, l1).y;
+  *reinterpret_cast<uint4*>(planes + u * 8) = h;
+  *reinterpret_cast<uint4*>(planes + (size_t)R * K + u * 8) = l;
+}
+
+template <int EPI, int MBLK, int NBLK, int XK>
+__global__ __launch_bounds__(XNT, 2) void gemm_pre_x3w_k(GemmArgs a, const float* __restrict__ rstd) {
+  constexpr bool SILU = EPI == EPI_SILU_MUL;
+  static_assert(!SILU || NBLK == 2, "SILU tile: one gate and one up block per wave");
+  constexpr int BM = 64 * MBLK;
+  constexpr int NBW = 2 * NBLK;
+  constexpr int BNO = SILU ? 64 : 64 * NBLK;
+  constexpr int KC = XK / 16;
+  constexpr int FR = 64 * 8;
+  __shared__ __attribute__((aligned(16))) uint16_t As[2][2][2 * MBLK][KC][FR], Ws[2][NBW][KC][2][FR];
+  __shared__ float rstd_s[BM];
+
+  const int tid = threadIdx.x, wave = tid >> 6, lane = tid & 63;
+  const int wm = wave & 1, wn = wave >> 1;
+  const int M = a.M, N = a.N, K = a.K;
+  const int m0 = blockIdx.y * BM, n0 = blockIdx.x * BNO;
+  const uint16_t* Wp = reinterpret_cast<const uint16_t*>(a.W);
+  const size_t plane = (size_t)(SILU ? 2 * N : N) * K;
+
+  if (rstd != nullptr && tid < BM) rstd_s[tid] = rstd[min(m0 + tid, M - 1)];
+
+  constexpr int UPR = XK / 8, PA = BM * UPR / XNT;
+  const int ku = tid % UPR;
+  const float* ap[PA];
+  int ad[PA];
+#pragma unroll
+  for (int p = 0; p < PA; ++p) {
+    const int r = (tid + XNT * p) / UPR;
+    ap[p] = a.A + (size_t)min(m0 + r, M - 1) * a.lda + ku * 8;
+    ad[p] = (((r >> 5) * KC + (ku >> 1)) * 64 + (ku & 1) * 32 + (r & 31)) * 8;
+  }
+  constexpr int PW = NBW * KC * 2 / 4;
+  const uint16_t* wp[PW];
+#pragma unroll
+  for (int p = 0; p < PW; ++p) {
+    const int f = wave + 4 * p, pl = f & 1, kc = (f >> 1) % KC, bw = (f >> 1) / KC;
+    const int gb = SILU ? ((bw & 1) * N + n0) / 32 + (bw >> 1) : n0 / 32 + bw;
+    wp[p] = Wp + pl * plane + (((size_t)gb * (K / 16) + kc) * 64 + lane) * 8;
+  }
+  float4 ra[PA][2], rg[2];
+  u32x4_t rw[PW];
+#define XW_FETCH(K0)                                                                                              \
+  do {                                                                                                            \
+    _Pragma("unroll") for (int p = 0; p < PA; ++p) {                                                              \
+      ra[p][0] = *reinterpret_cast<const float4*>(ap[p] + (K0));                                                  \
+      ra[p][1] = *reinterpret_cast<const float4*>(ap[p] + (K0) + 4);                                              \
+    }                                                                                                             \
+    _Pragma("unroll") for (int p = 0; p < PW; ++p) rw[p] = *reinterpret_cast<const u32x4_t*>(wp[p] + (size_t)(K0) * 32); \
+    if (a.norm_w != nullptr) {                                                                                    \
+      rg[0] = *reinterpret_cast<const float4*>(a.norm_w + (K0) + ku * 8);                                         \
+      rg[1] = *reinterpret_cast<const float4*>(a.norm_w + (K0) + ku * 8 + 4);                                     \
+    } else {                                                                                                      \
+      rg[0] = make_float4(1.f, 1.f, 1.f, 1.f); rg[1] = rg[0];                                                     \
+    }                                                                                                             \
+  } while (0)
+#define XW_STAGE(SB)                                                                                              \
+  do {                                                                                                            \
+    _Pragma("unroll") for (int p = 0; p < PA; ++p) {                                                              \
+      ushort4 h0, l0, h1, l1;                                                                                     \
+      split4(make_float4(ra[p][0].x * rg[0].x, ra[p][0].y * rg[0].y, ra[p][0].z * rg[0].z, ra[p][0].w * rg[0].w), h0, l0); \
+      split4(make_float4(ra[p][1].x * rg[1].x, ra[p][1].y * rg[1].y, ra[p][1].z * rg[1].z, ra[p][1].w * rg[1].w), h1, l1); \
+      uint16_t* dh = &As[SB][0][0][0][0] + ad[p];                                                                 \
+      uint16_t* dl = &As[SB][1][0][0][0] + ad[p];                                                                 \
+      *reinterpret_cast<ushort4*>(dh) = h0; *reinterpret_cast<ushort4*>(dh + 4) = h1;                             \
+      *reinterpret_cast<ushort4*>(dl) = l0; *reinterpret_cast<ushort4*>(dl + 4) = l1;                             \
+    }                                                                                                             \
+    _Pragma("unroll") for (int p = 0; p < PW; ++p)                                                                \
+      *reinterpret_cast<u32x4_t*>(&Ws[SB][0][0][0][0] + (size_t)(tid + XNT * p) * 8) = rw[p];                       \
+  } while (0)
+
+  f32x16 acc[MBLK][NBLK], accx[MBLK][NBLK];
+#pragma unroll
+  for (int i = 0; i < MBLK; ++i)
+#pragma unroll
+    for (int j = 0; j < NBLK; ++j)
+#pragma unroll
+      for (int r = 0; r < 16; ++r) { acc[i][j][r] = 0.f; accx[i][j][r] = 0.f; }
+
+  XW_FETCH(0);
+  XW_STAGE(0);
+  if (XK < K) XW_FETCH(XK);
+  __syncthreads();
+  int sb = 0;
+  for (int k0 = 0; k0 < K; k0 += XK) {
+    if (k0 + XK < K) XW_STAGE(sb ^ 1);
+    if (k0 + 2 * XK < K) XW_FETCH(k0 + 2 * XK);
+#pragma unroll
+    for (int kc = 0; kc < KC; ++kc) {
+      f16x8 wh[NBLK], wl[NBLK];
+#pragma unroll
+      for (int j = 0; j < NBLK; ++j) {
+        wh[j] = *reinterpret_cast<const f16x8*>(&Ws[sb][wn * NBLK + j][kc][0][lane * 8]);
+        wl[j] = *reinterpret_cast<const f16x8*>(&Ws[sb][wn * NBLK + j][kc][1][lane * 8]);
+      }
+#pragma unroll
+      for (int i = 0; i < MBLK; ++i) {
+        const f16x8 ah = *reinterpret_cast<const f16x8*>(&As[sb][0][wm * MBLK + i][kc][lane * 8]);
+        const f16x8 al = *reinterpret_cast<const f16x8*>(&As[sb][1][wm * MBLK + i][kc][lane * 8]);
+#pragma unroll
+        for (int j = 0; j < NBLK; ++j) {
+          f32x16 x = accx[i][j];
+          x = __builtin_amdgcn_mfma_f32_32x32x16_f16(al, wh[j], x, 0, 0, 0);
+          x = __builtin_amdgcn_mfma_f32_32x32x16_f16(ah, wl[j], x, 0, 0, 0);
+          accx[i][j] = x;
+          acc[i][j] = __builtin_amdgcn_mfma_f32_32x32x16_f16(ah, wh[j], acc[i][j], 0, 0, 0);
+        }
+      }
+    }
+    __syncthreads();
+    sb ^= 1;
+  }
+#undef XW_FETCH
+#undef XW_STAGE
+
+#pragma unroll
+  for (int i = 0; i < MBLK; ++i)
+#pragma unroll
+    for (int j = 0; j < NBLK; ++j)
+#pragma unroll
+      for (int r = 0; r < 16; ++r) acc[i][j][r] += accx[i][j][r] * X3_LO_INV;
+  const int cl = lane & 31;
+#pragma unroll
+  for (int i = 0; i < MBLK; ++i) {
+#pragma unroll
+    for (int r = 0; r < 16; ++r) {
+      const int lrow = (wm * MBLK + i) * 32 + (r & 3) + 8 * (r >> 2) + 4 * (lane >> 5);
+      const int row = m0 + lrow;
+      if (row >= M) continue;
+      const float rs = rstd != nullptr ? rstd_s[lrow] : 1.0f;
+      if (EPI == EPI_SILU_MUL) {
+        const int col = n0 + wn * 32 + cl;
+        a.C[(size_t)row * a.ldc + col] = silu_f(acc[i][0][r] * rs) * (acc[i][NBLK - 1][r] * rs);
+      } else {
+#pragma unroll
+        for (int j = 0; j < NBLK; ++j) {
+          const int col = n0 + (wn * NBLK + j) * 32 + cl;
           if (col >= N) continue;
           const float v = acc[i][j][r] * rs;
           a.C[(size_t)row * a.ldc + col] = (EPI == EPI_RES) ? a.res[(size_t)row * a.ldr + col] + v : v;
@@ -181,3 +326,51 @@
   }
   return hipGetLastError();
 }
+
+hipError_t launch_split_x3w(const float* W, uint16_t* planes, int R, int K, hipStream_t st) {
+  if (!W || !planes || R <= 0 || K <= 0 || (R % 32) || (K % 16)) return hipErrorInvalidValue;
+  const size_t units = (size_t)R * K / 8;
+  CTTS_LAUNCH(split_x3w_k, dim3((unsigned)((units + 255) / 256)), dim3(256), st, W, planes, R, K);
+  return hipGetLastError();
+}
+
+static int g_x3w_tile = 0;
+void gemm_pre_x3w_tile_override(int tile) { g_x3w_tile = tile; }
+
+hipError_t launch_gemm_pre_x3w(const GemmArgs& a, const float* rstd, hipStream_t st) {
+  if (a.M <= 0 || a.N <= 0 || a.K <= 0 || (a.K % 64) || (a.lda & 3) || !a.A || !a.W || !a.C || a.taps != 1) return hipErrorInvalidValue;
+  if ((a.norm_w != nullptr) != (rstd != nullptr)) return hipErrorInvalidValue;
+  const bool silu = a.epi == EPI_SILU_MUL;
+  if (silu ? (a.N % 64) != 0 : (a.N % 128) != 0) return hipErrorInvalidValue;
+  if (a.epi == EPI_RES && !a.res) return hipErrorInvalidValue;
+  static int env_tile = -1;
+  if (env_tile < 0) { const char* e = getenv("CTTS_PREX3W_TILE"); env_tile = e ? atoi(e) : 0; }
+  int tile = g_x3w_tile ? g_x3w_tile : (env_tile == 1 && silu ? 2 : env_tile);
+  if (tile == 1 && silu) return hipErrorInvalidValue;
+  if (tile < 0 || tile > 3) return hipErrorInvalidValue;
+  if (tile == 0) {
+    const long nx128 = silu ? a.N / 64 : a.N / 128;
+    if (nx128 * ((a.M + 127) / 128) >= 512) tile = 3;
+    else if (silu || nx128 * ((a.M + 63) / 64) >= 256) tile = 2;
+    else tile = 1;
+  }
+  const dim3 block(XNT);
+  const dim3 grid(tile == 1 ? a.N / 64 : (silu ? a.N / 64 : a.N / 128), tile == 3 ? (a.M + 127) / 128 : (a.M + 63) / 64);
+#define XW_GO(E)                                                                                                  \
+  do {                                                                                                            \
+    if (tile == 3) CTTS_LAUNCH((gemm_pre_x3w_k<E, 2, 2, 32>), grid, block, st, a, rstd);                          \
+    else CTTS_LAUNCH((gemm_pre_x3w_k<E, 1, 2, 32>), grid, block, st, a, rstd);                                    \
+  } while (0)
+  switch (a.epi) {
+    case EPI_SILU_MUL: XW_GO(EPI_SILU_MUL); break;
+    case EPI_RES:
+      if (tile == 1) CTTS_LAUNCH((gemm_pre_x3w_k<EPI_RES, 1, 1, 64>), grid, block, st, a, rstd); else XW_GO(EPI_RES);
+      break;
+    case EPI_STORE:
+      if (tile == 1) CTTS_LAUNCH((gemm_pre_x3w_k<EPI_STORE, 1, 1, 64>), grid, block, st, a, rstd); else XW_GO(EPI_STORE);
+      break;
+    default: return hipErrorInvalidValue;
+  }
+#undef XW_GO
+  return hipGetLastError();
+}
diff --git a/chattts_amd/engine.py b/chattts_amd/engine.py
--- a/chattts_amd/engine.py
+++ b/chattts_amd/engine.py
@@ -277,6 +277,12 @@
             self.x3 = [[pack_frag_x3(gain(t[qk_perm], g_)) for t, g_ in zip(self.wqkv, self.ln1)], [pack_frag_x3(t) for t in self.wo],
                        [pack_frag_x3(gain(t, g_)) for t, g_ in zip(self.wgu, self.ln2)], [pack_frag_x3(t) for t in self.wd]]
             self._x3_arrs = [_lib.ptr_array(x) for x in self.x3]
+        self.x3w, self._x3w_arrs = None, None
+        if self.x3 is not None and os.environ.get("CTTS_PRE_X3W", "1") != "0":
+            with torch.cuda.device(dev):
+                self.x3w = [[split_x3w(self.lib, t) for t in ws] for ws in (self.wqkv, self.wo, self.wgu, self.wd)]
+            torch.cuda.synchronize(dev)
+            self._x3w_arrs = [_lib.ptr_array(x) for x in self.x3w]
         self.wo_hd = [pack_wo_heads(t) for t in self.wo] if (use_packed and dtype == "bf16" and os.environ.get("CTTS_ATT_OPROJ") == "1") else None
         self._wo_hd_arr = None if self.wo_hd is None else _lib.ptr_array(self.wo_hd)
 
@@ -299,6 +305,8 @@
             w.wo_hd = C.cast(self._wo_hd_arr, _lib.PP)
         if self._x3_arrs is not None:
             w.wqkv_x3, w.wo_x3, w.wgu_x3, w.wd_x3 = [C.cast(a, _lib.PP) for a in self._x3_arrs]
+        if self._x3w_arrs is not None:
+            w.wqkv_x3w, w.wo_x3w, w.wgu_x3w, w.wd_x3w = [C.cast(a, _lib.PP) for a in self._x3w_arrs]
         self._w = w
         h = C.c_void_p()
         _lib.check(self.lib.ctts_gpt_create(C.byref(h), C.byref(w)), "ctts_gpt_create")
@@ -910,6 +918,29 @@
     return p.reshape(R // 32, K // 16, 2, 32, 8).permute(0, 3, 1, 2, 4).reshape(R, K).to(torch.float32)
 
 
+def pack_x3w(w: torch.Tensor) -> torch.Tensor:
+    hi, lo = split_f16(w)
+    R, K = w.shape
+    return torch.stack([pack_h1p(hi.float()), pack_h1p(lo.float())], 0).reshape(2, R // 32, K // 16, 64, 8).contiguous()
+
+
+def unpack_x3w(p: torch.Tensor, R: int, K: int):
+    q = p.reshape(2, R // 32, K // 16, 2, 32, 8).permute(0, 1, 4, 2, 3, 5).reshape(2, R, K)
+    return q[0], q[1]
+
+
+def x3w_offset(r: int, k: int, K: int) -> int:
+    return (((r // 32) * (K // 16) + k // 16) * 64 + (k % 16) // 8 * 32 + r % 32) * 8 + k % 8
+
+
+def split_x3w(lib, w: torch.Tensor) -> torch.Tensor:
+    R, K = w.shape
+    assert w.is_cuda and w.dtype == torch.float32 and w.is_contiguous() and R % 32 == 0 and K % 16 == 0
+    out = torch.empty((2, R // 32, K // 16, 64, 8), dtype=torch.float16, device=w.device)
+    _lib.check(lib.ctts_k_split_x3w(w.data_ptr(), R, K, out.data_ptr(), torch.cuda.current_stream(w.device).cuda_stream), "ctts_k_split_x3w")
+    return out
+
+
 class PendingWavs:
 
     def __init__(self, codec, view, done, keep):
diff --git a/include/chattts_amd.h b/include/chattts_amd.h
--- a/include/chattts_amd.h
+++ b/include/chattts_amd.h
@@ -48,6 +48,10 @@
   const void* const* wo_x3;
   const void* const* wgu_x3;
   const void* const* wd_x3;
+  const void* const* wqkv_x3w;
+  const void* const* wo_x3w;
+  const void* const* wgu_x3w;
+  const void* const* wd_x3w;
 } ctts_gpt_weights;
 
 typedef struct {
@@ -309,6 +313,10 @@
                        float* ssq_out, void* stream);
 int ctts_k_gemm_pre_x3(const float* A, int32_t lda, const float* W, float* C, int32_t ldc, int32_t M, int32_t N, int32_t K, int32_t epi,
                        const float* norm_w, const float* rstd, const float* res, int32_t ldr, void* stream);
+int ctts_k_split_x3w(const float* W, int32_t R, int32_t K, uint16_t* planes, void* stream);
+int ctts_k_gemm_pre_x3w(const float* A, int32_t lda, const uint16_t* Wp, float* C, int32_t ldc, int32_t M, int32_t N, int32_t K, int32_t epi,
+                        const float* norm_w, const float* rstd, const float* res, int32_t ldr, void* stream);
+int ctts_k_gemm_pre_x3w_tile(int32_t tile);
 const char* ctts_k_dec32_last_variant(void);
 int ctts_k_rows_prep(const float* x32, uint16_t* xb, float* ssq, int32_t M, void* stream);
 int ctts_k_rope_append(float* qkv, void* kcache, void* vcache, int32_t kv_dtype, int32_t cmax, const float* cos_tab, const float* sin_tab,
```

New measurement: 1065 (median of 3 runs). No clear change (+0.6%).
